# snap-research/graphless-neural-networks

Measured on AMD Instinct MI355X. Metric: aggregated edges/sec (teacher fwd) + student distill steps/sec, ogbn-products 1/2/4/8 GPU, higher is better.
Workload: dtype f32; 1 GPU; ogbn-products-shaped SAGE teacher forward (3 layers 100-256-256-47, BN, layer-wise full-neighbour inference, reference models.py:121-148) + MLP3w8 student KL distillation step; nodes=2449029, nnz=123718280, graph_fingerprint=2449029-123718280-12a892faaf-3b89008b386, parallelism=1 GPU

## Files before the change

graphless-neural-networks_amd/_lib.py:

```python
import ctypes
import os

_HERE = os.path.dirname(os.path.abspath(__file__))
LIB_PATH = os.environ.get("GLNN_LIB_PATH") or os.path.join(_HERE, "libglnn_hip.so")

c_i64, c_int, c_f32, c_vp, c_u32 = ctypes.c_int64, ctypes.c_int, ctypes.c_float, ctypes.c_void_p, ctypes.c_uint32
c_f64 = ctypes.c_double

SIGNATURES = {
    "glnn_abi_version": [],
    "glnn_device_info": [c_vp, c_vp, c_vp, c_int],
    "glnn_struct_bytes": [c_int],
    "glnn_spmm_csr_f32": [c_vp, c_vp, c_i64, c_i64, c_vp, c_i64, c_int, c_int, c_vp, c_vp, c_vp, c_i64, c_vp, c_vp, c_vp,
                          c_int, c_vp, c_i64, c_vp],
    "glnn_packed_weight_floats": [c_int, c_int],
    "glnn_pack_weight_f32": [c_vp, c_i64, c_int, c_int, c_vp, c_vp],
    "glnn_sage_fused_f32": [c_vp, c_vp, c_i64, c_i64, c_vp, c_i64, c_int, c_vp, c_i64, c_vp, c_int, c_vp, c_vp, c_int, c_vp,
                            c_i64, c_vp, c_int, c_vp, c_i64, c_vp, c_vp],
    "glnn_cast_f32_bf16": [c_vp, c_i64, c_i64, c_int, c_vp, c_i64, c_vp],
    "glnn_spmm_csr_bf16": [c_vp, c_vp, c_i64, c_i64, c_vp, c_i64, c_int, c_int, c_vp, c_vp, c_vp, c_i64, c_vp, c_vp, c_vp,
                           c_int, c_vp, c_i64, c_int, c_vp],
    "glnn_sage_fused_bf16": [c_vp, c_vp, c_i64, c_i64, c_vp, c_i64, c_int, c_vp, c_i64, c_vp, c_int, c_vp, c_vp, c_int, c_vp,
                             c_i64, c_int, c_vp, c_int, c_vp, c_i64, c_int, c_vp, c_vp],
    "glnn_hub_row_threshold": [],
    "glnn_hub_segment_edges": [],
    "glnn_spmm_csr_plan_f32": [c_vp, c_vp, c_i64, c_i64, c_vp, c_i64, c_int, c_int, c_vp, c_vp, c_vp, c_i64, c_vp, c_vp, c_vp,
                               c_int, c_vp, c_i64, c_vp, c_vp],
    "glnn_sage_fused_plan_f32": [c_vp, c_vp, c_i64, c_i64, c_vp, c_i64, c_int, c_vp, c_i64, c_vp, c_int, c_vp, c_vp, c_int, c_vp,
                                 c_i64, c_vp, c_int, c_vp, c_i64, c_vp, c_vp, c_vp],
    "glnn_sage_fused_agg_f32": [c_vp, c_vp, c_i64, c_i64, c_vp, c_i64, c_int, c_vp, c_i64, c_vp, c_int, c_vp, c_vp, c_int, c_vp,
                                c_i64, c_vp, c_int, c_vp, c_i64, c_vp, c_vp, c_vp, c_vp, c_i64, c_vp],
    "glnn_sage_fused_chunks_f32": [c_vp, c_vp, c_i64, c_i64, c_vp, c_i64, c_int, c_vp, c_i64, c_vp, c_int, c_vp, c_vp, c_int, c_vp,
                                   c_i64, c_vp, c_int, c_vp, c_i64, c_vp, c_vp, c_vp, c_vp],
    "glnn_spmm_csr_chunks_f32": [c_vp, c_vp, c_i64, c_i64, c_vp, c_i64, c_int, c_int, c_vp, c_vp, c_vp, c_i64, c_vp, c_vp, c_vp,
                                 c_int, c_vp, c_i64, c_vp, c_vp, c_vp],
    "glnn_signal_alloc": [c_vp],
    "glnn_signal_free": [c_vp],
    "glnn_signal_read": [c_vp, c_vp],
    "glnn_stream_wait_value32": [c_vp, c_vp, c_u32],
    "glnn_degrees_f32": [c_vp, c_vp, c_i64, c_i64, c_i64, c_int, c_vp, c_vp, c_vp],
    "glnn_gemm_f32": [c_vp, c_i64, c_vp, c_vp, c_vp, c_f32, c_u32, c_i64, c_int, c_vp, c_i64, c_int, c_int, c_vp, c_vp, c_vp, c_int,
                      c_vp, c_i64, c_vp, c_i64, c_vp],
    "glnn_gemm_tn_f32": [c_vp, c_i64, c_i64, c_int, c_vp, c_i64, c_vp, c_vp, c_vp, c_f32, c_u32, c_int, c_vp, c_i64, c_vp, c_vp,
                         c_i64, c_vp],
    "glnn_softmax_loss_f32": [c_vp, c_i64, c_i64, c_int, c_int, c_vp, c_vp, c_vp, c_i64, c_vp, c_f32, c_vp, c_i64,
                              c_vp, c_i64, c_vp, c_vp, c_vp, c_i64, c_vp],
    "glnn_log_softmax_f32": [c_vp, c_i64, c_i64, c_int, c_vp, c_i64, c_vp],
    "glnn_classifier_loss_f32": [c_vp, c_i64, c_vp, c_vp, c_f32, c_u32, c_i64, c_int, c_vp, c_i64, c_int, c_vp, c_vp, c_i64, c_int,
                                 c_vp, c_vp, c_vp, c_i64, c_vp, c_f32, c_vp, c_i64, c_vp, c_vp, c_vp, c_i64, c_vp],
    "glnn_linear_bn_stats_f32": [c_vp, c_i64, c_i64, c_int, c_vp, c_i64, c_int, c_vp, c_vp, c_i64, c_vp, c_vp, c_f32, c_f32, c_vp, c_vp, c_vp,
                                 c_vp, c_vp, c_vp, c_vp, c_vp, c_i64, c_vp, c_i64, c_vp],
    "glnn_bn_stats_f32": [c_vp, c_i64, c_i64, c_int, c_vp, c_vp, c_f32, c_f32, c_vp, c_vp, c_vp, c_vp, c_vp, c_vp,
                          c_vp, c_vp, c_i64, c_vp],
    "glnn_bn_relu_bwd_f32": [c_vp, c_i64, c_vp, c_i64, c_i64, c_int, c_vp, c_vp, c_vp, c_vp, c_vp, c_f32, c_u32, c_vp, c_i64,
                             c_vp, c_vp, c_vp, c_vp, c_i64, c_vp],
    "glnn_col_sum_f32": [c_vp, c_i64, c_i64, c_int, c_vp, c_vp, c_i64, c_vp],
    "glnn_adam_step_f32": [c_vp, c_vp, c_vp, c_vp, c_vp, c_int, c_i64, c_f32, c_f32, c_f32, c_f32, c_f32, c_i64, c_vp],
    "glnn_mlp_fwd_bwd_f32": [c_vp, c_vp, c_i64, c_vp, c_i64, c_int, c_vp, c_vp, c_i64, c_vp, c_f32, c_vp, c_vp],
    "glnn_mlp_train_step_f32": [c_vp, c_vp, c_i64, c_vp, c_i64, c_int, c_vp, c_vp, c_i64, c_vp, c_f32, c_vp, c_vp, c_vp],
    "glnn_sage_fwd_bwd_f32": [c_vp, c_vp],
    "glnn_sage_train_step_f32": [c_vp, c_vp, c_vp],
    "glnn_sage_step_ws_bn_floats": [c_i64, c_int],
    "glnn_sage_fwd_bwd_ln_f32": [c_vp, c_vp, c_vp],
    "glnn_sage_train_step_ln_f32": [c_vp, c_vp, c_vp, c_vp],
    "glnn_sage_step_ws_ln_floats": [c_i64, c_int],
    "glnn_sage_mean_fwd_bwd_f32": [c_vp, c_vp, c_vp, c_vp],
    "glnn_sage_mean_train_step_f32": [c_vp, c_vp, c_vp, c_vp, c_vp],
    "glnn_act_fwd_f32": [c_vp, c_i64, c_i64, c_int, c_vp, c_vp, c_f32, c_u32, c_vp, c_i64, c_vp],
    "glnn_norm_drop_fwd_f32": [c_vp, c_i64, c_i64, c_int, c_vp, c_vp, c_int, c_f32, c_u32, c_vp, c_i64, c_vp],
    "glnn_bn_bwd_f32": [c_vp, c_i64, c_vp, c_i64, c_i64, c_int, c_vp, c_vp, c_vp, c_vp, c_vp, c_int, c_f32, c_u32, c_vp, c_i64,
                        c_vp, c_vp, c_vp, c_vp, c_i64, c_vp],
    "glnn_layernorm_fwd_f32": [c_vp, c_i64, c_i64, c_int, c_vp, c_vp, c_f32, c_int, c_f32, c_u32, c_vp, c_i64, c_vp, c_vp, c_vp],
    "glnn_layernorm_bwd_workspace_floats": [c_i64, c_int],
    "glnn_layernorm_bwd_f32": [c_vp, c_i64, c_vp, c_i64, c_i64, c_int, c_vp, c_vp, c_vp, c_vp, c_int, c_f32, c_u32, c_vp, c_i64,
                               c_vp, c_vp, c_vp, c_vp, c_i64, c_vp],
    "glnn_dropout_mask_u8": [c_i64, c_int, c_f32, c_u32, c_vp, c_vp],
    "glnn_sample_neighbors": [c_vp, c_vp, c_vp, c_i64, c_int, c_u32, c_vp, c_vp, c_vp],
    "glnn_sample_csr_workspace_bytes": [c_i64],
    "glnn_sample_csr_indptr": [c_vp, c_i64, c_int, c_vp, c_vp, c_i64, c_vp],
    "glnn_sample_csr_fill": [c_vp, c_vp, c_i64, c_i64, c_vp, c_int, c_u32, c_vp, c_vp],
    "glnn_block_workspace_bytes": [c_i64, c_i64],
    "glnn_block_build": [c_vp, c_vp, c_vp, c_i64, c_vp, c_vp, c_int, c_i64, c_vp, c_vp, c_vp, c_vp, c_vp, c_vp, c_i64, c_vp],
    "glnn_block_build_ids": [c_vp, c_vp, c_vp, c_i64, c_vp, c_vp, c_int, c_i64, c_vp, c_vp, c_vp, c_vp, c_vp, c_i64, c_vp, c_i64, c_vp],
    "glnn_csr_transpose_workspace_bytes": [c_i64, c_i64],
    "glnn_csr_transpose": [c_vp, c_vp, c_i64, c_i64, c_i64, c_int, c_vp, c_vp, c_vp, c_i64, c_vp],
    "glnn_random_walk": [c_vp, c_vp, c_vp, c_i64, c_int, c_u32, c_vp, c_vp],
    "glnn_induced_subgraph_direct": [c_i64, c_i64],
    "glnn_induced_subgraph_workspace_bytes": [c_i64, c_i64],
    "glnn_induced_subgraph": [c_vp, c_vp, c_i64, c_vp, c_i64, c_int, c_i64, c_vp, c_vp, c_vp, c_vp, c_vp, c_i64, c_vp],
    "glnn_appnp_prop_f32": [c_vp, c_vp, c_i64, c_i64, c_vp, c_i64, c_int, c_vp, c_vp, c_vp, c_vp, c_i64, c_f32, c_f32, c_u32, c_int,
                            c_vp, c_i64, c_vp],
    "glnn_appnp_prop_bwd_f32": [c_vp, c_vp, c_vp, c_i64, c_i64, c_vp, c_i64, c_int, c_vp, c_vp, c_vp, c_f32, c_f32, c_u32, c_int, c_int,
                                c_vp, c_i64, c_vp, c_i64, c_vp],
    "glnn_csr_transpose_eids": [c_vp, c_vp, c_i64, c_i64, c_i64, c_vp, c_vp, c_vp, c_vp, c_i64, c_vp],
    "glnn_edge_drop_mask_u8": [c_i64, c_int, c_f32, c_u32, c_vp, c_vp],
    "glnn_deepwalk_pairs": [c_vp, c_vp, c_i64, c_vp, c_vp, c_i64, c_int, c_int, c_int, c_u32, c_u32, c_vp, c_vp, c_vp, c_vp, c_vp, c_vp],
    "glnn_deepwalk_score_f32": [c_vp, c_i64, c_int, c_vp, c_vp, c_i64, c_int, c_int, c_vp, c_vp, c_vp, c_vp, c_vp],
    "glnn_deepwalk_apply_f32": [c_vp, c_vp, c_vp, c_vp, c_i64, c_int, c_i64, c_int, c_int, c_vp, c_vp, c_vp, c_vp, c_vp, c_vp, c_f64,
                                c_f64, c_f64, c_f64, c_i64, c_vp, c_vp, c_vp],
    "glnn_node2vec_walk": [c_vp, c_vp, c_i64, c_vp, c_vp, c_i64, c_int, c_f64, c_f64, c_u32, c_vp, c_vp],
    "glnn_deepwalk_pairs_from_walks": [c_vp, c_i64, c_int, c_int, c_int, c_i64, c_u32, c_vp, c_vp, c_vp, c_vp, c_vp, c_vp],
    "glnn_deepwalk_score_ctx_f32": [c_vp, c_vp, c_i64, c_int, c_vp, c_vp, c_i64, c_int, c_int, c_vp, c_vp, c_vp, c_vp, c_vp],
    "glnn_gpr_prop_f32": [c_vp, c_vp, c_i64, c_i64, c_vp, c_i64, c_int, c_vp, c_vp, c_vp, c_vp, c_int, c_vp, c_i64, c_vp, c_i64, c_vp,
                          c_i64, c_vp, c_vp],
    "glnn_gpr_fold_f32": [c_vp, c_int, c_i64, c_vp, c_vp, c_i64, c_vp],
    "glnn_dagnn_gate_f32": [c_vp, c_i64, c_i64, c_int, c_vp, c_vp, c_int, c_vp, c_i64, c_vp, c_vp],
    "glnn_dagnn_gate_bwd_f32": [c_vp, c_i64, c_vp, c_i64, c_i64, c_int, c_vp, c_vp, c_int, c_vp, c_i64, c_vp, c_i64, c_vp, c_vp],
    "glnn_dagnn_fold_workspace_bytes": [c_i64, c_int],
    "glnn_dagnn_fold_f32": [c_vp, c_i64, c_vp, c_i64, c_int, c_vp, c_vp, c_vp, c_i64, c_vp],
    "glnn_gcnii_layer_f32": [c_vp, c_vp, c_i64, c_i64, c_vp, c_i64, c_int, c_vp, c_vp, c_vp, c_vp, c_i64, c_f32, c_f32, c_vp, c_f32, c_u32,
                             c_vp, c_i64, c_vp, c_i64, c_vp, c_vp],
    "glnn_gcnii_layer_bwd_f32": [c_vp, c_vp, c_i64, c_i64, c_vp, c_i64, c_int, c_vp, c_vp, c_vp, c_int, c_vp, c_i64, c_f32, c_u32, c_f32,
                                 c_f32, c_vp, c_f32, c_vp, c_i64, c_vp, c_i64, c_vp, c_i64, c_int, c_vp, c_vp],
    "glnn_gat_scores_f32": [c_vp, c_i64, c_vp, c_i64, c_i64, c_int, c_int, c_vp, c_vp, c_vp, c_vp, c_vp],
    "glnn_gat_attn_fwd_f32": [c_vp, c_vp, c_i64, c_i64, c_vp, c_i64, c_int, c_int, c_vp, c_vp, c_f32, c_f32, c_u32, c_int, c_vp, c_i64,
                              c_vp, c_vp],
    "glnn_gat_attn_bwd_workspace_floats": [c_i64, c_int, c_int],
    "glnn_gat_attn_bwd_f32": [c_vp, c_vp, c_vp, c_vp, c_vp, c_i64, c_i64, c_vp, c_i64, c_int, c_int, c_vp, c_vp, c_vp, c_vp, c_vp,
                              c_vp, c_i64, c_vp, c_i64, c_f32, c_f32, c_u32, c_vp, c_vp, c_vp, c_vp, c_i64, c_vp, c_vp, c_vp, c_i64, c_vp],
    "glnn_gat_attn_mask_u8": [c_i64, c_int, c_f32, c_u32, c_vp, c_vp],
    "glnn_gatv2_attn_fwd_f32": [c_vp, c_vp, c_i64, c_i64, c_vp, c_i64, c_vp, c_i64, c_int, c_int, c_vp, c_f32, c_f32, c_u32, c_int, c_vp,
                                c_i64, c_vp, c_vp],
    "glnn_gatv2_attn_bwd_workspace_floats": [c_i64, c_int, c_int],
    "glnn_gatv2_attn_bwd_f32": [c_vp, c_vp, c_vp, c_vp, c_vp, c_i64, c_i64, c_vp, c_i64, c_vp, c_i64, c_int, c_int, c_vp, c_vp, c_vp,
                                c_i64, c_f32, c_f32, c_u32, c_vp, c_vp, c_i64, c_vp, c_i64, c_vp, c_vp, c_i64, c_vp],
    "glnn_gt_attn_fwd_f32": [c_vp, c_vp, c_i64, c_i64, c_vp, c_i64, c_vp, c_i64, c_vp, c_i64, c_vp, c_i64, c_int, c_int, c_f32, c_u32, c_int,
                             c_vp, c_i64, c_vp, c_vp],
    "glnn_gt_attn_bwd_workspace_floats": [c_i64, c_int],
    "glnn_gt_attn_bwd_f32": [c_vp, c_vp, c_vp, c_vp, c_vp, c_i64, c_i64, c_vp, c_i64, c_vp, c_i64, c_vp, c_i64, c_int, c_int, c_vp, c_vp,
                             c_i64, c_f32, c_u32, c_vp, c_vp, c_i64, c_vp, c_i64, c_vp, c_i64, c_vp, c_i64, c_vp],
    "glnn_pna_agg_fwd_f32": [c_vp, c_vp, c_i64, c_i64, c_i64, c_vp, c_i64, c_int, c_vp, c_i64, c_vp, c_i64, c_vp, c_i64, c_vp, c_i64, c_vp],
    "glnn_pna_agg_bwd_f32": [c_vp, c_i64, c_vp, c_vp, c_vp, c_i64, c_i64, c_vp, c_i64, c_vp, c_i64, c_int, c_vp, c_i64, c_vp, c_i64, c_vp,
                             c_i64, c_vp, c_i64, c_vp],
    "glnn_pna_scale_fwd_f32": [c_vp, c_i64, c_int, c_f32, c_vp, c_i64, c_vp, c_i64, c_int, c_vp],
    "glnn_pna_scale_bwd_f32": [c_vp, c_i64, c_int, c_f32, c_vp, c_i64, c_vp, c_i64, c_vp],
    "glnn_pna_da_f32": [c_vp, c_i64, c_int, c_vp, c_i64, c_vp, c_i64, c_vp],
    "glnn_sage_mean_fused_f32": [c_vp, c_vp, c_i64, c_i64, c_vp, c_i64, c_int, c_vp, c_i64, c_vp, c_vp, c_int, c_vp, c_vp, c_int, c_vp,
                                 c_i64, c_vp, c_vp],
    "glnn_spmm_sage_mean_f32": [c_vp, c_vp, c_i64, c_i64, c_vp, c_i64, c_int, c_vp, c_i64, c_vp, c_vp, c_int, c_vp, c_i64, c_vp],
    "glnn_gather_rows_f32": [c_vp, c_i64, c_vp, c_i64, c_int, c_vp, c_i64, c_vp],
    "glnn_scatter_rows_f32": [c_vp, c_i64, c_vp, c_i64, c_int, c_vp, c_i64, c_vp],
    "glnn_gemm_bf16": [c_vp, c_i64, c_int, c_i64, c_int, c_vp, c_i64, c_int, c_vp, c_vp, c_int, c_vp, c_i64, c_int, c_int, c_vp],
    "glnn_mlp_forward_bf16": [c_vp, c_vp, c_i64, c_int, c_i64, c_vp, c_vp, c_i64, c_vp, c_i64, c_int, c_vp],
    "glnn_mlp_fused_bf16_tile_rows": [c_vp],
    "glnn_mlp_forward_fused_bf16": [c_vp, c_vp, c_i64, c_int, c_vp, c_i64, c_i64, c_vp, c_i64, c_int, c_vp],
    "glnn_position_rows": [c_vp, c_i64, c_vp, c_i64, c_int, c_int, c_vp, c_i64, c_int, c_i64, c_vp, c_i64, c_vp, c_vp, c_vp, c_i64, c_int,
                           c_vp],
}

MLP_MAX_LAYERS = 8
GPR_FOLD_CHUNK = 4096
DAGNN_FOLD_CHUNK = 2048
MLP_COUNTERS = 1024
_F = ctypes.c_void_p * MLP_MAX_LAYERS


ABI_VERSION = 12
GRAD_READY_FN = ctypes.CFUNCTYPE(ctypes.c_int, ctypes.c_void_p, ctypes.c_int, ctypes.c_void_p)
EXCHANGE_FN = ctypes.CFUNCTYPE(ctypes.c_int, ctypes.c_void_p, ctypes.c_void_p, ctypes.c_void_p, ctypes.c_int64, ctypes.c_void_p)


class AdamDesc(ctypes.Structure):
    _fields_ = [("params", ctypes.c_void_p), ("grads", ctypes.c_void_p), ("exp_avg", ctypes.c_void_p), ("exp_avg_sq", ctypes.c_void_p),
                ("sizes", ctypes.c_void_p), ("grads_host", ctypes.c_void_p), ("num_tensors", ctypes.c_int32), ("reserved", ctypes.c_int32),
                ("max_size", c_i64), ("lr", c_f32), ("beta1", c_f32), ("beta2", c_f32), ("eps", c_f32), ("weight_decay", c_f32),
                ("reserved2", ctypes.c_int32), ("step", c_i64)]


class HubPlanDesc(ctypes.Structure):
    _fields_ = [("rows", c_vp), ("seg_ptr", c_vp), ("n_hub", ctypes.c_int32), ("n_seg", ctypes.c_int32), ("slab", c_vp),
                ("ld_slab", c_i64), ("slab_rows", c_i64)]


MAX_CHUNKS = 8


class ChunkSignalsDesc(ctypes.Structure):
    _fields_ = [("n_chunks", ctypes.c_int32), ("row_start", c_i64 * (MAX_CHUNKS + 1)), ("self_row", c_i64 * MAX_CHUNKS),
# ... 116 lines not shown
```

graphless-neural-networks_amd/csrc/spmm.hip:

```cpp
#include "glnn_common.h"
#include "source_tail_dev.h"

namespace {

#ifndef GLNN_SPMM_U
#define GLNN_SPMM_U 8
#endif
#ifndef GLNN_FUSED_U
#define GLNN_FUSED_U 8
#endif
#ifndef GLNN_ROWS_PER_WAVE
#define GLNN_ROWS_PER_WAVE 16
#endif
#ifndef GLNN_LONG_ROW
#define GLNN_LONG_ROW 128
#endif
#ifndef GLNN_LONG_BLOCK_ROWS
#define GLNN_LONG_BLOCK_ROWS 512
#endif
#ifndef GLNN_LONG_BLOCK_CAP
#define GLNN_LONG_BLOCK_CAP 512
#endif
constexpr int kBlock = 512;
constexpr int kWavesPerBlock = kBlock / 64;
constexpr int kRowsPerWave = GLNN_ROWS_PER_WAVE;
constexpr int kLongRow = GLNN_LONG_ROW;
#ifndef GLNN_HUB_ROW
#define GLNN_HUB_ROW 1024
#endif
constexpr int kHubRow = GLNN_HUB_ROW;
constexpr int kHubSeg = 512;

struct HubPlan {
  const int64_t* rows;
  const int32_t* seg_ptr;
  int n_hub;
  float* slab;
  int64_t ld_slab;
};

struct ChunkMap {
  int n;
  int tile_start[GLNN_MAX_CHUNKS + 1];
  int64_t self_shift[GLNN_MAX_CHUNKS];
  int64_t out_shift[GLNN_MAX_CHUNKS];
  int* arrivals;
  uint32_t* signal[GLNN_MAX_CHUNKS];
  uint32_t epoch;
};

__device__ __forceinline__ int64_t cm_pick(const int64_t (&a)[GLNN_MAX_CHUNKS], int c) {
  int64_t r = a[0];
#pragma unroll
  for (int i = 1; i < GLNN_MAX_CHUNKS; ++i) r = (c == i) ? a[i] : r;
  return r;
}
__device__ __forceinline__ int cm_tile_start(const ChunkMap& cm, int c) {
  int r = cm.tile_start[0];
#pragma unroll
  for (int i = 1; i <= GLNN_MAX_CHUNKS; ++i) r = (c == i) ? cm.tile_start[i] : r;
  return r;
}
__device__ __forceinline__ uint32_t* cm_signal(const ChunkMap& cm, int c) {
  uint32_t* r = cm.signal[0];
#pragma unroll
  for (int i = 1; i < GLNN_MAX_CHUNKS; ++i) r = (c == i) ? cm.signal[i] : r;
  return r;
}
__device__ __forceinline__ void cm_arrive(const ChunkMap& cm, int c, int expected) {
  int* cnt = cm.arrivals + c;
  const int prev = __hip_atomic_fetch_add(cnt, 1, __ATOMIC_RELAXED, __HIP_MEMORY_SCOPE_AGENT);
  if (prev == expected - 1) {
    __hip_atomic_store(cnt, 0, __ATOMIC_RELAXED, __HIP_MEMORY_SCOPE_AGENT);
    __hip_atomic_store(cm_signal(cm, c), cm.epoch, __ATOMIC_RELEASE, __HIP_MEMORY_SCOPE_SYSTEM);
  }
}

struct SpmmArgs {
  const int64_t* indptr;
  const int32_t* indices;
  int64_t n_dst;
  const float* x;
  int64_t ldx;
  int d;
  const float* row_scale;
  const float* col_scale;
  const float* x_self;
  int64_t ld_self;
  const int64_t* self_rows;
  const float* ep_scale;
  const float* ep_shift;
  int relu;
  float* out;
  int64_t ldo;
  int n_long_blocks;
  int rows_per_block;
  int xf_on; const float* xf_scale; const float* xf_shift; uint32_t xf_thr; uint32_t xf_seed; float xf_dscale;
  const float* xf_mean; const float* xf_rstd;
  HubPlan hub;
  ChunkMap cm;
};

__device__ __forceinline__ float4 ld4(const float* p) { return *reinterpret_cast<const float4*>(p); }
__device__ __forceinline__ void st4(float* p, float4 v) { *reinterpret_cast<float4*>(p) = v; }
#ifndef GLNN_NT_STREAMS
#define GLNN_NT_STREAMS 1
#endif
typedef float f32x4_t __attribute__((ext_vector_type(4)));
__device__ __forceinline__ float4 ld4_stream(const float* p) {
#if GLNN_NT_STREAMS
  const f32x4_t t = __builtin_nontemporal_load(reinterpret_cast<const f32x4_t*>(p));
  return make_float4(t.x, t.y, t.z, t.w);
#else
  return ld4(p);
#endif
}
__device__ __forceinline__ void st4_stream(float* p, float4 v) {
#if GLNN_NT_STREAMS
  f32x4_t t = {v.x, v.y, v.z, v.w};
  __builtin_nontemporal_store(t, reinterpret_cast<f32x4_t*>(p));
#else
  st4(p, v);
#endif
}
__device__ __forceinline__ int ld_idx_stream(const int32_t* p) {
#if GLNN_NT_STREAMS
  return __builtin_nontemporal_load(p);
#else
  return *p;
#endif
}
__device__ __forceinline__ float div_corrected(float a, float d, float rd) {
  const float q = a * rd;
  const float e = fmaf(-q, d, a);
  return fmaf(e, rd, q);
}
__device__ __forceinline__ float4 mean4(float4 acc, float4 s, float d) {
  const float rd = __builtin_amdgcn_rcpf(d);
  return make_float4(div_corrected(acc.x + s.x, d, rd), div_corrected(acc.y + s.y, d, rd), div_corrected(acc.z + s.z, d, rd),
                     div_corrected(acc.w + s.w, d, rd));
}
__device__ __forceinline__ float4 add4(float4 a, float4 b) { return make_float4(a.x + b.x, a.y + b.y, a.z + b.z, a.w + b.w); }
__device__ __forceinline__ float4 fma4(float s, float4 v, float4 a) {
  return make_float4(fmaf(s, v.x, a.x), fmaf(s, v.y, a.y), fmaf(s, v.z, a.z), fmaf(s, v.w, a.w));
}
__device__ __forceinline__ float4 shfl_xor4(float4 v, int m) {
  return make_float4(__shfl_xor(v.x, m), __shfl_xor(v.y, m), __shfl_xor(v.z, m), __shfl_xor(v.w, m));
}

template <int LPR>
__device__ __forceinline__ float4 fold_groups(float4 acc) {
  constexpr int G = 64 / LPR;
  if (G >= 2) acc = add4(acc, shfl_xor4(acc, 32));
  if (G >= 4) acc = add4(acc, shfl_xor4(acc, 16));
  if (G >= 8) acc = add4(acc, shfl_xor4(acc, 8));
  if (G >= 16) acc = add4(acc, shfl_xor4(acc, 4));
  return acc;
}
template <int LPR, int U, bool CS, int XF = 0>
__device__ __forceinline__ float4 wave_gather_acc(const int32_t* __restrict__ indices, int64_t e0, int64_t e1,
                                                  int wave_id, int n_waves, const float* __restrict__ x,
                                                  int64_t ldx, int col4, bool col_ok,
                                                  const float* __restrict__ col_scale, int lane, const TailCols& xf, float4 acc) {
  constexpr int G = 64 / LPR;
  const int g = lane / LPR;
  for (int64_t base = e0 + (int64_t)wave_id * 64; base < e1; base += (int64_t)n_waves * 64) {
    const int64_t rem = e1 - base;
    const int cnt = rem < 64 ? (int)rem : 64;
    const int my_idx = lane < cnt ? ld_idx_stream(indices + base + lane) : 0;
    float my_cs = 1.f;
    if (CS) my_cs = lane < cnt ? col_scale[my_idx] : 0.f;
    for (int j = 0; j < cnt; j += G * U) {
      float4 v[U];
      float s[U];
      int srcs[U];
#pragma unroll
      for (int u = 0; u < U; ++u) {
        const int ei = j + u * G + g;
        int src;
        if (G == 1) {
          src = __builtin_amdgcn_readlane(my_idx, ei & 63);
        } else {
          src = __shfl(my_idx, ei & 63);
        }
        if (CS) s[u] = (G == 1) ? __builtin_bit_cast(float, __builtin_amdgcn_readlane(__builtin_bit_cast(int, my_cs), ei & 63))
                                : __shfl(my_cs, ei & 63);
        const bool ok = (ei < cnt) && col_ok;
        srcs[u] = ok ? src : -1;
        v[u] = ok ? ld4(x + (int64_t)src * ldx + col4) : make_float4(0.f, 0.f, 0.f, 0.f);
      }
      if (XF) {
#pragma unroll
        for (int u = 0; u < U; ++u)
          if (srcs[u] >= 0) v[u] = tail_apply<XF>(xf, v[u], (uint32_t)srcs[u]);
      }
#pragma unroll
      for (int u = 0; u < U; ++u) acc = CS ? fma4(s[u], v[u], acc) : add4(acc, v[u]);
    }
  }
  return acc;
}
template <int LPR, int U, bool CS, int XF = 0>
__device__ __forceinline__ float4 wave_gather_sum(const int32_t* __restrict__ indices, int64_t e0, int64_t e1,
                                                  int wave_id, int n_waves, const float* __restrict__ x,
                                                  int64_t ldx, int col4, bool col_ok,
                                                  const float* __restrict__ col_scale, int lane, const TailCols& xf) {
  return fold_groups<LPR>(wave_gather_acc<LPR, U, CS, XF>(indices, e0, e1, wave_id, n_waves, x, ldx, col4, col_ok, col_scale, lane, xf,
                                                           make_float4(0.f, 0.f, 0.f, 0.f)));
}

struct EpCols { float s[4], h[4]; };
__device__ __forceinline__ EpCols load_ep_cols(const SpmmArgs& a, int col4) {
  EpCols e;
#pragma unroll
  for (int t = 0; t < 4; ++t) {
    const bool ok = col4 + t < a.d;
    e.s[t] = (a.ep_scale && ok) ? a.ep_scale[col4 + t] : 1.f;
    e.h[t] = (a.ep_shift && ok) ? a.ep_shift[col4 + t] : 0.f;
  }
  return e;
}

template <int MODE>
__device__ __forceinline__ void finish_row_s(const SpmmArgs& a, int64_t v, int64_t deg, float4 acc, float4 s, int col4, const EpCols& ep,
                                             int64_t out_shift = 0) {
  float4 y;
  if (MODE == GLNN_AGG_SAGE_GCN) {
    const float dp1 = (float)deg + 1.0f;
    y = mean4(acc, s, dp1);
  } else {
    const float rs = a.row_scale ? a.row_scale[v] : 1.0f;
    y = make_float4(acc.x * rs, acc.y * rs, acc.z * rs, acc.w * rs);
  }
  float yy[4] = {y.x, y.y, y.z, y.w};
#pragma unroll
  for (int t = 0; t < 4; ++t) {
    const int c = col4 + t;
    if (c < a.d) {
      if (a.ep_scale) yy[t] *= ep.s[t];
      if (a.ep_shift) yy[t] += ep.h[t];
      if (a.relu) yy[t] = fmaxf(yy[t], 0.f);
    } else {
      yy[t] = 0.f;
    }
  }
  st4_stream(a.out + (v + out_shift) * a.ldo + col4, make_float4(yy[0], yy[1], yy[2], yy[3]));
}
template <int MODE, int XF = 0>
__device__ __forceinline__ void finish_row(const SpmmArgs& a, int64_t v, int64_t deg, float4 acc, int col4, const EpCols& ep,
                                           const TailCols& xf, int64_t out_shift = 0, int64_t self_shift = 0) {
  float4 s = make_float4(0.f, 0.f, 0.f, 0.f);
  if (MODE == GLNN_AGG_SAGE_GCN) {
    const int64_t sr = a.self_rows ? a.self_rows[v] : v + self_shift;
    s = ld4(a.x_self + sr * a.ld_self + col4);
    if (XF) s = tail_apply<XF>(xf, s, (uint32_t)sr);
  }
  finish_row_s<MODE>(a, v, deg, acc, s, col4, ep, out_shift);
}

__device__ __forceinline__ int hub_find(const HubPlan& h, int64_t v) {
  int lo = 0, hi = h.n_hub - 1;
  while (lo <= hi) {
    const int mid = (lo + hi) >> 1;
    const int64_t r = h.rows[mid];
    if (r == v) return mid;
    if (r < v) lo = mid + 1; else hi = mid - 1;
  }
  return -1;
}
template <int LPR, int U, bool CS, int XF>
__device__ __forceinline__ float4 hub_wave_share(const HubPlan& h, const int32_t* __restrict__ indices, int64_t v, int64_t e0, int64_t e1,
                                                 const float* __restrict__ x, int64_t ldx, int col4, bool col_ok, const float* __restrict__ col_scale,
                                                 int wave, int lane, const TailCols& xf) {
  float4 t = make_float4(0.f, 0.f, 0.f, 0.f);
  const int hi = h.n_hub > 0 ? hub_find(h, v) : -1;
  if (hi >= 0) {
    if (lane < LPR && col_ok) {
      const int s0 = h.seg_ptr[hi], s1 = h.seg_ptr[hi + 1];
      for (int sg = s0; sg < s1; ++sg) t = add4(t, ld4(h.slab + ((int64_t)sg * 8 + wave) * h.ld_slab + col4));
    }
    return t;
  }
  for (int64_t b = e0; b < e1; b += kHubSeg) {
    const int64_t be = b + kHubSeg < e1 ? b + kHubSeg : e1;
    t = add4(t, wave_gather_sum<LPR, U, CS, XF>(indices, b, be, wave, 8, x, ldx, col4, col_ok, col_scale, lane, xf));
  }
  return t;
}

template <int LPR, int U, bool CS, int XF>
__global__ __launch_bounds__(kBlock) void hub_gather_kernel(const SpmmArgs a) {
  const int lane = threadIdx.x & 63;
  const int wave = __builtin_amdgcn_readfirstlane(threadIdx.x >> 6);
  const int col4 = (lane % LPR) * 4;
  const bool col_ok = col4 < a.d;
  TailCols xf = {};
  if (XF) xf = load_tail_cols(a.xf_scale, a.xf_shift, a.xf_mean, a.xf_rstd, a.xf_thr, a.xf_seed, a.xf_dscale, a.d, col_ok ? col4 : 0, a.xf_on);
  const int sg = (int)blockIdx.x;
  int lo = 0, hi = a.hub.n_hub - 1;
  while (lo < hi) {
    const int mid = (lo + hi + 1) >> 1;
    if (a.hub.seg_ptr[mid] <= sg) lo = mid; else hi = mid - 1;
  }
  const int64_t v = a.hub.rows[lo];
  const int64_t e0 = a.indptr[v] + (int64_t)(sg - a.hub.seg_ptr[lo]) * kHubSeg;
  const int64_t e1r = a.indptr[v + 1];
  const int64_t e1 = e0 + kHubSeg < e1r ? e0 + kHubSeg : e1r;
  const float4 acc = wave_gather_sum<LPR, U, CS, XF>(a.indices, e0, e1, wave, 8, a.x, a.ldx, col4, col_ok, a.col_scale, lane, xf);
  if (lane < LPR && col_ok) st4(a.hub.slab + ((int64_t)sg * 8 + wave) * a.hub.ld_slab + col4, acc);
}

template <int LPR, int U, int MODE, bool CS, int XF = 0>
__device__ __forceinline__ void long_rows_role(const SpmmArgs& a, int lane, int wave, int col4, bool col_ok, const EpCols& ep,
                                               const TailCols& xf) {
  __shared__ int64_t s_rows[kBlock];
  __shared__ int s_count;
  __shared__ float4 s_part[kWavesPerBlock][64];
  const int64_t n_chunks = (a.n_dst + kBlock - 1) / kBlock;
  for (int64_t chunk = blockIdx.x; chunk < n_chunks; chunk += a.n_long_blocks) {
    if (threadIdx.x == 0) s_count = 0;
    __syncthreads();
    const int64_t r = (int64_t)threadIdx.x * n_chunks + chunk;
    if (r < a.n_dst && (a.indptr[r + 1] - a.indptr[r]) > kLongRow) {
      const int slot = atomicAdd(&s_count, 1);
      s_rows[slot] = r;
    }
    __syncthreads();
    const int n_found = s_count;
    for (int i = 0; i < n_found; ++i) {
      const int64_t v = s_rows[i];
      const int64_t e0 = a.indptr[v], e1 = a.indptr[v + 1];
      float4 acc;
      if (e1 - e0 > kHubRow)
        acc = hub_wave_share<LPR, U, CS, XF>(a.hub, a.indices, v, e0, e1, a.x, a.ldx, col4, col_ok, a.col_scale, wave, lane, xf);
      else
        acc = wave_gather_sum<LPR, U, CS, XF>(a.indices, e0, e1, wave, kWavesPerBlock, a.x, a.ldx, col4, col_ok, a.col_scale, lane, xf);
      if (lane < LPR) s_part[wave][lane] = acc;
      __syncthreads();
      if (wave == 0 && lane < LPR && col_ok) {
        float4 t = s_part[0][lane];
#pragma unroll
        for (int w = 1; w < kWavesPerBlock; ++w) t = add4(t, s_part[w][lane]);
        finish_row<MODE, XF>(a, v, e1 - e0, t, col4, ep, xf);
      }
      __syncthreads();
    }
  }
}

template <int LPR, int U, int MODE, bool CS, int XF>
__device__ __forceinline__ void long_rows_role_chunks(const SpmmArgs& a, const ChunkMap& cm, int lane, int wave, int col4, bool col_ok,
                                                      const EpCols& ep, const TailCols& xf) {
  __shared__ int64_t s_rows[kBlock];
  __shared__ int s_count;
  __shared__ float4 s_part[kWavesPerBlock][64];
  int64_t dealt = 0;
#pragma unroll 1
  for (int c = 0; c < cm.n; ++c) {
    const int64_t rs = (int64_t)cm_tile_start(cm, c) * 32;
    int64_t re = (int64_t)cm_tile_start(cm, c + 1) * 32;
    if (re > a.n_dst) re = a.n_dst;
    if (re <= rs) continue;
    const int64_t out_shift = cm_pick(cm.out_shift, c), self_shift = cm_pick(cm.self_shift, c);
    const int64_t n_sub = (re - rs + kBlock - 1) / kBlock;
    const int64_t first = ((int64_t)blockIdx.x - dealt % a.n_long_blocks + a.n_long_blocks) % a.n_long_blocks;
    dealt += n_sub;
#pragma unroll 1
    for (int64_t sub = first; sub < n_sub; sub += a.n_long_blocks) {
      if (threadIdx.x == 0) s_count = 0;
      __syncthreads();
      const int64_t r = rs + (int64_t)threadIdx.x * n_sub + sub;
      if (r < re && (a.indptr[r + 1] - a.indptr[r]) > kLongRow) {
        const int slot = atomicAdd(&s_count, 1);
        s_rows[slot] = r;
      }
      __syncthreads();
      const int n_found = s_count;
      for (int i = 0; i < n_found; ++i) {
        const int64_t v = s_rows[i];
        const int64_t e0 = a.indptr[v], e1 = a.indptr[v + 1];
        float4 acc;
        if (e1 - e0 > kHubRow)
          acc = hub_wave_share<LPR, U, CS, XF>(a.hub, a.indices, v, e0, e1, a.x, a.ldx, col4, col_ok, a.col_scale, wave, lane, xf);
        else
          acc = wave_gather_sum<LPR, U, CS, XF>(a.indices, e0, e1, wave, kWavesPerBlock, a.x, a.ldx, col4, col_ok, a.col_scale, lane, xf);
        if (lane < LPR) s_part[wave][lane] = acc;
        __syncthreads();
        if (wave == 0 && lane < LPR && col_ok) {
          float4 t = s_part[0][lane];
#pragma unroll
          for (int w = 1; w < kWavesPerBlock; ++w) t = add4(t, s_part[w][lane]);
          finish_row<MODE, XF>(a, v, e1 - e0, t, col4, ep, xf, out_shift, self_shift);
        }
        __syncthreads();
      }
    }
    if (wave == 0) {
      asm volatile("s_waitcnt vmcnt(0)" ::: "memory");
      if (lane == 0) {
        const int64_t rpb = a.rows_per_block;
        cm_arrive(cm, c, (int)((re - rs + rpb - 1) / rpb) + a.n_long_blocks);
      }
    }
  }
}

template <int LPR, int U, int MODE, bool CS, int XF = 0, bool CM = false>
__global__ __launch_bounds__(kBlock) void spmm_csr_kernel(const SpmmArgs a0) {
  SpmmArgs a = a0;
  if (gridDim.y > 1) {
    const int off = 256 * (int)blockIdx.y;
    a.x += off; a.out += off; a.d = a0.d - off < 256 ? a0.d - off : 256;
    if (a.x_self) a.x_self += off;
    if (a.ep_scale) a.ep_scale += off;
    if (a.ep_shift) a.ep_shift += off;
  }
  const int lane = threadIdx.x & 63;
  const int wave = __builtin_amdgcn_readfirstlane(threadIdx.x >> 6);
  const int c = lane % LPR;
  const int col4 = c * 4;
  const bool col_ok = col4 < a.d;
  const EpCols ep = load_ep_cols(a, col_ok ? col4 : 0);
  TailCols xf = {};
  if (XF) xf = load_tail_cols(a.xf_scale, a.xf_shift, a.xf_mean, a.xf_rstd, a.xf_thr, a.xf_seed, a.xf_dscale, a.d, col_ok ? col4 : 0, a.xf_on);

  if ((int)blockIdx.x < a.n_long_blocks) {
    if constexpr (CM) long_rows_role_chunks<LPR, U, MODE, CS, XF>(a, a0.cm, lane, wave, col4, col_ok, ep, xf);
    else long_rows_role<LPR, U, MODE, CS, XF>(a, lane, wave, col4, col_ok, ep, xf);
    return;
  }

  __shared__ int s_ticket;
  __shared__ int s_arrived;
  if (threadIdx.x == 0) { s_ticket = 0; if (CM) s_arrived = 0; }
  __syncthreads();
  const int64_t blk = (int64_t)blockIdx.x - a.n_long_blocks;
  const int64_t row_base = blk * a.rows_per_block;
  int chunk = 0;
  int64_t out_shift = 0, self_shift = 0;
  if constexpr (CM) {
#pragma unroll
    for (int c = 1; c < GLNN_MAX_CHUNKS; ++c)
      if (c < a0.cm.n && row_base >= (int64_t)a0.cm.tile_start[c] * 32) chunk = c;
    out_shift = cm_pick(a0.cm.out_shift, chunk);
    self_shift = cm_pick(a0.cm.self_shift, chunk);
  }
#pragma unroll 1
  while (true) {
    int lr = 0;
    if (lane == 0) lr = atomicAdd(&s_ticket, 1);
    lr = __builtin_amdgcn_readfirstlane(lr);
    if (lr >= a.rows_per_block) break;
    const int64_t v = row_base + lr;
    if (v >= a.n_dst) break;
    const int64_t e0 = a.indptr[v], e1 = a.indptr[v + 1];
    const int64_t deg = e1 - e0;
    if (deg > kLongRow) continue;
    float4 acc = wave_gather_sum<LPR, U, CS, XF>(a.indices, e0, e1, 0, 1, a.x, a.ldx, col4, col_ok, a.col_scale, lane, xf);
    if (lane < LPR && col_ok) finish_row<MODE, XF>(a, v, deg, acc, col4, ep, xf, out_shift, self_shift);
  }
  if constexpr (CM) {
    asm volatile("s_waitcnt vmcnt(0)" ::: "memory");
    if (lane == 0 && atomicAdd(&s_arrived, 1) == kWavesPerBlock - 1) {
      const int64_t rs = (int64_t)cm_tile_start(a0.cm, chunk) * 32;
      int64_t re = (int64_t)cm_tile_start(a0.cm, chunk + 1) * 32;
      if (re > a.n_dst) re = a.n_dst;
      const int64_t rpb = a.rows_per_block;
      cm_arrive(a0.cm, chunk, (int)((re - rs + rpb - 1) / rpb) + a.n_long_blocks);
    }
  }
}

constexpr int kShortRows = 4;
constexpr int kShortUnits = 3;
__device__ __forceinline__ int64_t readlane64(int64_t v, int l) {
  const uint32_t lo = (uint32_t)__builtin_amdgcn_readlane((int)(uint32_t)v, l);
  const uint32_t hi = (uint32_t)__builtin_amdgcn_readlane((int)(uint32_t)((uint64_t)v >> 32), l);
  return (int64_t)(((uint64_t)hi << 32) | lo);
}
template <int LPR, int U, int MODE, bool CS, int XF = 0>
__global__ __launch_bounds__(kBlock) void spmm_csr_short_kernel(const SpmmArgs a) {
  constexpr int G = 64 / LPR, RB = kShortRows, UB = kShortUnits;
  const int lane = threadIdx.x & 63;
  const int wave = __builtin_amdgcn_readfirstlane(threadIdx.x >> 6);
  const int c = lane % LPR, g = lane / LPR;
  const int col4 = c * 4;
  const bool col_ok = col4 < a.d;
  const EpCols ep = load_ep_cols(a, col_ok ? col4 : 0);
  TailCols xf = {};
  if (XF) xf = load_tail_cols(a.xf_scale, a.xf_shift, a.xf_mean, a.xf_rstd, a.xf_thr, a.xf_seed, a.xf_dscale, a.d, col_ok ? col4 : 0, a.xf_on);
  if ((int)blockIdx.x < a.n_long_blocks) {
    long_rows_role<LPR, U, MODE, CS, XF>(a, lane, wave, col4, col_ok, ep, xf);
    return;
  }
  __shared__ int s_ticket;
  if (threadIdx.x == 0) s_ticket = 0;
  __syncthreads();
  const int64_t blk = (int64_t)blockIdx.x - a.n_long_blocks;
  const int64_t row_base = blk * a.rows_per_block;
#pragma unroll 1
  while (true) {
    int lr = 0;
    if (lane == 0) lr = atomicAdd(&s_ticket, RB);
    lr = __builtin_amdgcn_readfirstlane(lr);
    if (lr >= a.rows_per_block) break;
    const int64_t v0 = row_base + lr;
    if (v0 >= a.n_dst) break;
    int nr = a.rows_per_block - lr;
    if (nr > RB) nr = RB;
    if (v0 + nr > a.n_dst) nr = (int)(a.n_dst - v0);
    const int64_t my_ptr = a.indptr[v0 + (lane <= nr ? lane : nr)];
    int64_t my_self = v0 + (lane < nr ? lane : 0);
    if (MODE == GLNN_AGG_SAGE_GCN && a.self_rows) my_self = a.self_rows[v0 + (lane < nr ? lane : 0)];
    int64_t e[RB + 1];
#pragma unroll
    for (int r = 0; r <= RB; ++r) e[r] = readlane64(my_ptr, r <= nr ? r : nr);
    const int64_t ebase = e[0];
    int64_t span = e[RB] - ebase;
    const int tot = span < 64 ? (int)span : 64;
    const int my_idx = lane < tot ? ld_idx_stream(a.indices + ebase + lane) : 0;
    float my_cs = 0.f;
    if (CS) my_cs = lane < tot ? a.col_scale[my_idx] : 0.f;
    int hd[RB];
    bool live[RB];
    float4 v[RB][UB], selfv[RB];
    float sc[RB][UB];
    int srcs[RB][UB];
#pragma unroll
    for (int r = 0; r < RB; ++r) {
      const int64_t deg = e[r + 1] - e[r];
      const int off = (int)(e[r] - ebase < 64 ? e[r] - ebase : 64);
      live[r] = r < nr && deg <= kLongRow;
      int h = deg < UB * G ? (int)deg : UB * G;
      if (!live[r] || off + h > tot) h = 0;
      hd[r] = h;
#pragma unroll
      for (int k = 0; k < UB; ++k) {
        const int first = k * G + g;
        const int ei = off + first;
        int src;
        if (G == 1) src = __builtin_amdgcn_readlane(my_idx, ei & 63);
        else src = __shfl(my_idx, ei & 63);
        float cs = 0.f;
        if (CS) cs = (G == 1) ? __builtin_bit_cast(float, __builtin_amdgcn_readlane(__builtin_bit_cast(int, my_cs), ei & 63)) : __shfl(my_cs, ei & 63);
        const bool ok = first < h && col_ok;
        srcs[r][k] = ok ? src : -1;
        sc[r][k] = ok ? cs : 0.f;
        v[r][k] = ok ? ld4(a.x + (int64_t)src * a.ldx + col4) : make_float4(0.f, 0.f, 0.f, 0.f);
      }
      selfv[r] = make_float4(0.f, 0.f, 0.f, 0.f);
      if (MODE == GLNN_AGG_SAGE_GCN) {
        const int64_t sr = readlane64(my_self, r < nr ? r : 0);
        if (live[r] && col_ok) {
          selfv[r] = ld4(a.x_self + sr * a.ld_self + col4);
          if (XF) selfv[r] = tail_apply<XF>(xf, selfv[r], (uint32_t)sr);
        }
      }
    }
#pragma unroll
    for (int r = 0; r < RB; ++r) {
      float4 acc = make_float4(0.f, 0.f, 0.f, 0.f);
#pragma unroll
      for (int k = 0; k < UB; ++k) {
        if (XF) {
          if (srcs[r][k] >= 0) v[r][k] = tail_apply<XF>(xf, v[r][k], (uint32_t)srcs[r][k]);
        }
        acc = CS ? fma4(sc[r][k], v[r][k], acc) : add4(acc, v[r][k]);
      }
      if (!live[r]) continue;
      const int64_t deg = e[r + 1] - e[r];
      if (deg > hd[r])
        acc = wave_gather_acc<LPR, U, CS, XF>(a.indices, e[r] + hd[r], e[r + 1], 0, 1, a.x, a.ldx, col4, col_ok, a.col_scale, lane, xf, acc);
      acc = fold_groups<LPR>(acc);
      if (lane < LPR && col_ok) finish_row_s<MODE>(a, v0 + r, deg, acc, selfv[r], col4, ep);
    }
  }
}

struct DyTail {
  const float* z; int64_t ldz; const float* mean; const float* rstd; const float* a_scale; const float* a_shift;
  uint32_t dthr; uint32_t dseed; float dscale; int relu; float* ws1; float* ws2; int h;
// ... 203 lines not shown
    dy[k] = d;
    dxh[k] = d * g[k];
    s1 += dxh[k];
    s2 = fmaf(dxh[k], x, s2);
  }
  const float m1 = wave_sum64(s1) * t.inv_h, m2 = wave_sum64(s2) * t.inv_h;
  if (!mine) return;
  float o[4];
#pragma unroll
  for (int k = 0; k < 4; ++k) {
    o[k] = col4 + k < t.h ? rs * (dxh[k] - m1 - xh[k] * m2) : 0.f;
    pg[k] = fmaf(dy[k], xh[k], pg[k]);
    pb[k] += dy[k];
    pz[k] += o[k];
  }
  st4_stream(a.out + v * a.ldo + col4, make_float4(o[0], o[1], o[2], o[3]));
}

template <int LPR, int U, bool DROP>
__global__ __launch_bounds__(kBlock) void spmm_ln_dz_kernel(const SpmmArgs a, const LnDzTail t) {
  const int lane = threadIdx.x & 63;
  const int wave = __builtin_amdgcn_readfirstlane(threadIdx.x >> 6);
  const int col4 = (lane % LPR) * 4;
  const bool col_ok = col4 < a.d;
  const bool mine = lane < LPR && col_ok;
  float g[4], b[4];
#pragma unroll
  for (int k = 0; k < 4; ++k) {
    const bool ok = col_ok && col4 + k < a.d;
    g[k] = ok ? t.gamma[col4 + k] : 0.f;
    b[k] = ok ? t.beta[col4 + k] : 0.f;
  }
  const TailCols xf = {};
  float pg[4] = {0.f, 0.f, 0.f, 0.f}, pb[4] = {0.f, 0.f, 0.f, 0.f}, pz[4] = {0.f, 0.f, 0.f, 0.f};
  __shared__ float4 s_part[kWavesPerBlock][64];
  if ((int)blockIdx.x < a.n_long_blocks) {
    __shared__ int64_t s_rows[kBlock], s_sorted[kBlock];
    __shared__ int s_count;
    const int64_t n_chunks = (a.n_dst + kBlock - 1) / kBlock;
    for (int64_t chunk = blockIdx.x; chunk < n_chunks; chunk += a.n_long_blocks) {
      if (threadIdx.x == 0) s_count = 0;
      __syncthreads();
      const int64_t r = (int64_t)threadIdx.x * n_chunks + chunk;
      if (r < a.n_dst && (a.indptr[r + 1] - a.indptr[r]) > kLongRow) s_rows[atomicAdd(&s_count, 1)] = r;
      __syncthreads();
      const int n_found = s_count;
      if ((int)threadIdx.x < n_found) {
        const int64_t me = s_rows[threadIdx.x];
        int rank = 0;
        for (int i = 0; i < n_found; ++i) rank += s_rows[i] < me ? 1 : 0;
        s_sorted[rank] = me;
      }
      __syncthreads();
      for (int i = 0; i < n_found; ++i) {
        const int64_t v = s_sorted[i];
        const int64_t e0 = a.indptr[v], e1 = a.indptr[v + 1];
        float4 z4 = make_float4(0.f, 0.f, 0.f, 0.f);
        if (wave == 0 && mine) z4 = ld4(t.z + v * t.ldz + col4);
        float4 acc;
        if (e1 - e0 > kHubRow) acc = hub_wave_share<LPR, U, true, 0>(a.hub, a.indices, v, e0, e1, a.x, a.ldx, col4, col_ok, a.col_scale, wave, lane, xf);
        else acc = wave_gather_sum<LPR, U, true, 0>(a.indices, e0, e1, wave, kWavesPerBlock, a.x, a.ldx, col4, col_ok, a.col_scale, lane, xf);
        if (lane < LPR) s_part[wave][lane] = acc;
        __syncthreads();
        if (wave == 0) {
          float4 sum = make_float4(0.f, 0.f, 0.f, 0.f);
          if (lane < LPR) {
            sum = s_part[0][lane];
#pragma unroll
            for (int w = 1; w < kWavesPerBlock; ++w) sum = add4(sum, s_part[w][lane]);
          }
          finish_ln_row<DROP>(a, t, g, b, v, sum, z4, col4, mine, pg, pb, pz);
        }
        __syncthreads();
      }
    }
  } else {
    const int64_t row_base = ((int64_t)blockIdx.x - a.n_long_blocks) * a.rows_per_block;
#pragma unroll 1
    for (int lr = wave; lr < a.rows_per_block; lr += kWavesPerBlock) {
      const int64_t v = row_base + lr;
      if (v >= a.n_dst) break;
      const int64_t e0 = a.indptr[v], e1 = a.indptr[v + 1];
      if (e1 - e0 > kLongRow) continue;
      float4 z4 = make_float4(0.f, 0.f, 0.f, 0.f);
      if (mine) z4 = ld4(t.z + v * t.ldz + col4);
      const float4 acc = wave_gather_sum<LPR, U, true, 0>(a.indices, e0, e1, 0, 1, a.x, a.ldx, col4, col_ok, a.col_scale, lane, xf);
      finish_ln_row<DROP>(a, t, g, b, v, acc, z4, col4, mine, pg, pb, pz);
    }
  }
  float* slot = t.ws + (int64_t)blockIdx.x * 3 * t.h;
#pragma unroll
  for (int q = 0; q < 3; ++q) {
    const float* p = q == 0 ? pg : (q == 1 ? pb : pz);
    __syncthreads();
    if (lane < LPR) s_part[wave][lane] = make_float4(p[0], p[1], p[2], p[3]);
    __syncthreads();
    if (wave == 0 && mine) {
      float4 u = s_part[0][lane];
#pragma unroll
      for (int w = 1; w < kWavesPerBlock; ++w) u = add4(u, s_part[w][lane]);
      const float uu[4] = {u.x, u.y, u.z, u.w};
#pragma unroll
      for (int k = 0; k < 4; ++k)
        if (col4 + k < t.h) slot[q * t.h + col4 + k] = uu[k];
    }
  }
}

typedef float f32x16 __attribute__((ext_vector_type(16)));
constexpr int kFusedWaves = 8;
constexpr int kFusedBlock = 64 * kFusedWaves;

template <bool CM>
__device__ __forceinline__ void store_out(float* p, float v) {
  *p = v;
}

template <bool CM>
__device__ __forceinline__ void chunk_arrive(const ChunkMap& cm, int chunk, bool stored, int lane, int* s_arrived) {
  if constexpr (CM) {
    if (stored) asm volatile("s_waitcnt vmcnt(0)" ::: "memory");
    if (lane != 0) return;
    if (atomicAdd(s_arrived, 1) != kFusedWaves - 1) return;
    int* cnt = cm.arrivals + chunk;
    const int prev = __hip_atomic_fetch_add(cnt, 1, __ATOMIC_RELAXED, __HIP_MEMORY_SCOPE_AGENT);
    int expected = 0;
    uint32_t* sig = nullptr;
#pragma unroll
    for (int c = 0; c < GLNN_MAX_CHUNKS; ++c)
      if (c == chunk) { expected = cm.tile_start[c + 1] - cm.tile_start[c]; sig = cm.signal[c]; }
    if (prev == expected - 1) {
      __hip_atomic_store(cnt, 0, __ATOMIC_RELAXED, __HIP_MEMORY_SCOPE_AGENT);
      __hip_atomic_store(sig, cm.epoch, __ATOMIC_RELEASE, __HIP_MEMORY_SCOPE_SYSTEM);
    }
  }
}

struct FusedArgs {
  const int64_t* indptr; const int32_t* indices; int64_t n_dst;
  const float* x; int64_t ldx; int d_in;
  const float* x_self; int64_t ld_self;
  const float* w_packed; int d_out; int kgroups;
  const float* ep_scale; const float* ep_shift; int relu;
  float* out; int64_t ldo;
  const float* w2_packed; int d_out2; int kgroups2; float* out2; int64_t ldo2;
  const int32_t* tile_order;
  HubPlan hub;
  ChunkMap cm;
  float* agg_out; const float* agg_in; int64_t ld_agg;
};

constexpr int kAggNone = 0, kAggOut = 1, kAggIn = 2;

template <int LPR, int U, int RT, bool CM = false, int AGG = kAggNone>
__global__ __launch_bounds__(kFusedBlock) void sage_fused_kernel(const FusedArgs a) {
  constexpr int kFusedRows = 32 * RT;
  extern __shared__ __attribute__((aligned(16))) float lds_a[];
  __shared__ float4 s_part[kFusedWaves / 2][64];
  const int lane = threadIdx.x & 63;
  const int wave = __builtin_amdgcn_readfirstlane(threadIdx.x >> 6);
  const int col4 = (lane % LPR) * 4;
  const bool col_ok = col4 < a.d_in;
  const int kpad = a.kgroups * 8;
  const int lda = kpad + 4;
  const int tile_id = (AGG != kAggIn && a.tile_order) ? a.tile_order[blockIdx.x] : (int)blockIdx.x;
  const int64_t row0 = (int64_t)tile_id * kFusedRows;
  int chunk = 0;
  int64_t self_shift = 0, out_shift = 0;
  if constexpr (CM) {
    self_shift = a.cm.self_shift[0];
    out_shift = a.cm.out_shift[0];
#pragma unroll
    for (int c = 1; c < GLNN_MAX_CHUNKS; ++c)
      if (c < a.cm.n && tile_id >= a.cm.tile_start[c]) { chunk = c; self_shift = a.cm.self_shift[c]; out_shift = a.cm.out_shift[c]; }
  }

  __shared__ int s_next;
  __shared__ int s_arrived;
  if constexpr (AGG == kAggIn) {
    const int kv = kpad / 4, dpad = (a.d_in + 3) & ~3;
    for (int i = threadIdx.x; i < kFusedRows * kv; i += kFusedBlock) {
      const int lr = i / kv, c4 = (i - lr * kv) * 4;
      const int64_t v = row0 + lr;
      float4 y = make_float4(0.f, 0.f, 0.f, 0.f);
      if (v < a.n_dst && c4 < dpad) y = ld4_stream(a.agg_in + v * a.ld_agg + c4);
      st4(lds_a + lr * lda + c4, y);
    }
  }
  if (threadIdx.x == 0) { s_next = 0; if (CM) s_arrived = 0; }
  __syncthreads();
#pragma unroll 1
  while (AGG != kAggIn) {
    int lr = 0;
    if (lane == 0) lr = atomicAdd(&s_next, 1);
    lr = __builtin_amdgcn_readfirstlane(lr);
    if (lr >= kFusedRows) break;
    const int64_t v = row0 + lr;
    float4 y = make_float4(0.f, 0.f, 0.f, 0.f);
    bool deferred = false;
    if (v < a.n_dst) {
      const int64_t e0 = a.indptr[v], e1 = a.indptr[v + 1];
      const int64_t deg = e1 - e0;
      deferred = deg > kLongRow;
      if (!deferred) {
        const float4 acc = wave_gather_sum<LPR, U, false>(a.indices, e0, e1, 0, 1, a.x, a.ldx, col4, col_ok, nullptr, lane, TailCols{});
        if (lane < LPR && col_ok) {
          const float4 sf = ld4(a.x_self + (v + self_shift) * a.ld_self + col4);
          const float dp1 = (float)deg + 1.0f;
          y = mean4(acc, sf, dp1);
          if (col4 + 1 >= a.d_in) y.y = 0.f;
          if (col4 + 2 >= a.d_in) y.z = 0.f;
          if (col4 + 3 >= a.d_in) y.w = 0.f;
        }
      }
    }
    if (!deferred && lane < LPR && col4 < kpad) {
      st4(lds_a + lr * lda + col4, y);
      if constexpr (AGG == kAggOut)
        if (v < a.n_dst && col4 < a.ld_agg) st4_stream(a.agg_out + v * a.ld_agg + col4, y);
    }
  }
  __syncthreads();
#pragma unroll 1
  for (int lr = 0; AGG != kAggIn && lr < kFusedRows; ++lr) {
    const int64_t v = row0 + lr;
    if (v >= a.n_dst) break;
    const int64_t e0 = a.indptr[v], e1 = a.indptr[v + 1];
    if (e1 - e0 <= kLongRow) continue;
    const float4 acc = e1 - e0 > kHubRow
        ? hub_wave_share<LPR, U, false, false>(a.hub, a.indices, v, e0, e1, a.x, a.ldx, col4, col_ok, nullptr, wave, lane, TailCols{})
        : wave_gather_sum<LPR, U, false>(a.indices, e0, e1, wave, kFusedWaves, a.x, a.ldx, col4, col_ok, nullptr, lane, TailCols{});
    if (wave >= 4 && lane < LPR) s_part[wave - 4][lane] = acc;
    __syncthreads();
    if (wave < 4 && lane < LPR) s_part[wave][lane] = add4(acc, s_part[wave][lane]);
    __syncthreads();
    if (wave == 0 && lane < LPR && col4 < kpad) {
      const float4 t = add4(add4(s_part[0][lane], s_part[1][lane]), add4(s_part[2][lane], s_part[3][lane]));
      float4 y = make_float4(0.f, 0.f, 0.f, 0.f);
      if (col_ok) {
        const float4 sf = ld4(a.x_self + (v + self_shift) * a.ld_self + col4);
        const float dp1 = (float)(e1 - e0) + 1.0f;
        y = mean4(t, sf, dp1);
        if (col4 + 1 >= a.d_in) y.y = 0.f;
        if (col4 + 2 >= a.d_in) y.z = 0.f;
        if (col4 + 3 >= a.d_in) y.w = 0.f;
      }
      st4(lds_a + lr * lda + col4, y);
      if constexpr (AGG == kAggOut)
        if (col4 < a.ld_agg) st4_stream(a.agg_out + v * a.ld_agg + col4, y);
    }
    __syncthreads();
  }

  const int n_tiles = (a.d_out + 31) / 32;
  const int nt = wave;
  const bool chain = a.w2_packed != nullptr;
  if (nt >= n_tiles && !chain) { chunk_arrive<CM>(a.cm, chunk, false, lane, &s_arrived); return; }
  const int li = lane & 31, kk = lane >> 5;
  f32x16 acc[RT];
#pragma unroll
  for (int t = 0; t < RT; ++t)
#pragma unroll
    for (int r = 0; r < 16; ++r) acc[t][r] = 0.f;
  if (nt < n_tiles) {
    const float4* wp = reinterpret_cast<const float4*>(a.w_packed) + ((int64_t)nt * a.kgroups) * 64 + lane;
    const float* ap = lds_a + li * lda + kk * 4;
    constexpr int PF = 4;
    float4 bq[PF];
#pragma unroll
    for (int q = 0; q < PF; ++q) bq[q] = (q < a.kgroups) ? wp[(int64_t)q * 64] : make_float4(0.f, 0.f, 0.f, 0.f);
    for (int kg0 = 0; kg0 < a.kgroups; kg0 += PF) {
#pragma unroll
      for (int q = 0; q < PF; ++q) {
        const int kg = kg0 + q;
        if (kg < a.kgroups) {
          const float4 bv = bq[q];
          const int nxt = kg + PF;
          if (nxt < a.kgroups) bq[q] = wp[(int64_t)nxt * 64];
          float4 av[RT];
#pragma unroll
          for (int t = 0; t < RT; ++t) av[t] = *reinterpret_cast<const float4*>(ap + t * 32 * lda + kg * 8);
#pragma unroll
          for (int t = 0; t < RT; ++t) acc[t] = __builtin_amdgcn_mfma_f32_32x32x2f32(av[t].x, bv.x, acc[t], 0, 0, 0);
#pragma unroll
          for (int t = 0; t < RT; ++t) acc[t] = __builtin_amdgcn_mfma_f32_32x32x2f32(av[t].y, bv.y, acc[t], 0, 0, 0);
#pragma unroll
          for (int t = 0; t < RT; ++t) acc[t] = __builtin_amdgcn_mfma_f32_32x32x2f32(av[t].z, bv.z, acc[t], 0, 0, 0);
#pragma unroll
          for (int t = 0; t < RT; ++t) acc[t] = __builtin_amdgcn_mfma_f32_32x32x2f32(av[t].w, bv.w, acc[t], 0, 0, 0);
        }
      }
    }
  }
  const int col = nt * 32 + li;
  const int ldh = a.kgroups2 * 8 + 4;
  if (chain) __syncthreads();
  if (nt < n_tiles) {
    const bool col_ok2 = col < a.d_out;
    const float es = (a.ep_scale && col_ok2) ? a.ep_scale[col] : 1.f;
    const float eh = (a.ep_shift && col_ok2) ? a.ep_shift[col] : 0.f;
#pragma unroll
    for (int t = 0; t < RT; ++t)
#pragma unroll
      for (int r = 0; r < 16; ++r) {
        const int lr = t * 32 + (r & 3) + 8 * (r >> 2) + 4 * kk;
        const int64_t row = row0 + lr;
        float v = fmaf(acc[t][r], es, eh);
        if (a.relu) v = fmaxf(v, 0.f);
        if (!col_ok2) v = 0.f;
        if (a.out && col_ok2 && row < a.n_dst) store_out<CM>(a.out + (row + out_shift) * a.ldo + col, v);
        if (chain && col < a.kgroups2 * 8) lds_a[lr * ldh + col] = v;
      }
  }
  if (!chain) { chunk_arrive<CM>(a.cm, chunk, true, lane, &s_arrived); return; }
  __syncthreads();
  const int n_tiles2 = (a.d_out2 + 31) / 32;
  if (nt >= n_tiles2) { chunk_arrive<CM>(a.cm, chunk, a.out != nullptr && nt < n_tiles, lane, &s_arrived); return; }
  {
    const float4* wp = reinterpret_cast<const float4*>(a.w2_packed) + ((int64_t)nt * a.kgroups2) * 64 + lane;
    const float* ap = lds_a + li * ldh + kk * 4;
#pragma unroll
    for (int t = 0; t < RT; ++t)
#pragma unroll
      for (int r = 0; r < 16; ++r) acc[t][r] = 0.f;
    for (int kg = 0; kg < a.kgroups2; ++kg) {
      const float4 bv = wp[(int64_t)kg * 64];
#pragma unroll
      for (int t = 0; t < RT; ++t) {
        const float4 av = *reinterpret_cast<const float4*>(ap + t * 32 * ldh + kg * 8);
        acc[t] = __builtin_amdgcn_mfma_f32_32x32x2f32(av.x, bv.x, acc[t], 0, 0, 0);
        acc[t] = __builtin_amdgcn_mfma_f32_32x32x2f32(av.y, bv.y, acc[t], 0, 0, 0);
        acc[t] = __builtin_amdgcn_mfma_f32_32x32x2f32(av.z, bv.z, acc[t], 0, 0, 0);
        acc[t] = __builtin_amdgcn_mfma_f32_32x32x2f32(av.w, bv.w, acc[t], 0, 0, 0);
      }
    }
    const int col2 = nt * 32 + li;
    if (col2 < a.d_out2) {
#pragma unroll
      for (int t = 0; t < RT; ++t)
#pragma unroll
        for (int r = 0; r < 16; ++r) {
          const int64_t row = row0 + t * 32 + (r & 3) + 8 * (r >> 2) + 4 * kk;
          if (row < a.n_dst) store_out<CM>(a.out2 + (row + out_shift) * a.ldo2 + col2, acc[t][r]);
        }
    }
  }
  chunk_arrive<CM>(a.cm, chunk, true, lane, &s_arrived);
}

__global__ void pack_weight_kernel(const float* __restrict__ w, int64_t ldw, int d_out, int d_in, int kgroups,
                                   float* __restrict__ wp) {
  const int64_t total = (int64_t)((d_out + 31) / 32) * kgroups * 256;
  for (int64_t i = (int64_t)blockIdx.x * blockDim.x + threadIdx.x; i < total; i += (int64_t)gridDim.x * blockDim.x) {
    const int t = (int)(i & 3), lane = (int)((i >> 2) & 63);
    const int64_t g = i >> 8;
    const int kg = (int)(g % kgroups), nt = (int)(g / kgroups);
    const int n = nt * 32 + (lane & 31), k = kg * 8 + (lane >> 5) * 4 + t;
    wp[i] = (n < d_out && k < d_in) ? w[(int64_t)n * ldw + k] : 0.f;
  }
}

template <int LPR, int U>
int launch_hub_gather(const SpmmArgs& a, int mode, int n_seg, hipStream_t st) {
  const bool cs = a.col_scale != nullptr;
  const dim3 g((unsigned)n_seg);
  if (mode == GLNN_AGG_SAGE_GCN && a.xf_on == 2) hipLaunchKernelGGL((hub_gather_kernel<LPR, U, false, 2>), g, dim3(kBlock), 0, st, a);
  else if (mode == GLNN_AGG_SAGE_GCN && a.xf_on) hipLaunchKernelGGL((hub_gather_kernel<LPR, U, false, true>), g, dim3(kBlock), 0, st, a);
  else if (cs) hipLaunchKernelGGL((hub_gather_kernel<LPR, U, true, false>), g, dim3(kBlock), 0, st, a);
  else hipLaunchKernelGGL((hub_gather_kernel<LPR, U, false, false>), g, dim3(kBlock), 0, st, a);
  return glnn::check_launch("glnn_spmm_csr_f32(hub segments)");
}

template <int LPR, int U>
int launch_lpr(const SpmmArgs& a, int mode, hipStream_t st, int grid, int col_tiles = 1, int hub_segs = 0, bool short_rows = false) {
  const bool cs = a.col_scale != nullptr;
  const dim3 g(grid, col_tiles);
  if (hub_segs > 0) {
    const int rc = launch_hub_gather<LPR, U>(a, mode, hub_segs, st);
    if (rc != GLNN_OK) return rc;
  }
  if constexpr (LPR >= 32) {
    if (short_rows && col_tiles == 1 && mode == GLNN_AGG_SAGE_GCN && !a.xf_on && a.cm.n == 0) {
      hipLaunchKernelGGL((spmm_csr_short_kernel<LPR, U, GLNN_AGG_SAGE_GCN, false>), g, dim3(kBlock), 0, st, a);
      return glnn::check_launch("glnn_spmm_csr_f32(short rows)");
    }
  }
  if (a.cm.n > 0) {
    if (mode != GLNN_AGG_SAGE_GCN || a.xf_on || col_tiles != 1)
      return glnn::fail(GLNN_ERR_UNSUPPORTED, "glnn_spmm_csr_chunks_f32: SAGE_GCN rows of <= 256 floats without a source transform only");
    hipLaunchKernelGGL((spmm_csr_kernel<LPR, U, GLNN_AGG_SAGE_GCN, false, false, true>), g, dim3(kBlock), 0, st, a);
    return glnn::check_launch("glnn_spmm_csr_chunks_f32");
  }
  if (mode == GLNN_AGG_SAGE_GCN && a.xf_on == 2) {
    hipLaunchKernelGGL((spmm_csr_kernel<LPR, U, GLNN_AGG_SAGE_GCN, false, 2>), g, dim3(kBlock), 0, st, a);
  } else if (mode == GLNN_AGG_SAGE_GCN && a.xf_on) {
    hipLaunchKernelGGL((spmm_csr_kernel<LPR, U, GLNN_AGG_SAGE_GCN, false, true>), g, dim3(kBlock), 0, st, a);
  } else if (mode == GLNN_AGG_SAGE_GCN) {
    hipLaunchKernelGGL((spmm_csr_kernel<LPR, U, GLNN_AGG_SAGE_GCN, false>), g, dim3(kBlock), 0, st, a);
  } else if (cs) {
    hipLaunchKernelGGL((spmm_csr_kernel<LPR, U, GLNN_AGG_SUM, true>), g, dim3(kBlock), 0, st, a);
  } else {
    hipLaunchKernelGGL((spmm_csr_kernel<LPR, U, GLNN_AGG_SUM, false>), g, dim3(kBlock), 0, st, a);
  }
  return glnn::check_launch("glnn_spmm_csr_f32");
}

__device__ __forceinline__ float degree_transform(float deg, int transform) {
  if (transform == GLNN_DEG_RSQRT_CLAMP1) return rsqrtf(fmaxf(deg, 1.0f));
  if (transform == GLNN_DEG_INV_PLUS1) return 1.0f / (deg + 1.0f);
  return deg;
}

__global__ void degrees_kernel(const int64_t* __restrict__ indptr, const int32_t* __restrict__ indices, int64_t n_dst,
                               int64_t nnz, float* in_deg, float* out_deg_as_int, int transform) {
  const int64_t i = (int64_t)blockIdx.x * blockDim.x + threadIdx.x;
  const int64_t stride = (int64_t)gridDim.x * blockDim.x;
  if (in_deg)
    for (int64_t v = i; v < n_dst; v += stride) in_deg[v] = degree_transform((float)(indptr[v + 1] - indptr[v]), transform);
  if (out_deg_as_int) {
    int* cnt = reinterpret_cast<int*>(out_deg_as_int);
    for (int64_t e = i; e < nnz; e += stride) atomicAdd(&cnt[indices[e]], 1);
  }
}

__global__ void int_to_float_kernel(float* p, int64_t n, int transform) {
  const int64_t i = (int64_t)blockIdx.x * blockDim.x + threadIdx.x;
  if (i < n) p[i] = degree_transform((float)reinterpret_cast<int*>(p)[i], transform);
}

}

static int hub_plan_of(const glnn_hub_plan* plan, int d, HubPlan* h, int* n_seg, const char* who) {
  h->rows = nullptr; h->seg_ptr = nullptr; h->n_hub = 0; h->slab = nullptr; h->ld_slab = 0;
  *n_seg = 0;
  if (!plan || plan->n_hub == 0) return GLNN_OK;
  const int dpad = (d + 3) & ~3;
  GLNN_REQUIRE(plan->n_hub > 0 && plan->n_seg >= plan->n_hub && plan->rows && plan->seg_ptr && plan->slab, "%s: incomplete hub plan", who);
  GLNN_REQUIRE(plan->ld_slab % 4 == 0 && plan->ld_slab >= dpad && plan->slab_rows >= 8 * (int64_t)plan->n_seg && glnn::aligned16(plan->slab),
               "%s: the hub plan's slab needs >= %d rows (8 per segment) of >= %d floats (ld multiple of 4), 16-byte aligned", who, 8 * plan->n_seg, dpad);
  h->rows = plan->rows; h->seg_ptr = plan->seg_ptr; h->n_hub = plan->n_hub; h->slab = plan->slab; h->ld_slab = plan->ld_slab;
  *n_seg = plan->n_seg;
  return GLNN_OK;
}

static int fill_chunk_map(const glnn_chunk_signals* chunks, int64_t n_dst, ChunkMap* cm, const char* who) {
  *cm = ChunkMap{};
  if (!chunks) return GLNN_OK;
  const int nc = chunks->n_chunks;
  GLNN_REQUIRE(nc >= 1 && nc <= GLNN_MAX_CHUNKS && chunks->arrivals && chunks->row_start[0] == 0 && chunks->row_start[nc] >= n_dst,
               "%s: 1..%d chunks covering rows [0, n_dst), arrival counters", who, GLNN_MAX_CHUNKS);
  const int64_t tiles = (n_dst + 31) / 32;
  GLNN_REQUIRE(tiles < ((int64_t)1 << 31), "%s: n_dst too large for one launch", who);
  cm->n = nc; cm->arrivals = chunks->arrivals; cm->epoch = chunks->epoch;
  for (int c = 0; c < nc; ++c) {
    const int64_t r0 = chunks->row_start[c], r1 = chunks->row_start[c + 1];
    GLNN_REQUIRE(r0 % 32 == 0 && r1 >= r0 && chunks->signal[c] && chunks->self_row[c] >= 0 && chunks->out_row[c] >= 0,
                 "%s: chunk %d: row_start must be an ascending multiple of 32, signal / rows set", who, c);
    cm->tile_start[c] = (int)(r0 / 32 < tiles ? r0 / 32 : tiles);
    cm->self_shift[c] = chunks->self_row[c] - r0;
    cm->out_shift[c] = chunks->out_row[c] - r0;
    cm->signal[c] = chunks->signal[c];
  }
  for (int c = nc; c <= GLNN_MAX_CHUNKS; ++c) cm->tile_start[c] = (int)tiles;
  return GLNN_OK;
}

static int spmm_impl(const int64_t* indptr, const int32_t* indices, int64_t n_dst, int64_t n_src,
                     const float* x, int64_t ldx, int d, int mode, const float* row_scale,
                     const float* col_scale, const float* x_self, int64_t ld_self, const int64_t* self_rows,
                     const float* ep_scale, const float* ep_shift, int relu, float* out, int64_t ldo,
                     void* stream, const glnn::SourceTail* tail, const glnn_hub_plan* plan = nullptr, int64_t nnz_hint = -1,
                     const glnn_chunk_signals* chunks = nullptr) {
  if (n_dst == 0) return GLNN_OK;
  GLNN_REQUIRE(indptr && x && out, "glnn_spmm_csr_f32: null pointer");
  GLNN_REQUIRE(n_dst >= 0 && n_src >= 0 && n_src < (int64_t)1 << 31, "glnn_spmm_csr_f32: bad n_dst/n_src");
  GLNN_REQUIRE(d >= 1, "glnn_spmm_csr_f32: d=%d must be >= 1", d);
  GLNN_REQUIRE(mode == GLNN_AGG_SUM || mode == GLNN_AGG_SAGE_GCN, "glnn_spmm_csr_f32: unknown mode %d", mode);
  const int dpad = (d + 3) & ~3;
  GLNN_REQUIRE(ldx % 4 == 0 && ldx >= dpad, "glnn_spmm_csr_f32: ldx=%lld must be a multiple of 4 and >= %d", (long long)ldx, dpad);
  GLNN_REQUIRE(ldo % 4 == 0 && ldo >= dpad, "glnn_spmm_csr_f32: ldo=%lld must be a multiple of 4 and >= %d", (long long)ldo, dpad);
  GLNN_REQUIRE(glnn::aligned16(x) && glnn::aligned16(out), "glnn_spmm_csr_f32: x/out must be 16-byte aligned");
  if (mode == GLNN_AGG_SAGE_GCN) {
    GLNN_REQUIRE(x_self && ld_self % 4 == 0 && ld_self >= dpad && glnn::aligned16(x_self),
                 "glnn_spmm_csr_f32: SAGE_GCN needs x_self with ld multiple of 4");
    GLNN_REQUIRE(!row_scale && !col_scale, "glnn_spmm_csr_f32: scales are not used in SAGE_GCN mode");
  } else {
    GLNN_REQUIRE(!self_rows, "glnn_spmm_csr_f32: self_rows belongs to SAGE_GCN mode");
  }
  if (n_dst == 0) return GLNN_OK;
  hipStream_t st = reinterpret_cast<hipStream_t>(stream);

  const bool wide = d > 256 && (d + 255) / 256 <= 65535;
  if (tail) {
    GLNN_REQUIRE(mode == GLNN_AGG_SAGE_GCN && d <= 256, "glnn::spmm_csr_tail: SAGE_GCN rows of <= 256 floats only");
    GLNN_REQUIRE((tail->scale == nullptr) == (tail->shift == nullptr) && tail->drop_p >= 0.f && tail->drop_p < 1.f, "glnn::spmm_csr_tail: bad tail");
    GLNN_REQUIRE((tail->mean == nullptr) == (tail->rstd == nullptr) && (!tail->mean || tail->scale), "glnn::spmm_csr_tail: bad LayerNorm tail");
  }
  for (int c0 = 0; c0 < d; c0 += (wide ? d : 256)) {
    const int dt = wide ? 256 : ((d - c0) < 256 ? (d - c0) : 256);
    SpmmArgs a;
    a.indptr = indptr; a.indices = indices; a.n_dst = n_dst;
    a.x = x + c0; a.ldx = ldx; a.d = wide ? d : dt;
    a.row_scale = row_scale; a.col_scale = col_scale;
    a.x_self = x_self ? x_self + c0 : nullptr; a.ld_self = ld_self; a.self_rows = self_rows;
    a.ep_scale = ep_scale ? ep_scale + c0 : nullptr; a.ep_shift = ep_shift ? ep_shift + c0 : nullptr;
    a.relu = relu; a.out = out + c0; a.ldo = ldo;
    a.xf_on = tail ? (tail->mean ? 2 : 1) : 0;
    a.xf_mean = tail ? tail->mean : nullptr; a.xf_rstd = tail ? tail->rstd : nullptr;
    a.xf_scale = tail ? tail->scale : nullptr; a.xf_shift = tail ? tail->shift : nullptr;
    a.xf_thr = tail ? glnn::drop_threshold(tail->drop_p) : 0u; a.xf_seed = tail ? tail->drop_seed : 0u;
    a.xf_dscale = tail ? 1.0f / (1.0f - tail->drop_p) : 1.f;
    {
      GLNN_REQUIRE(!chunks || (d <= 256 && mode == GLNN_AGG_SAGE_GCN && !tail), "glnn_spmm_csr_chunks_f32: SAGE_GCN rows of <= 256 floats only");
      const int rcm = fill_chunk_map(chunks, n_dst, &a.cm, "glnn_spmm_csr_chunks_f32");
      if (rcm != GLNN_OK) return rcm;
    }
    int hub_segs = 0;
    {
      const int rch = hub_plan_of(d <= 256 ? plan : nullptr, d, &a.hub, &hub_segs, "glnn_spmm_csr_f32");
      if (rch != GLNN_OK) return rch;
    }
    int64_t n_long = (n_dst + GLNN_LONG_BLOCK_ROWS - 1) / GLNN_LONG_BLOCK_ROWS;
    if (n_long < 1) n_long = 1;
    if (n_long > GLNN_LONG_BLOCK_CAP) n_long = GLNN_LONG_BLOCK_CAP;
    a.n_long_blocks = (int)n_long;
    int64_t rpw = n_dst / (2048 * kWavesPerBlock);
    if (rpw < 1) rpw = 1;
    if (rpw > kRowsPerWave) rpw = kRowsPerWave;
    if (a.cm.n > 0) {
      int64_t p = 1;
      while (p * 2 <= rpw) p *= 2;
      for (int c = 1; c < a.cm.n; ++c)
        while (p > 1 && ((int64_t)a.cm.tile_start[c] * 32) % (kWavesPerBlock * p) != 0) p /= 2;
      rpw = p;
    }
    const int64_t rows_per_block = kWavesPerBlock * rpw;
    a.rows_per_block = (int)rows_per_block;
    const int64_t row_blocks = (n_dst + rows_per_block - 1) / rows_per_block;
    GLNN_REQUIRE(row_blocks + n_long < ((int64_t)1 << 31), "glnn_spmm_csr_f32: n_dst too large for one launch");
    const int grid = (int)(row_blocks + n_long);
    const int dv = (dt + 3) / 4;
    const bool short_rows = nnz_hint >= 0 && nnz_hint <= 6 * n_dst && glnn::opts().spmm_short != 0 && a.rows_per_block % kShortRows == 0;
    int rc;
    if (dv <= 4) rc = launch_lpr<4, GLNN_SPMM_U>(a, mode, st, grid, 1, hub_segs);
    else if (dv <= 8) rc = launch_lpr<8, GLNN_SPMM_U>(a, mode, st, grid, 1, hub_segs);
    else if (dv <= 16) rc = launch_lpr<16, GLNN_SPMM_U>(a, mode, st, grid, 1, hub_segs);
    else if (dv <= 32) rc = launch_lpr<32, GLNN_SPMM_U>(a, mode, st, grid, 1, hub_segs, short_rows);
    else rc = launch_lpr<64, GLNN_SPMM_U>(a, mode, st, grid, wide ? (d + 255) / 256 : 1, hub_segs, short_rows);
    if (rc != GLNN_OK) return rc;
  }
  return GLNN_OK;
}

extern "C" int glnn_spmm_csr_f32(const int64_t* indptr, const int32_t* indices, int64_t n_dst, int64_t n_src,
                                 const float* x, int64_t ldx, int d, int mode, const float* row_scale,
                                 const float* col_scale, const float* x_self, int64_t ld_self, const int64_t* self_rows,
                                 const float* ep_scale, const float* ep_shift, int relu, float* out, int64_t ldo,
                                 void* stream) {
  return spmm_impl(indptr, indices, n_dst, n_src, x, ldx, d, mode, row_scale, col_scale, x_self, ld_self, self_rows, ep_scale, ep_shift, relu,
                   out, ldo, stream, nullptr);
}

extern "C" int glnn_spmm_csr_plan_f32(const int64_t* indptr, const int32_t* indices, int64_t n_dst, int64_t n_src,
                                      const float* x, int64_t ldx, int d, int mode, const float* row_scale,
                                      const float* col_scale, const float* x_self, int64_t ld_self, const int64_t* self_rows,
                                      const float* ep_scale, const float* ep_shift, int relu, float* out, int64_t ldo,
                                      const glnn_hub_plan* plan, void* stream) {
  return spmm_impl(indptr, indices, n_dst, n_src, x, ldx, d, mode, row_scale, col_scale, x_self, ld_self, self_rows, ep_scale, ep_shift, relu,
                   out, ldo, stream, nullptr, plan);
}

extern "C" int glnn_spmm_csr_chunks_f32(const int64_t* indptr, const int32_t* indices, int64_t n_dst, int64_t n_src,
                                        const float* x, int64_t ldx, int d, int mode, const float* row_scale,
                                        const float* col_scale, const float* x_self, int64_t ld_self, const int64_t* self_rows,
                                        const float* ep_scale, const float* ep_shift, int relu, float* out, int64_t ldo,
                                        const glnn_hub_plan* plan, const glnn_chunk_signals* chunks, void* stream) {
  GLNN_REQUIRE(chunks, "glnn_spmm_csr_chunks_f32: chunks is NULL (use glnn_spmm_csr_plan_f32)");
  return spmm_impl(indptr, indices, n_dst, n_src, x, ldx, d, mode, row_scale, col_scale, x_self, ld_self, self_rows, ep_scale, ep_shift, relu,
                   out, ldo, stream, nullptr, plan, -1, chunks);
}

extern "C" int glnn_hub_row_threshold(void) { return kHubRow; }
extern "C" int glnn_hub_segment_edges(void) { return kHubSeg; }

int glnn::spmm_csr_tail(const int64_t* indptr, const int32_t* indices, int64_t n_dst, int64_t n_src, const float* z, int64_t ldz, int d,
                        const glnn::SourceTail& tail, float* out, int64_t ldo, void* stream, int64_t nnz) {
  return spmm_impl(indptr, indices, n_dst, n_src, z, ldz, d, GLNN_AGG_SAGE_GCN, nullptr, nullptr, z, ldz, nullptr, nullptr, nullptr, 0, out, ldo,
                   stream, &tail, nullptr, nnz);
}

int glnn::spmm_csr_nnz(const int64_t* indptr, const int32_t* indices, int64_t n_dst, int64_t n_src, int64_t nnz, const float* x, int64_t ldx, int d,
                       int mode, const float* col_scale, const float* x_self, int64_t ld_self, const int64_t* self_rows, float* out, int64_t ldo,
                       void* stream) {
  return spmm_impl(indptr, indices, n_dst, n_src, x, ldx, d, mode, nullptr, col_scale, x_self, ld_self, self_rows, nullptr, nullptr, 0, out, ldo,
                   stream, nullptr, nullptr, nnz);
}

static int64_t bn_dy_grid(int64_t n_dst, int* n_long_blocks, int* rows_per_block) {
  int64_t n_long = (n_dst + GLNN_LONG_BLOCK_ROWS - 1) / GLNN_LONG_BLOCK_ROWS;
  if (n_long < 1) n_long = 1;
  if (n_long > GLNN_LONG_BLOCK_CAP) n_long = GLNN_LONG_BLOCK_CAP;
  int64_t rpw = n_dst / (2048 * kWavesPerBlock);
  if (rpw < 4) rpw = 4;
  if (rpw > kRowsPerWave) rpw = kRowsPerWave;
  const int64_t rpb = kWavesPerBlock * rpw;
  if (n_long_blocks) *n_long_blocks = (int)n_long;
  if (rows_per_block) *rows_per_block = (int)rpb;
  return (n_dst + rpb - 1) / rpb + n_long;
}
extern "C" int64_t glnn_sage_step_ws_bn_floats(int64_t n_dst_0, int hidden) {
  if (n_dst_0 < 1 || hidden < 1) return 0;
  const int64_t h = (hidden + 3) & ~3;
  return 2 * bn_dy_grid(n_dst_0, nullptr, nullptr) * h + 5 * h + 8;
}

int glnn::spmm_csr_bn_dy(const int64_t* indptr, const int32_t* indices, int64_t n_dst, int64_t n_src, const float* x, int64_t ldx, int d,
                         const float* col_scale, const glnn::BnTail& tail, float* out, int64_t ldo, float* ws, int64_t ws_floats, int* nslots,
                         void* stream) {
  if (!indptr || !x || !out || !col_scale || !ws || !nslots || n_dst < 1 || n_src < 0 || n_src >= ((int64_t)1 << 31)) return GLNN_ERR_UNSUPPORTED;
  if (d <= 64 || d > 256 || (d & 3) || (ldx & 3) || (ldo & 3) || (tail.ldz & 3) || ldx < d || ldo < d || tail.ldz < d) return GLNN_ERR_UNSUPPORTED;
  if (!tail.z || !tail.mean || !tail.rstd || !tail.a_scale || !tail.a_shift || tail.drop_p < 0.f || tail.drop_p >= 1.f) return GLNN_ERR_UNSUPPORTED;
  if (!glnn::aligned16(x) || !glnn::aligned16(out) || !glnn::aligned16(tail.z) || !glnn::aligned16(tail.mean) || !glnn::aligned16(tail.rstd) ||
      !glnn::aligned16(tail.a_scale) || !glnn::aligned16(tail.a_shift) || !glnn::aligned16(ws))
    return GLNN_ERR_UNSUPPORTED;
  SpmmArgs a = {};
  a.indptr = indptr; a.indices = indices; a.n_dst = n_dst; a.x = x; a.ldx = ldx; a.d = d; a.col_scale = col_scale; a.out = out; a.ldo = ldo;
  const int64_t slots = bn_dy_grid(n_dst, &a.n_long_blocks, &a.rows_per_block);
  if (slots >= ((int64_t)1 << 24) || 2 * slots * d > ws_floats) return GLNN_ERR_UNSUPPORTED;
  DyTail t;
  t.z = tail.z; t.ldz = tail.ldz; t.mean = tail.mean; t.rstd = tail.rstd; t.a_scale = tail.a_scale; t.a_shift = tail.a_shift;
  t.dthr = glnn::drop_threshold(tail.drop_p); t.dseed = tail.drop_seed; t.dscale = 1.0f / (1.0f - tail.drop_p); t.relu = tail.relu;
  t.ws1 = ws; t.ws2 = ws + slots * d; t.h = d;
  hipStream_t st = reinterpret_cast<hipStream_t>(stream);
  const dim3 g((unsigned)slots);
  if (d > 128) {
    if (t.dthr) hipLaunchKernelGGL((spmm_bn_dy_kernel<64, GLNN_SPMM_U, true>), g, dim3(kBlock), 0, st, a, t);
    else hipLaunchKernelGGL((spmm_bn_dy_kernel<64, GLNN_SPMM_U, false>), g, dim3(kBlock), 0, st, a, t);
  } else {
    if (t.dthr) hipLaunchKernelGGL((spmm_bn_dy_kernel<32, GLNN_SPMM_U, true>), g, dim3(kBlock), 0, st, a, t);
    else hipLaunchKernelGGL((spmm_bn_dy_kernel<32, GLNN_SPMM_U, false>), g, dim3(kBlock), 0, st, a, t);
  }
  *nslots = (int)slots;
  return glnn::check_launch("glnn::spmm_csr_bn_dy");
}

int64_t glnn::spmm_csr_ln_dz_ws_floats(int64_t n_dst, int d) { return n_dst < 1 || d < 1 ? 0 : 3 * bn_dy_grid(n_dst, nullptr, nullptr) * (int64_t)d; }

int glnn::spmm_csr_ln_dz(const int64_t* indptr, const int32_t* indices, int64_t n_dst, int64_t n_src, const float* x, int64_t ldx, int d,
                         const float* col_scale, const glnn::LnTail& tail, float* out, int64_t ldo, float* ws, int64_t ws_floats, int* nslots,
                         void* stream) {
  if (!indptr || !x || !out || !col_scale || !ws || !nslots || n_dst < 1 || n_src < 0 || n_src >= ((int64_t)1 << 31)) return GLNN_ERR_UNSUPPORTED;
  const int dpad = (d + 3) & ~3;
  if (d < 1 || d > 256 || (ldx & 3) || (ldo & 3) || (tail.ldz & 3) || ldx < dpad || ldo < dpad || tail.ldz < dpad) return GLNN_ERR_UNSUPPORTED;
  if (!tail.z || !tail.mean || !tail.rstd || !tail.gamma || !tail.beta || tail.drop_p < 0.f || tail.drop_p >= 1.f) return GLNN_ERR_UNSUPPORTED;
  if (!glnn::aligned16(x) || !glnn::aligned16(out) || !glnn::aligned16(tail.z)) return GLNN_ERR_UNSUPPORTED;
  SpmmArgs a = {};
  a.indptr = indptr; a.indices = indices; a.n_dst = n_dst; a.x = x; a.ldx = ldx; a.d = d; a.col_scale = col_scale; a.out = out; a.ldo = ldo;
  const int64_t slots = bn_dy_grid(n_dst, &a.n_long_blocks, &a.rows_per_block);
  if (slots >= ((int64_t)1 << 24) || 3 * slots * d > ws_floats) return GLNN_ERR_UNSUPPORTED;
  LnDzTail t;
  t.z = tail.z; t.ldz = tail.ldz; t.mean = tail.mean; t.rstd = tail.rstd; t.gamma = tail.gamma; t.beta = tail.beta;
  t.dthr = glnn::drop_threshold(tail.drop_p); t.dseed = tail.drop_seed; t.dscale = 1.0f / (1.0f - tail.drop_p); t.inv_h = 1.0f / (float)d;
  t.ws = ws; t.h = d;
  hipStream_t st = reinterpret_cast<hipStream_t>(stream);
  const dim3 g((unsigned)slots);
  const int dv = dpad / 4;
  const bool drop = t.dthr != 0;
#define GLNN_LN_DZ(LPR)                                                                                             \
  do {                                                                                                              \
    if (drop) hipLaunchKernelGGL((spmm_ln_dz_kernel<LPR, GLNN_SPMM_U, true>), g, dim3(kBlock), 0, st, a, t);        \
    else hipLaunchKernelGGL((spmm_ln_dz_kernel<LPR, GLNN_SPMM_U, false>), g, dim3(kBlock), 0, st, a, t);            \
  } while (0)
  if (dv <= 8) GLNN_LN_DZ(8);
  else if (dv <= 16) GLNN_LN_DZ(16);
  else if (dv <= 32) GLNN_LN_DZ(32);
  else GLNN_LN_DZ(64);
#undef GLNN_LN_DZ
  *nslots = (int)slots;
  return glnn::check_launch("glnn::spmm_csr_ln_dz");
}

extern "C" int64_t glnn_sage_step_ws_ln_floats(int64_t n_dst, int hidden) {
  if (n_dst < 1 || hidden < 1) return 0;
  const int64_t fused = glnn::spmm_csr_ln_dz_ws_floats(n_dst, hidden), plain = glnn_layernorm_bwd_workspace_floats(n_dst, hidden);
  return (fused > plain ? fused : plain) + 1024;
}

extern "C" int glnn_degrees_f32(const int64_t* indptr, const int32_t* indices, int64_t n_dst, int64_t n_src,
                                int64_t nnz, int transform, float* in_deg, float* out_deg, void* stream) {
  GLNN_REQUIRE(indptr, "glnn_degrees_f32: null indptr");
  GLNN_REQUIRE(transform >= GLNN_DEG_RAW && transform <= GLNN_DEG_INV_PLUS1, "glnn_degrees_f32: unknown transform %d", transform);
  GLNN_REQUIRE(!out_deg || indices, "glnn_degrees_f32: out_deg needs indices");
  hipStream_t st = reinterpret_cast<hipStream_t>(stream);
  GLNN_REQUIRE(nnz >= 0 && n_dst >= 0 && n_src >= 0, "glnn_degrees_f32: negative size");
  if (out_deg) {
    if (hipMemsetAsync(out_deg, 0, sizeof(float) * (size_t)n_src, st) != hipSuccess)
      return glnn::fail(GLNN_ERR_HIP, "glnn_degrees_f32: memset failed");
  }
  const int64_t work = nnz > n_dst ? nnz : n_dst;
  int grid = (int)((work + 255) / 256);
  if (grid > 4096) grid = 4096;
  if (grid < 1) grid = 1;
  hipLaunchKernelGGL(degrees_kernel, dim3(grid), dim3(256), 0, st, indptr, indices, n_dst, nnz, in_deg, out_deg, transform);
  if (out_deg && n_src > 0)
    hipLaunchKernelGGL(int_to_float_kernel, dim3((unsigned)((n_src + 255) / 256)), dim3(256), 0, st, out_deg, n_src, transform);
  return glnn::check_launch("glnn_degrees_f32");
}

extern "C" int64_t glnn_packed_weight_floats(int d_out, int d_in) {
  return (int64_t)((d_out + 31) / 32) * ((d_in + 7) / 8) * 256;
}

extern "C" int glnn_pack_weight_f32(const float* w, int64_t ldw, int d_out, int d_in, float* w_packed, void* stream) {
  GLNN_REQUIRE(w && w_packed && d_out >= 1 && d_in >= 1 && ldw >= d_in, "glnn_pack_weight_f32: bad arguments");
  GLNN_REQUIRE(glnn::aligned16(w_packed), "glnn_pack_weight_f32: w_packed must be 16-byte aligned");
  const int kgroups = (d_in + 7) / 8;
  const int64_t total = glnn_packed_weight_floats(d_out, d_in);
  int64_t blocks = (total + 255) / 256;
  if (blocks > 1024) blocks = 1024;
  hipLaunchKernelGGL(pack_weight_kernel, dim3((unsigned)blocks), dim3(256), 0, reinterpret_cast<hipStream_t>(stream), w, ldw, d_out,
                     d_in, kgroups, w_packed);
  return glnn::check_launch("glnn_pack_weight_f32");
}

static int sage_fused_agg_in(int64_t n_dst, int d_in, const float* w_packed, int d_out, const float* ep_scale, const float* ep_shift,
                             int relu, float* out, int64_t ldo, const float* w2_packed, int d_out2, float* out2, int64_t ldo2,
                             const float* agg_in, int64_t ld_agg, void* stream) {
  GLNN_REQUIRE(w_packed && (out || w2_packed), "glnn_sage_fused_agg_f32: null pointer");
  GLNN_REQUIRE(!w2_packed || (out2 && d_out2 >= 1 && d_out2 <= 256 && ldo2 >= d_out2 && glnn::aligned16(w2_packed)),
               "glnn_sage_fused_agg_f32: the chained projection needs out2 with ldo2 >= d_out2 in [1,256]");
  GLNN_REQUIRE(n_dst >= 0, "glnn_sage_fused_agg_f32: bad n_dst");
  GLNN_REQUIRE(d_in >= 1 && d_in <= 256 && d_out >= 1 && d_out <= 256, "glnn_sage_fused_agg_f32: d_in and d_out must be in [1,256]");
  const int dpad = (d_in + 3) & ~3;
  GLNN_REQUIRE(ld_agg % 4 == 0 && ld_agg >= dpad && (!out || ldo >= d_out),
               "glnn_sage_fused_agg_f32: leading dimensions (ld_agg a multiple of 4 and >= %d; ldo >= d_out)", dpad);
  GLNN_REQUIRE(glnn::aligned16(agg_in) && glnn::aligned16(w_packed), "glnn_sage_fused_agg_f32: 16-byte alignment required");
  FusedArgs a = {};
  a.n_dst = n_dst; a.d_in = d_in; a.w_packed = w_packed; a.d_out = d_out; a.kgroups = (d_in + 7) / 8; a.ep_scale = ep_scale;
  a.ep_shift = ep_shift; a.relu = relu; a.out = out; a.ldo = ldo;
  a.w2_packed = w2_packed; a.d_out2 = w2_packed ? d_out2 : 0; a.kgroups2 = w2_packed ? (d_out + 7) / 8 : 0; a.out2 = out2; a.ldo2 = ldo2;
  a.agg_in = agg_in; a.ld_agg = ld_agg;
  if (!w2_packed && out && d_out >= 96 && n_dst >= 2048 && glnn::opts().agg_in_rowwalk) {
    const int rc = glnn::gemm_rowwalk_packed(agg_in, ld_agg, n_dst, d_in, w_packed, d_out, ep_scale, ep_shift, relu, out, ldo, stream);
    if (rc != GLNN_ERR_UNSUPPORTED) return rc;
    (void)hipGetLastError();
  }
  constexpr int rt = 1;
  const int64_t blocks = (n_dst + 32 * rt - 1) / (32 * rt);
  GLNN_REQUIRE(blocks < ((int64_t)1 << 31), "glnn_sage_fused_agg_f32: n_dst too large for one launch");
  const int kg_lds = a.kgroups2 > a.kgroups ? a.kgroups2 : a.kgroups;
  const size_t smem = sizeof(float) * 32 * rt * (kg_lds * 8 + 4);
  hipLaunchKernelGGL((sage_fused_kernel<64, GLNN_FUSED_U, rt, false, kAggIn>), dim3((unsigned)blocks), dim3(kFusedBlock), smem,
                     reinterpret_cast<hipStream_t>(stream), a);
  return glnn::check_launch("glnn_sage_fused_agg_f32");
}

static int sage_fused_impl(const int64_t* indptr, const int32_t* indices, int64_t n_dst, int64_t n_src, const float* x,
                           int64_t ldx, int d_in, const float* x_self, int64_t ld_self, const float* w_packed,
                           int d_out, const float* ep_scale, const float* ep_shift, int relu, float* out,
                           int64_t ldo, const float* w2_packed, int d_out2, float* out2, int64_t ldo2, const int32_t* tile_order,
                           const glnn_hub_plan* plan, void* stream, const glnn_chunk_signals* chunks = nullptr,
                           float* agg_out = nullptr, const float* agg_in = nullptr, int64_t ld_agg = 0) {
  if (n_dst == 0) return GLNN_OK;
  if (agg_in) return sage_fused_agg_in(n_dst, d_in, w_packed, d_out, ep_scale, ep_shift, relu, out, ldo, w2_packed, d_out2, out2, ldo2,
                                       agg_in, ld_agg, stream);
  GLNN_REQUIRE(indptr && x && x_self && w_packed && (out || w2_packed), "glnn_sage_fused_f32: null pointer");
  GLNN_REQUIRE(!w2_packed || (out2 && d_out2 >= 1 && d_out2 <= 256 && ldo2 >= d_out2 && glnn::aligned16(w2_packed)),
               "glnn_sage_fused_f32: the chained projection needs out2 with ldo2 >= d_out2 in [1,256]");
  GLNN_REQUIRE(n_dst >= 0 && n_src >= 0 && n_src < (int64_t)1 << 31, "glnn_sage_fused_f32: bad n_dst/n_src");
  GLNN_REQUIRE(d_in >= 1 && d_in <= 256 && d_out >= 1 && d_out <= 256, "glnn_sage_fused_f32: d_in and d_out must be in [1,256]");
  const int dpad = (d_in + 3) & ~3;
  GLNN_REQUIRE(ldx % 4 == 0 && ldx >= dpad && ld_self % 4 == 0 && ld_self >= dpad && (!out || ldo >= d_out),
               "glnn_sage_fused_f32: leading dimensions (ldx, ld_self multiples of 4 and >= %d; ldo >= d_out)", dpad);
  GLNN_REQUIRE(glnn::aligned16(x) && glnn::aligned16(x_self) && glnn::aligned16(w_packed), "glnn_sage_fused_f32: 16-byte alignment required");
  GLNN_REQUIRE(!agg_out || (ld_agg % 4 == 0 && ld_agg >= dpad && glnn::aligned16(agg_out) && !chunks),
               "glnn_sage_fused_agg_f32: agg_out needs ld_agg a multiple of 4 and >= %d, 16-byte alignment, no chunks", dpad);
  if (n_dst == 0) return GLNN_OK;
  FusedArgs a;
  a.agg_out = agg_out; a.agg_in = nullptr; a.ld_agg = ld_agg;
  a.indptr = indptr; a.indices = indices; a.n_dst = n_dst; a.x = x; a.ldx = ldx; a.d_in = d_in; a.x_self = x_self;
  a.ld_self = ld_self; a.w_packed = w_packed; a.d_out = d_out; a.kgroups = (d_in + 7) / 8; a.ep_scale = ep_scale;
  a.ep_shift = ep_shift; a.relu = relu; a.out = out; a.ldo = ldo;
  a.w2_packed = w2_packed; a.d_out2 = w2_packed ? d_out2 : 0; a.kgroups2 = w2_packed ? (d_out + 7) / 8 : 0; a.out2 = out2; a.ldo2 = ldo2;
  a.tile_order = tile_order;
  {
    const int rcm = fill_chunk_map(chunks, n_dst, &a.cm, "glnn_sage_fused_chunks_f32");
    if (rcm != GLNN_OK) return rcm;
  }
  constexpr int rt = 1;
  const int rows_per_wg = 32 * rt;
  const int64_t blocks = (n_dst + rows_per_wg - 1) / rows_per_wg;
  GLNN_REQUIRE(blocks < ((int64_t)1 << 31), "glnn_sage_fused_f32: n_dst too large for one launch");
  const int kg_lds = a.kgroups2 > a.kgroups ? a.kgroups2 : a.kgroups;
  const size_t smem = sizeof(float) * rows_per_wg * (kg_lds * 8 + 4);
  hipStream_t st = reinterpret_cast<hipStream_t>(stream);
  const int dv = dpad / 4;
  const int kv = a.kgroups * 2;
  int hub_segs = 0;
  {
    const int rch = hub_plan_of(plan, d_in, &a.hub, &hub_segs, "glnn_sage_fused_f32");
    if (rch != GLNN_OK) return rch;
  }
  if (hub_segs > 0) {
    SpmmArgs h = {};
    h.indptr = indptr; h.indices = indices; h.n_dst = n_dst; h.x = x; h.ldx = ldx; h.d = d_in; h.hub = a.hub;
    int rc;
    if (kv <= 16 && dv <= 16) rc = launch_hub_gather<16, GLNN_FUSED_U>(h, GLNN_AGG_SUM, hub_segs, st);
    else if (kv <= 32) rc = launch_hub_gather<32, GLNN_FUSED_U>(h, GLNN_AGG_SUM, hub_segs, st);
    else rc = launch_hub_gather<64, GLNN_FUSED_U>(h, GLNN_AGG_SUM, hub_segs, st);
    if (rc != GLNN_OK) return rc;
  }
#define GLNN_FUSED_LAUNCH(LPR_, RT_)                                                                                                          \
  do {                                                                                                                                        \
    if (a.cm.n) hipLaunchKernelGGL((sage_fused_kernel<LPR_, GLNN_FUSED_U, RT_, true>), dim3((unsigned)blocks), dim3(kFusedBlock), smem, st, a); \
    else if (a.agg_out)                                                                                                                       \
      hipLaunchKernelGGL((sage_fused_kernel<LPR_, GLNN_FUSED_U, RT_, false, kAggOut>), dim3((unsigned)blocks), dim3(kFusedBlock), smem, st, a); \
    else hipLaunchKernelGGL((sage_fused_kernel<LPR_, GLNN_FUSED_U, RT_>), dim3((unsigned)blocks), dim3(kFusedBlock), smem, st, a);             \
  } while (0)
  if (kv <= 16 && dv <= 16) GLNN_FUSED_LAUNCH(16, 1); else if (kv <= 32) GLNN_FUSED_LAUNCH(32, 1); else GLNN_FUSED_LAUNCH(64, 1);
#undef GLNN_FUSED_LAUNCH
  return glnn::check_launch("glnn_sage_fused_f32");
}

extern "C" int glnn_sage_fused_f32(const int64_t* indptr, const int32_t* indices, int64_t n_dst, int64_t n_src, const float* x,
                                   int64_t ldx, int d_in, const float* x_self, int64_t ld_self, const float* w_packed,
                                   int d_out, const float* ep_scale, const float* ep_shift, int relu, float* out,
                                   int64_t ldo, const float* w2_packed, int d_out2, float* out2, int64_t ldo2, const int32_t* tile_order,
                                   void* stream) {
  return sage_fused_impl(indptr, indices, n_dst, n_src, x, ldx, d_in, x_self, ld_self, w_packed, d_out, ep_scale, ep_shift, relu, out, ldo,
                         w2_packed, d_out2, out2, ldo2, tile_order, nullptr, stream);
}

extern "C" int glnn_sage_fused_plan_f32(const int64_t* indptr, const int32_t* indices, int64_t n_dst, int64_t n_src, const float* x,
                                        int64_t ldx, int d_in, const float* x_self, int64_t ld_self, const float* w_packed,
                                        int d_out, const float* ep_scale, const float* ep_shift, int relu, float* out,
                                        int64_t ldo, const float* w2_packed, int d_out2, float* out2, int64_t ldo2, const int32_t* tile_order,
                                        const glnn_hub_plan* plan, void* stream) {
  return sage_fused_impl(indptr, indices, n_dst, n_src, x, ldx, d_in, x_self, ld_self, w_packed, d_out, ep_scale, ep_shift, relu, out, ldo,
                         w2_packed, d_out2, out2, ldo2, tile_order, plan, stream);
}

extern "C" int glnn_sage_fused_chunks_f32(const int64_t* indptr, const int32_t* indices, int64_t n_dst, int64_t n_src, const float* x,
                                          int64_t ldx, int d_in, const float* x_self, int64_t ld_self, const float* w_packed,
                                          int d_out, const float* ep_scale, const float* ep_shift, int relu, float* out,
                                          int64_t ldo, const float* w2_packed, int d_out2, float* out2, int64_t ldo2, const int32_t* tile_order,
                                          const glnn_hub_plan* plan, const glnn_chunk_signals* chunks, void* stream) {
  GLNN_REQUIRE(chunks, "glnn_sage_fused_chunks_f32: chunks is NULL (use glnn_sage_fused_plan_f32)");
  return sage_fused_impl(indptr, indices, n_dst, n_src, x, ldx, d_in, x_self, ld_self, w_packed, d_out, ep_scale, ep_shift, relu, out, ldo,
                         w2_packed, d_out2, out2, ldo2, tile_order, plan, stream, chunks);
}

extern "C" int glnn_sage_fused_agg_f32(const int64_t* indptr, const int32_t* indices, int64_t n_dst, int64_t n_src, const float* x,
                                       int64_t ldx, int d_in, const float* x_self, int64_t ld_self, const float* w_packed,
                                       int d_out, const float* ep_scale, const float* ep_shift, int relu, float* out,
                                       int64_t ldo, const float* w2_packed, int d_out2, float* out2, int64_t ldo2, const int32_t* tile_order,
                                       const glnn_hub_plan* plan, float* agg_out, const float* agg_in, int64_t ld_agg, void* stream) {
  GLNN_REQUIRE((agg_out != nullptr) != (agg_in != nullptr), "glnn_sage_fused_agg_f32: exactly one of agg_out and agg_in must be given");
  return sage_fused_impl(indptr, indices, n_dst, n_src, x, ldx, d_in, x_self, ld_self, w_packed, d_out, ep_scale, ep_shift, relu, out, ldo,
                         w2_packed, d_out2, out2, ldo2, tile_order, plan, stream, nullptr, agg_out, agg_in, ld_agg);
}

extern "C" int glnn_signal_alloc(uint32_t** signal) {
  GLNN_REQUIRE(signal, "glnn_signal_alloc: null pointer");
  void* p = nullptr;
  if (hipExtMallocWithFlags(&p, 8, hipMallocSignalMemory) != hipSuccess || !p) {
    (void)hipGetLastError();
    return glnn::fail(GLNN_ERR_HIP, "glnn_signal_alloc: hipExtMallocWithFlags(hipMallocSignalMemory) failed");
  }
  if (hipMemset(p, 0, 8) != hipSuccess) return glnn::fail(GLNN_ERR_HIP, "glnn_signal_alloc: memset failed");
  *signal = reinterpret_cast<uint32_t*>(p);
  return GLNN_OK;
}

extern "C" int glnn_signal_free(uint32_t* signal) {
  if (signal && hipFree(signal) != hipSuccess) return glnn::fail(GLNN_ERR_HIP, "glnn_signal_free: hipFree failed");
  return GLNN_OK;
}

extern "C" int glnn_signal_read(const uint32_t* signal, uint32_t* value) {
  GLNN_REQUIRE(signal && value, "glnn_signal_read: null pointer");
  if (hipMemcpy(value, signal, 4, hipMemcpyDeviceToHost) != hipSuccess) return glnn::fail(GLNN_ERR_HIP, "glnn_signal_read: copy failed");
  return GLNN_OK;
}

__global__ void signal_fence_kernel() {}

extern "C" int glnn_stream_wait_value32(void* stream, uint32_t* signal, uint32_t value) {
  GLNN_REQUIRE(signal, "glnn_stream_wait_value32: null pointer");
  hipStream_t st = reinterpret_cast<hipStream_t>(stream);
  if (hipStreamWaitValue32(st, signal, value, hipStreamWaitValueGte, 0xffffffffu) != hipSuccess) {
    (void)hipGetLastError();
    return glnn::fail(GLNN_ERR_HIP, "glnn_stream_wait_value32: hipStreamWaitValue32 failed (not supported on this device?)");
  }
  if (glnn::opts().signal_fence) {
    hipLaunchKernelGGL(signal_fence_kernel, dim3(1), dim3(64), 0, st);
    return glnn::check_launch("glnn_stream_wait_value32(fence)");
  }
  return GLNN_OK;
}
```

graphless-neural-networks_amd/graph.py:

```python
import torch


class CSRGraph:
    def __init__(self, indptr, indices, n_dst, n_src=None):
        assert indptr.dtype == torch.int64 and indices.dtype == torch.int32
        assert indptr.numel() == n_dst + 1
        self.indptr = indptr.contiguous()
        self.indices = indices.contiguous()
        self.n_dst = int(n_dst)
        self.n_src = int(n_dst if n_src is None else n_src)
        self.ndata = {}
        self._nnz = None
        self._cache = {}
        self.gindices = None
        self.dst_nodes = None
        self.t_indptr = self.t_indices = self.inv_deg = None
        self.t_add_self = None

    @classmethod
    def from_edges(cls, src, dst, num_nodes):
        src = torch.as_tensor(src, dtype=torch.int64)
        dst = torch.as_tensor(dst, dtype=torch.int64)
        order = torch.argsort(dst, stable=True)
        counts = torch.bincount(dst, minlength=num_nodes)
        indptr = torch.zeros(num_nodes + 1, dtype=torch.int64, device=dst.device)
        torch.cumsum(counts, 0, out=indptr[1:])
        return cls(indptr, src[order].to(torch.int32), num_nodes)

    @property
    def device(self):
        return self.indptr.device

    def num_nodes(self):
        return self.n_src

    number_of_nodes = num_nodes

    def num_src_nodes(self):
        return self.n_src

    def num_dst_nodes(self):
        return self.n_dst

    def num_edges(self):
        if self._nnz is None:
            self._nnz = int(self.indptr[-1].item())
        return self._nnz

    number_of_edges = num_edges

    def int(self):
        return self

    def create_formats_(self):
        return None

    def to(self, device):
        device = torch.device(device) if not isinstance(device, torch.device) else device
        if device == self.indptr.device:
            return self
        g = CSRGraph(self.indptr.to(device), self.indices.to(device), self.n_dst, self.n_src)
        g._nnz = self._nnz
        g.ndata = {k: v.to(device) for k, v in self.ndata.items()}
        return g

    def in_degrees(self):
        return self.indptr[1:] - self.indptr[:-1]

    def out_degrees(self):
        return torch.bincount(self.indices.long(), minlength=self.n_src)

    def degree_norms(self):
        if "norms" not in self._cache:
            from . import ops
            self._cache["norms"] = ops.degrees(self.indptr, self.indices, self.n_dst, self.n_src, self.num_edges(),
                                               transform=ops.DEG_RSQRT_CLAMP1)
        return self._cache["norms"]

    def inv_deg_plus1(self):
        if "inv1" not in self._cache:
            from . import ops
            self._cache["inv1"] = ops.degrees(self.indptr, None, self.n_dst, self.n_src, 0, want_out=False, transform=ops.DEG_INV_PLUS1)[0]
        return self._cache["inv1"]

    def fused_tile_order(self):
        if self.n_dst < 4096 or not self.indptr.is_cuda:
            return None
        if "tile_order" not in self._cache:
            from . import ops
            self._cache["tile_order"] = ops.fused_tile_order(self.indptr, self.n_dst)
        return self._cache["tile_order"]

    def hub_plan(self):
        if not self.indptr.is_cuda or self.n_dst == 0:
            return None
        if "hub_plan" not in self._cache:
            from . import ops
            self._cache["hub_plan"] = ops.hub_plan(self.indptr, self.n_dst)
        return self._cache["hub_plan"]

    def has_zero_in_degree(self):
        if "zero_in" not in self._cache:
            self._cache["zero_in"] = bool((self.in_degrees() == 0).any()) if self.n_dst else False
        return self._cache["zero_in"]

    def transposed(self, add_self=False):
        key = ("tr", bool(add_self))
        if key not in self._cache:
            from . import ops
            t_indptr, t_indices = ops.csr_transpose(self.indptr, self.indices, self.n_dst, self.n_src, self.num_edges(), add_self)
            t = CSRGraph(t_indptr, t_indices, self.n_src, self.n_dst)
            t._nnz = self.num_edges() + (self.n_dst if add_self else 0)
            self._cache[key] = t
        return self._cache[key]

    def transposed_eids(self):
        if "tr_eids" not in self._cache:
            from . import ops
            t_indptr, t_indices, t_eids = ops.csr_transpose_eids(self.indptr, self.indices, self.n_dst, self.n_src, self.num_edges())
            t = CSRGraph(t_indptr, t_indices, self.n_src, self.n_dst)
            t._nnz = self.num_edges()
            self._cache["tr_eids"] = (t, t_eids)
        return self._cache["tr_eids"]

    def reverse(self):
        if self.indptr.is_cuda:
            return self.transposed(False)
        if "rev" not in self._cache:
            dst_all = torch.repeat_interleave(torch.arange(self.n_dst), self.in_degrees())
            src = self.indices.long()
            order = torch.argsort(src, stable=True)
            indptr = torch.zeros(self.n_src + 1, dtype=torch.int64)
            torch.cumsum(torch.bincount(src, minlength=self.n_src), 0, out=indptr[1:])
            self._cache["rev"] = CSRGraph(indptr, dst_all[order].to(torch.int32), self.n_src, self.n_dst)
        return self._cache["rev"]

    def sampled(self, fanout, seed):
        from . import ops
        ops._check_fanout("CSRGraph.sampled", fanout)
        if not self.indptr.is_cuda:
            raise RuntimeError("CSRGraph.sampled: the sampled graph is built on the GPU (move the graph with g.to(device))")
        key = ("sampled_indptr", fanout)
        if key not in self._cache:
            s_indptr = ops.sample_csr_indptr(self.indptr, self.n_dst, fanout)
            self._cache[key] = (s_indptr, int(s_indptr[-1].item()))
        s_indptr, nnz = self._cache[key]
        s_indices = ops.sample_csr_fill(self.indptr, self.indices, self.n_dst, self.n_src, s_indptr, nnz, fanout, int(seed) & 0xFFFFFFFF)
        g = CSRGraph(s_indptr, s_indices, self.n_dst, self.n_src)
        g._nnz = nnz
        g._cache["tile_order"] = None
        return g

    def row_range(self, start, stop):
        lo, hi = int(self.indptr[start].item()), int(self.indptr[stop].item())
        g = CSRGraph((self.indptr[start:stop + 1] - lo).contiguous(), self.indices[lo:hi], stop - start, self.n_src)
        g._nnz = hi - lo
        return g

    def subgraph(self, idx):
        idx = torch.as_tensor(idx, dtype=torch.int64, device=self.device)
        remap = torch.full((self.n_src,), -1, dtype=torch.int64, device=self.device)
        remap[idx] = torch.arange(idx.numel(), device=self.device)
        deg = self.in_degrees()
        dst_all = torch.repeat_interleave(torch.arange(self.n_dst, device=self.device), deg)
        src_new, dst_new = remap[self.indices.long()], remap[dst_all]
        keep = (src_new >= 0) & (dst_new >= 0)
        g = CSRGraph.from_edges(src_new[keep], dst_new[keep], idx.numel())
        g.ndata = {k: v[idx] for k, v in self.ndata.items()}
        return g


class FullNeighborLoader:

    def __init__(self, graph, batch_size):
        self.graph = graph
        self.batch_size = int(batch_size)
        self.global_blocks = False

    def __len__(self):
        return (self.graph.n_dst + self.batch_size - 1) // self.batch_size

    def __iter__(self):
        from . import ops
        g = self.graph
        if not g.indptr.is_cuda:
            raise RuntimeError("FullNeighborLoader: blocks are built on the GPU (move the graph with g.to(device))")
        n = g.n_dst
        bounds = list(range(0, n, self.batch_size)) + [n]
        key = ("loader_offs", self.batch_size)
        if key not in g._cache:
            g._cache[key] = g.indptr[torch.tensor(bounds, device=g.device)].tolist()
        offs = g._cache[key]
        for b in range(len(bounds) - 1):
            s, e = bounds[b], bounds[b + 1]
            if getattr(self, "global_blocks", False):
                output_nodes = None
                block = CSRGraph(g.indptr[s:e + 1], g.indices, e - s, g.n_src)
                block._nnz = offs[b + 1] - offs[b]
                block.dst_range = (s, e)
                block._cache["tile_order"] = None
                yield None, output_nodes, [block]
                continue
            output_nodes = torch.arange(s, e, device=g.device)
            indptr, indices, _, input_nodes, nnz, n_src = ops.block_build(output_nodes, g.indptr, g.indices, nnz_cap=offs[b + 1] - offs[b],
                                                                          n_nodes=g.n_src)
            block = CSRGraph(indptr, indices, e - s, n_src)
            block._nnz = nnz
            yield input_nodes, output_nodes, [block]


class MultiLayerNeighborSampler:

    def __init__(self, fanouts):
        self.fanouts = [int(f) for f in fanouts]


class MultiLayerFullNeighborSampler:

    def __init__(self, n_layers):
        self.n_layers = int(n_layers)


_SIDE_STREAMS = {}


class NodeDataLoader:

    def __init__(self, g, nids, sampler, batch_size=1, shuffle=False, drop_last=False, num_workers=0, seed=None):
        self.g, self.nids, self.sampler = g, torch.as_tensor(nids, dtype=torch.int64), sampler
        self.batch_size, self.shuffle, self.drop_last = int(batch_size), shuffle, drop_last
        self._epoch = 0
        self._seed = int(torch.initial_seed() if seed is None else seed) & 0x7FFFFFFF
        self.prefetch, self._side = True, None
        self.threaded = __import__("os").environ.get("GLNN_LOADER_THREAD", "1") != "0"
        self.depth = 2
        self.global_first_block = False
        self.plain_transpose = False
        if isinstance(sampler, MultiLayerFullNeighborSampler) and sampler.n_layers == 1 and not shuffle \
                and self.nids.numel() == g.num_dst_nodes() and bool((self.nids.cpu() == torch.arange(g.num_dst_nodes())).all()):
            self.graph = g

    def __len__(self):
        n = self.nids.numel()
        return n // self.batch_size if self.drop_last else (n + self.batch_size - 1) // self.batch_size

    def _block(self, seeds, fanout, rng_seed, want_global=False, global_only=False):
        from . import ops
        g = self.g
        if fanout is None:
            deg_sum = int((g.indptr[seeds + 1] - g.indptr[seeds]).sum().item())
            indptr, indices, gidx, input_nodes, nnz, n_src = ops.block_build(seeds, g.indptr, g.indices, nnz_cap=deg_sum,
                                                                              want_global=want_global, n_nodes=g.n_src, global_only=global_only)
# ... 173 lines not shown
```

graphless-neural-networks_amd/models.py:

```python
import contextlib
import os
import weakref

import torch
import torch.nn as nn
import torch.nn.functional as F

from . import _lib, ops
from .autograd import appnp_propagate, gcnii_stack, linear_fn, norm_act_drop
from .kinds import BY_KIND, FULL_GRAPH_KINDS, teacher_kind
from .nn import DAGNNConv, GATConv, GATv2Conv, GCNIIConv, GPRConv, GraphConv, PNAConv, SAGEConv, TransformerConv, _whole_graph_only


def _bn_eval_fold(bn, bias):
    s = bn.weight.detach() * torch.rsqrt(bn.running_var + bn.eps)
    b = bias.detach() if bias is not None else 0.0
    return s.contiguous(), ((b - bn.running_mean) * s + bn.bias.detach()).contiguous()


def _need_hip(x, what):
    if not x.is_cuda:
        raise _lib.GlnnError(f"{what}: tensors must live on the GPU -- this package computes on libglnn_hip.so only, there is no "
                             "CPU path (the reference's default --device -1 selects the CPU: pass --device 0)")

# ... 311 lines not shown
                                      "resident graph); the chunked and literal sweeps are fp32")
        if self.norm_type == "layer":
            raise NotImplementedError("SAGE.inference(dtype=torch.bfloat16): LayerNorm teachers are fp32 only (the per-row statistics pass "
                                      "is not part of the bf16 storage path)")
        with torch.no_grad():
            first = self.layers[0]
            if first._in_feats <= first._out_feats:
                x = ops.as_bf16_feat(feats) if feats.dtype == torch.bfloat16 else ops.to_bf16(feats)
            else:
                x = feats.float() if feats.dtype == torch.bfloat16 else feats
            projected = None
            for l in range(self.num_layers):
                x, projected = self._whole_graph_layer_bf16(l, g, x, projected)
            return x

    def _inference_mean(self, dataloader, feats, whole_graph, dtype):
        if dtype != torch.float32:
            raise NotImplementedError("SAGE.inference(dtype=torch.bfloat16): bf16 activation storage is implemented for the 'gcn' aggregator "
                                      "only, not for aggregator_type 'mean'")
        g = getattr(dataloader, "graph", None)
        if g is None or not (whole_graph or hasattr(dataloader, "global_blocks")):
            raise NotImplementedError("SAGE.inference(aggregator_type 'mean'): a glnn_amd.graph.FullNeighborLoader over the resident graph")
        with torch.no_grad():
            x = ops.as_feat(feats)
            n = g.num_dst_nodes()
            for l, layer in enumerate(self.layers):
                tail = self._layer_tail(l)
                if whole_graph:
                    y = layer(g, (x, x[:n]), ep_scale=tail[0], ep_shift=tail[1], relu=tail[2])
                else:
                    y = ops.feat_empty(n, layer._out_feats, x.device, zero=True)
                    self._mean_engine_layer(l, dataloader, x, y, tail)
                x = _eval_tail(self, l, y) if tail[3] else y
            return x

    def _mean_engine_layer(self, l, dataloader, x, y, tail):
        layer, form = self.layers[l], self.layers[l].mean_form()
        ep_scale, ep_shift, relu, _ = tail
        wn, ws, d, r4 = layer.fc_neigh.weight, layer.fc_self.weight, layer._out_feats, ops.round4(layer._out_feats)
        if form == "project":
            p = ops.gemm(x, ops.stack_weight_pair(wn, ws))
            chunk = lambda s, e, block: ops.spmm_sage_mean(block.indptr, block.indices, p[:, :d], p[s:e, r4:], e - s, ep_scale=ep_scale,
                                                           ep_shift=ep_shift, relu=relu, out=y[s:e])
        else:
            wp = ops.pack_weight_pair(wn, ws) if form == "fused" else None
            chunk = lambda s, e, block: layer(block, (x, x[s:e]), ep_scale=ep_scale, ep_shift=ep_shift, relu=relu, w_packed=wp, out=y[s:e])
        with _chunk_sweep(dataloader, x.device, []) as chunks:
            for _, s, e, block in chunks:
                chunk(s, e, block)

    def _check_fan_out(self, fan_out, dataloader, whole_graph):
        if isinstance(fan_out, (str, bytes)) or not hasattr(fan_out, "__len__"):
            raise ValueError(f"SAGE.inference: fan_out must be a list of {self.num_layers} integers, one per layer (got {fan_out!r})")
        fan_out = list(fan_out)
        if len(fan_out) != self.num_layers:
            raise ValueError(f"SAGE.inference: fan_out names {len(fan_out)} layers, the encoder has {self.num_layers} (got {fan_out!r})")
        for f in fan_out:
            if isinstance(f, bool) or not isinstance(f, int):
                raise ValueError(f"SAGE.inference: fan_out must hold integers (got {f!r} in {fan_out!r})")
            if not 1 <= f <= 64:
                raise ValueError(f"SAGE.inference: every fan_out value must be in [1, 64] (got {f} in {fan_out!r})")
        if not whole_graph:
            raise NotImplementedError("SAGE.inference(fan_out=...): the whole-graph sweep only (whole_graph=True); the chunked and literal "
                                      "sweeps are full-neighbour")
        if getattr(dataloader, "graph", None) is None:
            raise NotImplementedError("SAGE.inference(fan_out=...): a loader over a resident graph (one that sweeps every node in id order "
                                      "and carries `.graph`); this one has none")
        return fan_out

    def inference_over(self, graphs, feats, dtype=torch.float32):
        _need_hip(feats, "SAGE.inference_over")
        if len(graphs) != self.num_layers:
            raise ValueError(f"SAGE.inference_over: {len(graphs)} graphs for {self.num_layers} layers")
        if dtype not in (torch.float32, torch.bfloat16):
            raise ValueError(f"SAGE.inference_over: dtype must be torch.float32 or torch.bfloat16, not {dtype}")
        mean = self.aggregator_type != "gcn"
        if mean:
            _check_tail(self)
            if dtype != torch.float32:
                raise NotImplementedError("SAGE.inference(dtype=torch.bfloat16): bf16 activation storage is implemented for the 'gcn' aggregator "
                                          "only, not for aggregator_type 'mean'")
        elif dtype == torch.bfloat16 and self.norm_type == "layer":
            raise NotImplementedError("SAGE.inference(dtype=torch.bfloat16): LayerNorm teachers are fp32 only (the per-row statistics pass "
                                      "is not part of the bf16 storage path)")
        with torch.no_grad():
            if mean:
                x = ops.as_feat(feats)
                for l, (layer, g) in enumerate(zip(self.layers, graphs)):
                    tail = self._layer_tail(l)
                    y = layer(g, (x, x[:g.num_dst_nodes()]), ep_scale=tail[0], ep_shift=tail[1], relu=tail[2])
                    x = _eval_tail(self, l, y) if tail[3] else y
                return x
            projected = None
            if dtype == torch.bfloat16:
                first = self.layers[0]
                if first._in_feats <= first._out_feats:
                    x = ops.as_bf16_feat(feats) if feats.dtype == torch.bfloat16 else ops.to_bf16(feats)
                else:
                    x = feats.float() if feats.dtype == torch.bfloat16 else feats
                for l, g in enumerate(graphs):
                    x, projected = self._whole_graph_layer_bf16(l, g, x, projected)
                return x
            x = ops.as_feat(feats)
            for l, g in enumerate(graphs):
                x, projected = self._whole_graph_layer(l, g, x, projected, place=False)
            return x

    def sampled_graphs(self, g, fan_out, sample_seed=0):
        return [g.sampled(f, sample_layer_seed(sample_seed, l)) for l, f in enumerate(fan_out)]

    def inference(self, dataloader, feats, whole_graph=True, dtype=torch.float32, fan_out=None, sample_seed=0):
        if fan_out is not None:
            fan_out = self._check_fan_out(fan_out, dataloader, whole_graph)
            _need_hip(feats, "SAGE.inference")
            return self.inference_over(self.sampled_graphs(dataloader.graph, fan_out, sample_seed), feats, dtype)
        _need_hip(feats, "SAGE.inference")
        if dtype not in (torch.float32, torch.bfloat16):
            raise ValueError(f"SAGE.inference: dtype must be torch.float32 or torch.bfloat16, not {dtype}")
        if self.aggregator_type != "gcn":
            _check_tail(self)
            return self._inference_mean(dataloader, feats, whole_graph, dtype)
        if dtype == torch.bfloat16:
            return self._inference_bf16(dataloader, feats, whole_graph)
        g = getattr(dataloader, "graph", None)
        with torch.no_grad():
            x = ops.as_feat(feats)
            if not whole_graph or g is None:
                return self._inference_chunked(dataloader, x)
            x = self._placed_input(g, feats, x)
            agg, agg_ent = self._input_aggregate(g, feats, x)
            projected = None
            for l in range(self.num_layers):
                x, projected = self._whole_graph_layer(l, g, x, projected, agg=agg if l == 0 else None)
                if l == 0 and agg_ent is not None:
                    self.__dict__["_agg_x"] = agg_ent
            return x

    def _inference_chunked(self, dataloader, x):
        for l, layer in enumerate(self.layers):
            tail = self._layer_tail(l)
            y = ops.feat_empty(x.shape[0], self.hidden_dim if l != self.num_layers - 1 else self.output_dim, x.device, zero=True)
            wp = ops.pack_weight(layer.fc_neigh.weight) if layer.fused_eligible() else None
            engine = hasattr(dataloader, "global_blocks") and not tail[3]
            (self._engine_layer if engine else self._literal_layer)(l, dataloader, x, y, tail, wp)
            x = y
        return x

    def _engine_layer(self, l, dataloader, x, y, tail, wp):
        layer, g = self.layers[l], getattr(dataloader, "graph", None)
        ep_scale, ep_shift, relu, _ = tail
        xp = ops.gemm(x, layer.fc_neigh.weight) if layer._in_feats > layer._out_feats else None
        if g is not None and (xp is not None or layer.fused_eligible()):
            tailed = ep_scale is not None or ep_shift is not None or relu
            launch = (ops.RowRangeLaunch(g.indptr, g.indices, xp, y, ep_scale=ep_scale, ep_shift=ep_shift, relu=relu) if xp is not None else
                      ops.RowRangeLaunch(g.indptr, g.indices, x, y, w=layer.fc_neigh.weight, ep_scale=ep_scale,
                                         ep_shift=ep_shift if tailed else layer.fc_neigh.bias, relu=relu, w_packed=wp))
            chunk = lambda s, e, block: launch(s, e)
        elif xp is not None:
            chunk = lambda s, e, block: ops.spmm(block.indptr, block.indices, xp, e - s, ops.AGG_SAGE_GCN, ep_scale=ep_scale, ep_shift=ep_shift,
                                                 relu=relu, out=y[s:e], x_self=xp[s:e])
        else:
            chunk = lambda s, e, block: layer(block, (x, x[s:e]), ep_scale=ep_scale, ep_shift=ep_shift, relu=relu, w_packed=wp, out=y[s:e])
        with _chunk_sweep(dataloader, x.device, _sweep_streams(x.device)) as chunks:
            for _, s, e, block in chunks:
                chunk(s, e, block)

    def _literal_layer(self, l, dataloader, x, y, tail, wp):
        layer, (ep_scale, ep_shift, relu, post_ln) = self.layers[l], tail
        for input_nodes, output_nodes, blocks in dataloader:
            block = blocks[0].int().to(x.device)
            h = ops.gather_rows(x, input_nodes)
            h = layer(block, (h, h[: block.num_dst_nodes()]), ep_scale=ep_scale, ep_shift=ep_shift, relu=relu, w_packed=wp)
            if post_ln:
                h = _eval_tail(self, l, h)
            ops.scatter_rows(h, output_nodes, y)


@contextlib.contextmanager
def _chunk_sweep(dataloader, device, pool):
    def chunks():
        for k, (input_nodes, _, blocks) in enumerate(dataloader):
            if input_nodes is not None:
                raise RuntimeError(f"SAGE.inference: {type(dataloader).__name__} has a global_blocks attribute and ignores it: its chunks carry input_nodes")
            s, e = blocks[0].dst_range
            if pool:
                with torch.cuda.stream(pool[k % len(pool)]):
                    yield k, s, e, blocks[0]
            else:
                yield k, s, e, blocks[0]
    cur = torch.cuda.current_stream(device)
    for st in pool:
        st.wait_stream(cur)
    dataloader.global_blocks = True
    it = chunks()
    try:
        yield it
    finally:
        it.close()
        dataloader.global_blocks = False
    for st in pool:
        cur.wait_stream(st)


SWEEP_STREAMS = int(os.environ.get("GLNN_SWEEP_STREAMS", "8"))
_SWEEP_POOLS = {}


def _sweep_streams(device):
    if SWEEP_STREAMS <= 1 or device.type != "cuda":
        return []
    key = (device.index, SWEEP_STREAMS)
    if key not in _SWEEP_POOLS:
        _SWEEP_POOLS[key] = [torch.cuda.Stream(device=device) for _ in range(SWEEP_STREAMS)]
    return _SWEEP_POOLS[key]


class GCN(nn.Module):

    def __init__(self, num_layers, input_dim, hidden_dim, output_dim, dropout_ratio, activation, norm_type="none"):
        super().__init__()
        self.num_layers = num_layers
        self.norm_type = norm_type
        self.dropout = nn.Dropout(dropout_ratio)
        self.layers = nn.ModuleList()
        self.norms = nn.ModuleList()
        if num_layers == 1:
            self.layers.append(GraphConv(input_dim, output_dim, activation=activation))
        else:
            self.layers.append(GraphConv(input_dim, hidden_dim, activation=activation))
            self._add_norm(hidden_dim)
            for _ in range(num_layers - 2):
                self.layers.append(GraphConv(hidden_dim, hidden_dim, activation=activation))
                self._add_norm(hidden_dim)
            self.layers.append(GraphConv(hidden_dim, output_dim))

    def _add_norm(self, hidden_dim):
        if self.norm_type == "batch":
            self.norms.append(nn.BatchNorm1d(hidden_dim))
        elif self.norm_type == "layer":
            self.norms.append(nn.LayerNorm(hidden_dim))

    def forward(self, g, feats):
        _need_hip(feats, "GCN.forward")
        _check_tail(self)
        h = feats
        h_list = []
        for l, layer in enumerate(self.layers):
            h = layer(g, h)
            if l != self.num_layers - 1:
                h_list.append(h)
                if self.training:
                    if self.norm_type != "none" or self.dropout.p > 0:
                        h = norm_act_drop(h, _norm_of(self, l), self.dropout.p, relu=False)
                elif self.norm_type != "none":
                    with torch.no_grad():
                        h = _eval_tail(self, l, h, relu=False)
        return h_list, h


class _TrunkProp(MLP):

    def __init__(self, num_layers, input_dim, hidden_dim, output_dim, dropout_ratio, activation, norm_type="none"):
        super().__init__(num_layers, input_dim, hidden_dim, output_dim, dropout_ratio, norm_type)
        self.activation = activation
        self.reset_parameters()

    def reset_parameters(self):
        for layer in self.layers:
            layer.reset_parameters()

    def forward(self, g, feats):
        h_list, h = super().forward(feats)
        return h_list, self.propagate(g, h)


class APPNP(_TrunkProp):

    def __init__(self, num_layers, input_dim, hidden_dim, output_dim, dropout_ratio, activation, norm_type="none", edge_drop=0.5,
                 alpha=0.1, k=10):
        super().__init__(num_layers, input_dim, hidden_dim, output_dim, dropout_ratio, activation, norm_type)
        self.k, self.alpha, self.edge_drop = int(k), float(alpha), float(edge_drop)

    def propagate(self, g, h):
        return appnp_propagate(g, h, self.k, self.alpha, self.edge_drop, self.training)


class GPRGNN(_TrunkProp):

    def __init__(self, num_layers, input_dim, hidden_dim, output_dim, dropout_ratio, activation, norm_type="none", k=10, alpha=0.1,
                 init="PPR"):
        super().__init__(num_layers, input_dim, hidden_dim, output_dim, dropout_ratio, activation, norm_type)
        self.propagate = GPRConv(k, alpha, init)
        self.k, self.alpha = self.propagate.k, self.propagate.alpha


class DAGNN(_TrunkProp):

    def __init__(self, num_layers, input_dim, hidden_dim, output_dim, dropout_ratio, activation, norm_type="none", k=10):
        super().__init__(num_layers, input_dim, hidden_dim, output_dim, dropout_ratio, activation, norm_type)
        self.propagate = DAGNNConv(k, output_dim)
        self.k = self.propagate.k


STACK_MAX_LAYERS = 64


class _ConvStack(nn.Module):
    MAX_HIDDEN = WHY = None

    def __init__(self, conv, num_layers, input_dim, hidden_dim, output_dim, dropout_ratio, activation, norm_type):
        super().__init__()
        who, (why_width, why_norm, why_relu) = type(self).__name__, self.WHY
        if hidden_dim > self.MAX_HIDDEN:
            raise NotImplementedError(f"{who}: hidden_dim of at most {self.MAX_HIDDEN} ({why_width}; got {hidden_dim})")
        if norm_type != "none":
            raise NotImplementedError(f"{who}: norm_type 'none' only ({why_norm}; got {norm_type!r})")
        if not 1 <= num_layers <= STACK_MAX_LAYERS:
            raise NotImplementedError(f"{who}: 1 to {STACK_MAX_LAYERS} conv layers (got num_layers {num_layers})")
        if activation is not F.relu and getattr(activation, "__name__", "") != "relu":
            raise NotImplementedError(f"{who}: only the ReLU activation ({why_relu})")
        self.num_layers, self.norm_type, self.activation, self.hidden_dim = num_layers, norm_type, activation, hidden_dim
        self.dropout = nn.Dropout(dropout_ratio)
        self.fc_in = nn.Linear(input_dim, hidden_dim)
        self.layers = nn.ModuleList(conv(l) for l in range(1, num_layers + 1))
        self.fc_out = nn.Linear(hidden_dim, output_dim)

    def forward(self, g, feats):
        who = type(self).__name__
        _need_hip(feats, f"{who}.forward")
        _whole_graph_only(g, feats, who, f"{who} runs on the whole graph")
        if not self.training:
            with torch.no_grad():
                h0 = ops.gemm(ops.as_feat(feats), self.fc_in.weight, ep_shift=self.fc_in.bias, relu=True)
                hs = self.stack(g, h0)
                return hs, ops.gemm(hs[-1], self.fc_out.weight, ep_shift=self.fc_out.bias)
        p = self.dropout.p
        x = norm_act_drop(feats, None, p, relu=False) if p > 0 else feats
        h0 = norm_act_drop(linear_fn(x, self.fc_in.weight, self.fc_in.bias), None, 0.0)
        hs = self.stack(g, h0)
        h = norm_act_drop(hs[-1], None, p, relu=False) if p > 0 else hs[-1]
        return hs, linear_fn(h, self.fc_out.weight, self.fc_out.bias)


class GCNII(_ConvStack):
    MAX_HIDDEN = ops.GCNII_MAX_HIDDEN
    WHY = ("the fused kernel's tile width", "the paper's model has no norm layers", "the fused layer kernel's epilogue")

    def __init__(self, num_layers, input_dim, hidden_dim, output_dim, dropout_ratio, activation, norm_type="none", alpha=0.1, lamda=0.5):
        super().__init__(lambda l: GCNIIConv(hidden_dim, l, alpha, lamda), num_layers, input_dim, hidden_dim, output_dim, dropout_ratio,
                         activation, norm_type)
        self.alpha, self.lamda = float(alpha), float(lamda)

    def betas(self):
        return [layer.beta for layer in self.layers]

    def stack(self, g, h0):
        return gcnii_stack(g, h0, [layer.weight for layer in self.layers], self.alpha, self.betas(),
# ... 173 lines not shown
```

graphless-neural-networks_amd/ops.py:

```python
import ctypes

import torch

from . import _lib

AGG_SUM, AGG_SAGE_GCN = 0, 1
LOSS_NLL, LOSS_KL = 0, 1

_TIMING = None


def set_timing(collector):
    global _TIMING
    _TIMING = collector


class _Timed:
    __slots__ = ("name", "info", "s")

    def __init__(self, name, **info):
        self.name, self.info, self.s = name, info, None

    def __enter__(self):
        if _TIMING is not None:
# ... 21 lines not shown
    return None if t is None else ctypes.c_void_p(t.data_ptr())


def _need_cuda(*ts):
    for t in ts:
        if t is not None and not t.is_cuda:
            raise _lib.GlnnError("glnn_amd.ops: tensors must live on the GPU (HIP path only, no CPU fallback)")


def _vec(t, n, name, dtype=torch.float32):
    if t is None:
        return None
    if t.dtype != dtype or t.dim() != 1 or t.numel() < n or not t.is_contiguous():
        raise ValueError(f"{name}: expected contiguous {dtype} vector with >= {n} elements")
    return t


def _mat(t, name):
    if t.dtype != torch.float32 or t.dim() != 2 or (t.shape[1] > 1 and t.stride(1) != 1):
        raise ValueError(f"{name}: expected 2-D float32 row-major tensor")
    return t


def _ld(t):
    return t.stride(0) if t.shape[0] > 1 else max(t.stride(0), t.shape[1])


def round4(d):
    return (d + 3) // 4 * 4


def feat_empty(n, d, device, zero=False):
    ld = round4(d)
    buf = (torch.zeros if zero else torch.empty)((n, ld), dtype=torch.float32, device=device)
    return buf[:, :d]


DTYPE_F32, DTYPE_BF16 = 0, 1


def round8(d):
    return (d + 7) // 8 * 8


def bf16_empty(n, d, device, zero=False):
    buf = (torch.zeros if zero else torch.empty)((n, round8(d)), dtype=torch.bfloat16, device=device)
    return buf[:, :d]


def _bf16_mat(t, name):
    if t.dtype != torch.bfloat16 or t.dim() != 2 or (t.shape[1] > 1 and t.stride(1) != 1):
        raise ValueError(f"{name}: expected 2-D bfloat16 row-major tensor")
    return t


def as_bf16_feat(t):
    _bf16_mat(t, "as_bf16_feat")
    if _ld(t) % 8 == 0 and _ld(t) >= t.shape[1] and t.data_ptr() % 16 == 0:
        return t
    out = bf16_empty(t.shape[0], t.shape[1], t.device, zero=True)
    out.copy_(t)
    return out


def to_bf16(x, out=None):
    _need_cuda(x, out)
    _mat(x, "to_bf16 x")
    n, d = x.shape
    if out is None:
        out = bf16_empty(n, d, x.device)
    elif tuple(out.shape) != (n, d) or _ld(_bf16_mat(out, "to_bf16 out")) % 8:
        raise ValueError("to_bf16: out must be a bf16 [n, d] tensor with a leading dimension that is a multiple of 8")
    if n == 0 or d == 0:
        return out
    rc = _lib.lib().glnn_cast_f32_bf16(_p(x), _ld(x), n, d, _p(out), _ld(out), _stream())
    _lib.check(rc, "glnn_cast_f32_bf16")
    return out


def _out_like(out, out_dtype, default, n, d, device, name):
    if out_dtype is not None and out_dtype not in (torch.float32, torch.bfloat16):
        raise ValueError(f"{name}: out_dtype must be torch.float32 or torch.bfloat16")
    if out is None:
        dt = default if out_dtype is None else out_dtype
        return bf16_empty(n, d, device) if dt == torch.bfloat16 else feat_empty(n, d, device)
    if out_dtype is not None and out.dtype != out_dtype:
        raise ValueError(f"{name}: out is {out.dtype}, out_dtype {out_dtype}")
    if out.dtype == torch.bfloat16:
        _bf16_mat(out, name)
    else:
        _mat(out, name)
    if out.shape[0] < n or out.shape[1] != d:
        raise ValueError(f"{name}: out must hold {n} rows of {d} columns")
    return out


def _dtype_code(t):
    return DTYPE_BF16 if t.dtype == torch.bfloat16 else DTYPE_F32


_RANDPERM_LOCK = __import__("threading").Lock()


def randperm_cpu(n):
    with _RANDPERM_LOCK:
        k = torch.get_num_threads()
        if k <= 1:
            return torch.randperm(n)
        torch.set_num_threads(1)
        try:
            return torch.randperm(n)
        finally:
            torch.set_num_threads(k)


_PADDED = []


def _pad_key(t):
    try:
        ver = t._version
    except RuntimeError:
        return None
    return (ver, t.data_ptr(), tuple(t.stride()), tuple(t.shape))


def clear_pad_cache():
    _PADDED.clear()


def as_feat(t):
    _mat(t, "as_feat")
    if t.stride(0) % 4 == 0 and t.stride(0) >= t.shape[1] and t.data_ptr() % 16 == 0:
        return t
    _PADDED[:] = [e for e in _PADDED if e[0]() is not None]
    key = _pad_key(t) if (t.numel() >= (1 << 20) and not t.requires_grad) else None
    if key is not None:
        for i, (ref, k, pad) in enumerate(_PADDED):
            if ref() is t and k == key and pad.device == t.device:
                if i:
                    _PADDED.insert(0, _PADDED.pop(i))
                return pad
    out = feat_empty(t.shape[0], t.shape[1], t.device, zero=True)
    out.copy_(t)
    if key is not None:
        import weakref
        _PADDED[:] = [e for e in _PADDED if e[0]() is not t][:1]
        _PADDED.insert(0, (weakref.ref(t), key, out))
    return out


class HubPlan:

    def __init__(self, indptr, n_dst):
        thr, seg = _lib.lib().glnn_hub_row_threshold(), _lib.lib().glnn_hub_segment_edges()
        deg = indptr[1:n_dst + 1] - indptr[:n_dst]
        rows = torch.nonzero(deg > thr).flatten()
        self.n_hub = int(rows.numel())
        self.rows = rows.contiguous()
        segs = (deg[rows] + (seg - 1)) // seg
        self.seg_ptr = torch.zeros(self.n_hub + 1, dtype=torch.int32, device=indptr.device)
        if self.n_hub:
            self.seg_ptr[1:] = segs.cumsum(0).to(torch.int32)
        self.n_seg = int(self.seg_ptr[-1].item()) if self.n_hub else 0
        self.hub_edges = int(deg[rows].sum().item()) if self.n_hub else 0
        self.slab = None
        self.desc = _lib.HubPlanDesc()

    def desc_for(self, d, device):
        if self.n_hub == 0:
            return None
        ld = (d + 3) // 4 * 4
        if self.slab is None or self.slab.shape[1] < ld:
            self.slab = torch.empty(8 * self.n_seg, ld, dtype=torch.float32, device=device)
        p = self.desc
        p.rows, p.seg_ptr, p.n_hub, p.n_seg = _p(self.rows), _p(self.seg_ptr), self.n_hub, self.n_seg
        p.slab, p.ld_slab, p.slab_rows = _p(self.slab), self.slab.shape[1], self.slab.shape[0]
        return ctypes.byref(p)


def hub_plan(indptr, n_dst):
    _need_cuda(indptr)
    plan = HubPlan(indptr, int(n_dst))
    return plan if plan.n_hub else None


def spmm(indptr, indices, x, n_dst, mode, row_scale=None, col_scale=None, ep_scale=None, ep_shift=None,
         relu=False, out=None, x_self=None, self_rows=None, hub=None, chunks=None, out_dtype=None):
    _need_cuda(indptr, indices, x, row_scale, col_scale, ep_scale, ep_shift, out, x_self, self_rows)
    if x.dtype == torch.bfloat16:
        return _spmm_bf16(indptr, indices, x, n_dst, mode, row_scale, col_scale, ep_scale, ep_shift, relu, out, x_self, self_rows, hub,
                          chunks, out_dtype)
    if out_dtype not in (None, torch.float32):
        raise ValueError("spmm: fp32 rows give an fp32 output (a bf16 output needs bf16 rows: ops.to_bf16)")
    x = as_feat(x)
    if self_rows is not None and (self_rows.dtype != torch.int64 or not self_rows.is_contiguous() or self_rows.numel() < n_dst):
        raise ValueError("spmm: self_rows must be a contiguous int64 vector of n_dst row ids")
    if x_self is None:
        x_self = x
    elif (self_rows is None and chunks is None and x_self.shape[0] < n_dst) or x_self.shape[1] != x.shape[1]:
        raise ValueError("spmm: x_self must hold n_dst rows of the same width as x")
    if chunks is not None and (out is None or mode != AGG_SAGE_GCN):
        raise ValueError("spmm(chunks=...): SAGE_GCN with the whole output buffer given (it is addressed by the chunks' rows)")
    n_src, d = x.shape
    if indptr.dtype != torch.int64 or indices.dtype != torch.int32:
        raise ValueError("spmm: indptr must be int64 and indices int32")
    if out is None:
        out = feat_empty(n_dst, d, x.device)
    _mat(out, "spmm out")
    with _Timed("spmm", d=d, n_dst=n_dst, mode=mode):
        rc = _spmm_call(indptr, indices, n_dst, n_src, x, d, mode, row_scale, col_scale, ep_scale, ep_shift, relu, out,
                        as_feat(x_self), self_rows, hub, chunks)
    _lib.check(rc, "glnn_spmm_csr_f32")
    return out


def _spmm_call(indptr, indices, n_dst, n_src, x, d, mode, row_scale, col_scale, ep_scale, ep_shift, relu, out, x_self,
               self_rows=None, hub=None, chunks=None):
    args = (_p(indptr), _p(indices), n_dst, n_src, _p(x), _ld(x), d, mode,
            _p(_vec(row_scale, n_dst, "row_scale")), _p(_vec(col_scale, n_src, "col_scale")),
            _p(x_self) if mode == AGG_SAGE_GCN else None, _ld(x_self), _p(self_rows),
            _p(_vec(ep_scale, d, "ep_scale")), _p(_vec(ep_shift, d, "ep_shift")), 1 if relu else 0,
            _p(out), _ld(out))
    plan = hub.desc_for(d, x.device) if hub is not None else None
    if chunks is not None:
        return _lib.lib().glnn_spmm_csr_chunks_f32(*args, plan, ctypes.byref(chunks), _stream())
    if plan is not None:
        return _lib.lib().glnn_spmm_csr_plan_f32(*args, plan, _stream())
    return _lib.lib().glnn_spmm_csr_f32(*args, _stream())


def _spmm_bf16(indptr, indices, x, n_dst, mode, row_scale, col_scale, ep_scale, ep_shift, relu, out, x_self, self_rows, hub, chunks,
               out_dtype):
    if hub is not None or chunks is not None:
        raise ValueError("spmm: bf16 rows take neither a hub plan nor chunks")
    x = as_bf16_feat(x)
    if self_rows is not None and (self_rows.dtype != torch.int64 or not self_rows.is_contiguous() or self_rows.numel() < n_dst):
        raise ValueError("spmm: self_rows must be a contiguous int64 vector of n_dst row ids")
    if x_self is None:
        x_self = x
    elif x_self.dtype != torch.bfloat16 or (self_rows is None and x_self.shape[0] < n_dst) or x_self.shape[1] != x.shape[1]:
        raise ValueError("spmm: x_self must be bf16 like x and hold n_dst rows of the same width")
    n_src, d = x.shape
    if indptr.dtype != torch.int64 or indices.dtype != torch.int32:
        raise ValueError("spmm: indptr must be int64 and indices int32")
    out = _out_like(out, out_dtype, torch.bfloat16, n_dst, d, x.device, "spmm out")
    x_self = as_bf16_feat(x_self)
    with _Timed("spmm_bf16", d=d, n_dst=n_dst, mode=mode):
        rc = _lib.lib().glnn_spmm_csr_bf16(
            _p(indptr), _p(indices), n_dst, n_src, _p(x), _ld(x), d, mode,
            _p(_vec(row_scale, n_dst, "row_scale")), _p(_vec(col_scale, n_src, "col_scale")),
            _p(x_self) if mode == AGG_SAGE_GCN else None, _ld(x_self), _p(self_rows),
            _p(_vec(ep_scale, d, "ep_scale")), _p(_vec(ep_shift, d, "ep_shift")), 1 if relu else 0,
            _p(out), _ld(out), _dtype_code(out), _stream())
    _lib.check(rc, "glnn_spmm_csr_bf16")
    return out


PARAM_EPOCH = 0


def note_param_write():
    global PARAM_EPOCH
    PARAM_EPOCH += 1


_PACKED = []


def pack_weight(w):
    _need_cuda(w)
    key = (w.data_ptr(), tuple(w.shape), w.stride(0), w._version, PARAM_EPOCH)
    for i, (ref, k, wp) in enumerate(_PACKED):
        if ref() is w and k == key:
            if i:
                _PACKED.insert(0, _PACKED.pop(i))
            return wp
    wp = _pack_weight(w)
    import weakref
    _PACKED[:] = [e for e in _PACKED if e[0]() is not None and e[0]() is not w][:15]
    _PACKED.insert(0, (weakref.ref(w), key, wp))
    return wp


def _pack_weight(w):
    _mat(w, "pack_weight w")
    d_out, d_in = w.shape
    wp = torch.empty(_lib.lib().glnn_packed_weight_floats(d_out, d_in), dtype=torch.float32, device=w.device)
    rc = _lib.lib().glnn_pack_weight_f32(_p(w), _ld(w), d_out, d_in, _p(wp), _stream())
    _lib.check(rc, "glnn_pack_weight_f32")
    return wp


def fused_tile_order(indptr, n_dst):
    deg = (indptr[1:n_dst + 1] - indptr[:n_dst])
    tiles = (n_dst + 31) // 32
    pad = tiles * 32 - n_dst
    if pad:
        deg = torch.cat([deg, deg.new_zeros(pad)])
    return torch.argsort(deg.view(tiles, 32).amax(1), descending=True, stable=True).to(torch.int32)


class ChunkSignals:
    MAX = _lib.MAX_CHUNKS

    def __init__(self, row_start, device):
        n = len(row_start) - 1
        if not 1 <= n <= self.MAX or row_start[0] != 0 or any(r % 32 for r in row_start[:-1]) or any(a > b for a, b in zip(row_start[:-1], row_start[1:])):
            raise ValueError(f"ChunkSignals: 1..{self.MAX} chunks whose first rows are ascending multiples of 32, starting at 0")
        self.row_start, self.n, self.device, self.epoch = [int(r) for r in row_start], n, device, 0
        self.arrivals = torch.zeros(n, dtype=torch.int32, device=device)
        self._signals = []
        for _ in range(n):
            p = ctypes.c_void_p()
            _lib.check(_lib.lib().glnn_signal_alloc(ctypes.byref(p)), "glnn_signal_alloc")
            self._signals.append(p.value)
        self._n_dst = None

    def empty(self, c, n_dst=None):
        n_dst = self._n_dst if n_dst is None else n_dst
        return min(self.row_start[c + 1], n_dst) <= self.row_start[c]

    def launch(self, self_rows, out_rows, n_dst):
        if len(self_rows) != self.n or len(out_rows) != self.n or self.row_start[-1] < n_dst:
            raise ValueError("ChunkSignals.launch: one self row and one output row per chunk, chunks covering the launch's rows")
        self.epoch += 1
        self._n_dst = int(n_dst)
        d = _lib.ChunkSignalsDesc()
        d.n_chunks = self.n
        for c in range(self.n + 1):
            d.row_start[c] = self.row_start[c]
# ... 98 lines not shown
            _p(_vec(ep_shift, d_out, "ep_shift")), 1 if relu else 0, _p(out), _ld(out) if out is not None else 0,
            _p(w2p), d_out2, _p(out_next), _ld(out_next) if out_next is not None else 0, None, None, None, _p(agg), _ld(agg), _stream())
    _lib.check(rc, "glnn_sage_fused_agg_f32")
    return out if w_next is None else (out, out_next)


def _sage_fused_bf16(indptr, indices, x, n_dst, w, ep_scale, ep_shift, relu, out, x_self, w_packed, w_next, out_next, want_out, tile_order,
                     hub, chunks, out_dtype, out_next_dtype):
    if hub is not None or chunks is not None:
        raise ValueError("sage_fused: bf16 rows take neither a hub plan nor chunks")
    x = as_bf16_feat(x)
    if x_self is not None and (x_self.dtype != torch.bfloat16 or x_self.shape[0] < n_dst or x_self.shape[1] != x.shape[1]):
        raise ValueError("sage_fused: x_self must be bf16 like x and hold n_dst rows of the same width")
    x_self = x if x_self is None else as_bf16_feat(x_self)
    n_src, d_in = x.shape
    d_out = w.shape[0]
    if w.shape[1] != d_in:
        raise ValueError("sage_fused: weight must be [d_out, d_in]")
    if indptr.dtype != torch.int64 or indices.dtype != torch.int32:
        raise ValueError("sage_fused: indptr must be int64 and indices int32")
    if tile_order is not None and (tile_order.dtype != torch.int32 or not tile_order.is_contiguous() or tile_order.numel() != (n_dst + 31) // 32):
        raise ValueError("sage_fused: tile_order must be a contiguous int32 permutation of the ceil(n_dst / 32) tile ids")
    if w_packed is None:
        w_packed = pack_weight(w)
    if out is not None or want_out or w_next is None:
        out = _out_like(out, out_dtype, torch.bfloat16, n_dst, d_out, x.device, "sage_fused out")
    w2p, d_out2 = None, 0
    if w_next is not None:
        if w_next.shape[1] != d_out:
            raise ValueError("sage_fused: w_next must be [d_out2, d_out]")
        w2p, d_out2 = pack_weight(w_next), w_next.shape[0]
        out_next = _out_like(out_next, out_next_dtype, torch.bfloat16, n_dst, d_out2, x.device, "sage_fused out_next")
    with _Timed("sage_fused_bf16", d=d_in, n_dst=n_dst, d_out=d_out, d_chain=d_out2, d_written=(d_out if out is not None else 0) + d_out2):
        rc = _lib.lib().glnn_sage_fused_bf16(
            _p(indptr), _p(indices), n_dst, n_src, _p(x), _ld(x), d_in, _p(x_self), _ld(x_self),
            _p(w_packed), d_out, _p(_vec(ep_scale, d_out, "ep_scale")), _p(_vec(ep_shift, d_out, "ep_shift")), 1 if relu else 0,
            _p(out), _ld(out) if out is not None else 0, _dtype_code(out) if out is not None else DTYPE_F32,
            _p(w2p), d_out2, _p(out_next), _ld(out_next) if out_next is not None else 0,
            _dtype_code(out_next) if out_next is not None else DTYPE_F32, _p(tile_order), _stream())
    _lib.check(rc, "glnn_sage_fused_bf16")
    return out if w_next is None else (out, out_next)


_PAIRS = []


def _pair_cached(kind, w_neigh, w_self, build):
    key = tuple((w.data_ptr(), tuple(w.shape), w.stride(0), w._version) for w in (w_neigh, w_self)) + (PARAM_EPOCH,)
    for i, (kd, rn, rs, k, val) in enumerate(_PAIRS):
        if kd == kind and rn() is w_neigh and rs() is w_self and k == key:
            if i:
                _PAIRS.insert(0, _PAIRS.pop(i))
            return val
    val = build()
    import weakref
    _PAIRS[:] = [e for e in _PAIRS if e[1]() is not None and e[2]() is not None
                 and not (e[0] == kind and e[1]() is w_neigh and e[2]() is w_self)][:15]
    _PAIRS.insert(0, (kind, weakref.ref(w_neigh), weakref.ref(w_self), key, val))
    return val


def _check_pair(w_neigh, w_self, who):
    _need_cuda(w_neigh, w_self)
    _mat(w_neigh, who + " w_neigh")
    _mat(w_self, who + " w_self")
    if w_neigh.shape != w_self.shape:
        raise ValueError(f"{who}: fc_neigh.weight and fc_self.weight must have the same [d_out, d_in] shape")


def pack_weight_pair(w_neigh, w_self):
    _check_pair(w_neigh, w_self, "pack_weight_pair")

    def build():
        d_out, d_in = w_neigh.shape
        kpad = round8(d_in)
        cat = torch.zeros(d_out, 2 * kpad, dtype=torch.float32, device=w_neigh.device)
        cat[:, :d_in] = w_neigh.detach()
        cat[:, kpad:kpad + d_in] = w_self.detach()
        return _pack_weight(cat)
    return _pair_cached("cat", w_neigh, w_self, build)


def stack_weight_pair(w_neigh, w_self):
    _check_pair(w_neigh, w_self, "stack_weight_pair")

    def build():
        d_out, d_in = w_neigh.shape
        r4 = round4(d_out)
        st = torch.zeros(r4 + d_out, d_in, dtype=torch.float32, device=w_neigh.device)
        st[:d_out] = w_neigh.detach()
        st[r4:] = w_self.detach()
        return st
    return _pair_cached("stack", w_neigh, w_self, build)


def sage_mean_fused(indptr, indices, x, n_dst, w_neigh, w_self, ep_scale=None, ep_shift=None, relu=False, out=None, x_self=None,
                    self_rows=None, w_packed=None, tile_order=None):
    _need_cuda(indptr, indices, x, ep_scale, ep_shift, out, x_self, self_rows, w_packed, tile_order)
    _check_pair(w_neigh, w_self, "sage_mean_fused")
    x = as_feat(x)
    x_self = x if x_self is None else as_feat(x_self)
    n_src, d_in = x.shape
    d_out = w_neigh.shape[0]
    if w_neigh.shape[1] != d_in or x_self.shape[1] != d_in:
        raise ValueError("sage_mean_fused: weights must be [d_out, d_in] and x_self as wide as x")
    if indptr.dtype != torch.int64 or indices.dtype != torch.int32 or indptr.numel() < n_dst + 1:
        raise ValueError("sage_mean_fused: indptr must be int64 with n_dst + 1 entries and indices int32")
    if self_rows is not None:
        if self_rows.dtype != torch.int64 or not self_rows.is_contiguous() or self_rows.numel() < n_dst:
            raise ValueError("sage_mean_fused: self_rows must be a contiguous int64 vector of n_dst row ids")
    elif x_self.shape[0] < n_dst:
        raise ValueError("sage_mean_fused: x_self must hold n_dst rows")
    if tile_order is not None and (tile_order.dtype != torch.int32 or not tile_order.is_contiguous() or tile_order.numel() != (n_dst + 31) // 32):
        raise ValueError("sage_mean_fused: tile_order must be a contiguous int32 permutation of the ceil(n_dst / 32) tile ids")
    if w_packed is None:
        w_packed = pack_weight_pair(w_neigh, w_self)
    if out is None:
        out = feat_empty(n_dst, d_out, x.device)
    _mat(out, "sage_mean_fused out")
    if out.shape[0] < n_dst or out.shape[1] != d_out:
        raise ValueError("sage_mean_fused: out must hold n_dst rows of d_out columns")
    with _Timed("sage_mean_fused", d=d_in, n_dst=n_dst, d_out=d_out):
        rc = _lib.lib().glnn_sage_mean_fused_f32(
            _p(indptr), _p(indices), n_dst, n_src, _p(x), _ld(x), d_in, _p(x_self), _ld(x_self), _p(self_rows), _p(w_packed), d_out,
            _p(_vec(ep_scale, d_out, "ep_scale")), _p(_vec(ep_shift, d_out, "ep_shift")), 1 if relu else 0, _p(out), _ld(out),
            _p(tile_order), _stream())
    _lib.check(rc, "glnn_sage_mean_fused_f32")
    return out


def spmm_sage_mean(indptr, indices, x, s, n_dst, ep_scale=None, ep_shift=None, relu=False, out=None):
    _need_cuda(indptr, indices, x, s, ep_scale, ep_shift, out)
    x, s = as_feat(x), as_feat(s)
    n_src, d = x.shape
    if s.shape[1] != d or s.shape[0] < n_dst:
        raise ValueError("spmm_sage_mean: s must hold n_dst rows as wide as x")
    if indptr.dtype != torch.int64 or indices.dtype != torch.int32 or indptr.numel() < n_dst + 1:
        raise ValueError("spmm_sage_mean: indptr must be int64 with n_dst + 1 entries and indices int32")
    if out is None:
        out = feat_empty(n_dst, d, x.device)
    _mat(out, "spmm_sage_mean out")
    if out.shape[0] < n_dst or out.shape[1] != d:
        raise ValueError("spmm_sage_mean: out must hold n_dst rows of d columns")
    with _Timed("spmm_sage_mean", d=d, n_dst=n_dst):
        rc = _lib.lib().glnn_spmm_sage_mean_f32(
            _p(indptr), _p(indices), n_dst, n_src, _p(x), _ld(x), d, _p(s), _ld(s), _p(_vec(ep_scale, d, "ep_scale")),
            _p(_vec(ep_shift, d, "ep_shift")), 1 if relu else 0, _p(out), _ld(out), _stream())
    _lib.check(rc, "glnn_spmm_sage_mean_f32")
    return out


class RowRangeLaunch:

    def __init__(self, indptr, indices, x, out, w=None, ep_scale=None, ep_shift=None, relu=False, w_packed=None):
        _need_cuda(indptr, indices, x, out, w, ep_scale, ep_shift)
        x = as_feat(x)
        _mat(out, "RowRangeLaunch out")
        if indptr.dtype != torch.int64 or indices.dtype != torch.int32 or out.shape[0] < indptr.numel() - 1:
            raise ValueError("RowRangeLaunch: indptr int64, indices int32, one output row per CSR row")
        n_src, d_in = x.shape
        self.keep = (indptr, indices, x, out, w, ep_scale, ep_shift)
        self.n = indptr.numel() - 1
        self.ip0, self.x0, self.ldx, self.o0, self.ldo = indptr.data_ptr(), x.data_ptr(), _ld(x), out.data_ptr(), _ld(out)
        if w is None:
            d = d_in
            if out.shape[1] != d:
                raise ValueError("RowRangeLaunch: out must be as wide as x")
            self.fused, self.info = False, dict(d=d, mode=AGG_SAGE_GCN)
            self.tail = (_p(_vec(ep_scale, d, "ep_scale")), _p(_vec(ep_shift, d, "ep_shift")), 1 if relu else 0)
            self.head = (_p(indices),)
            self.mid = (n_src, self.x0, self.ldx, d, AGG_SAGE_GCN, None, None)
        else:
            d_out = w.shape[0]
            if w.shape[1] != d_in or d_in > 256 or d_out > 256 or out.shape[1] != d_out:
                raise ValueError("RowRangeLaunch: weight [d_out, d_in] with d_in, d_out <= 256, out [n, d_out]")
            wp = pack_weight(w) if w_packed is None else w_packed
            self.keep += (wp,)
            self.fused, self.info = True, dict(d=d_in, d_out=d_out, d_chain=0, d_written=d_out)
            self.head = (_p(indices),)
            self.mid = (n_src, self.x0, self.ldx, d_in)
            self.tail = (_p(wp), d_out, _p(_vec(ep_scale, d_out, "ep_scale")), _p(_vec(ep_shift, d_out, "ep_shift")), 1 if relu else 0)
        self.fn = _lib.lib().glnn_sage_fused_f32 if self.fused else _lib.lib().glnn_spmm_csr_f32

    def __call__(self, s, e):
        if not 0 <= s <= e <= self.n:
            raise ValueError("RowRangeLaunch: row range outside the CSR")
        n_dst = e - s
        ip, xs, o = self.ip0 + 8 * s, self.x0 + 4 * self.ldx * s, self.o0 + 4 * self.ldo * s
        if self.fused:
            args = (ip,) + self.head + (n_dst,) + self.mid + (xs, self.ldx) + self.tail + (o, self.ldo, None, 0, None, 0, None, _stream())
        else:
            args = (ip,) + self.head + (n_dst,) + self.mid + (xs, self.ldx, None) + self.tail + (o, self.ldo, _stream())
        if _TIMING is not None:
            with _Timed("sage_fused" if self.fused else "spmm", n_dst=n_dst, **self.info):
                rc = self.fn(*args)
        else:
            rc = self.fn(*args)
        if rc != 0:
            _lib.check(rc, "glnn_sage_fused_f32" if self.fused else "glnn_spmm_csr_f32")


import os as _os
PLACEMENT_CANDIDATES = int(_os.environ.get("GLNN_PLACEMENT_CANDIDATES", "12"))
PLACEMENT_BALLAST_FRAC = float(_os.environ.get("GLNN_PLACEMENT_BALLAST_FRAC", "0.15"))
PLACEMENT_BALLAST_MAX = 48 << 30
PLACEMENT_MIN_BYTES = 1 << 30
PLACEMENT_MAX_BYTES = 8 << 30
PLACEMENT_LOG = []


def placement_applies(rows, d):
    nbytes = 4 * rows * round4(d)
    return PLACEMENT_CANDIDATES > 1 and PLACEMENT_MIN_BYTES <= nbytes <= PLACEMENT_MAX_BYTES


def placed_for_gather(rows, d, device, indptr, indices, n_dst, what="", first=None, zero=False, probe=None):
    if not placement_applies(rows, d):
        return first if first is not None else feat_empty(rows, d, device, zero=zero)
    nbytes_m = 4 * rows * round4(d)
    cands, ballast = ([first] if first is not None else []), []
    scratch = None

    def fallback():
        del cands[:], ballast[:]
        torch.cuda.empty_cache()
        return first if first is not None else feat_empty(rows, d, device, zero=zero)

    try:
        budget = torch.cuda.mem_get_info(device)[0] - 2 * nbytes_m
        want = PLACEMENT_CANDIDATES
        while len(cands) < want:
            if budget < nbytes_m:
                break
            if len(cands) and len(cands) % 4 == 0 and PLACEMENT_BALLAST_FRAC > 0:
                free = torch.cuda.mem_get_info(device)[0]
                nb = int(min(PLACEMENT_BALLAST_FRAC * free, PLACEMENT_BALLAST_MAX))
                if nb >= (1 << 30) and free - nb > 8 * nbytes_m and budget - nb >= (want - len(cands)) * nbytes_m:
                    ballast.append(torch.empty(nb, dtype=torch.uint8, device=device))
                    budget -= nb
            cands.append(feat_empty(rows, d, device, zero=zero))
            budget -= nbytes_m
    except torch.cuda.OutOfMemoryError:
        del ballast[:]
        torch.cuda.empty_cache()
    try:
        if len(cands) <= 1:
            return fallback() if not cands else cands[0]
        if probe is None:
            scratch = feat_empty(n_dst, d, device)

            def probe(c):
                _lib.check(_spmm_call(indptr, indices, n_dst, rows, c, d, AGG_SAGE_GCN, None, None, None, None, False, scratch,
                                      c[:n_dst] if rows >= n_dst else c, None), "glnn_spmm_csr_f32 (placement probe)")
        ms = []
        for c in cands:
            probe(c)
            best = None
            for _ in range(3):
                e0, e1 = torch.cuda.Event(enable_timing=True), torch.cuda.Event(enable_timing=True)
                e0.record()
                probe(c)
                e1.record()
                e1.synchronize()
                t = e0.elapsed_time(e1)
                best = t if best is None else min(best, t)
            ms.append(best)
    except torch.cuda.OutOfMemoryError:
        scratch = None
        return fallback()
    k = min(range(len(cands)), key=lambda i: ms[i])
    PLACEMENT_LOG.append({"what": what, "rows": int(rows), "d": int(d), "ms": [round(v, 3) for v in ms], "chosen": k})
    keep = cands[k]
    del cands, scratch, ballast
    torch.cuda.empty_cache()
    return keep


def place_for_gather(x, indptr, indices, n_dst, what="features"):
    x = as_feat(x)
    if not placement_applies(x.shape[0], x.shape[1]) or x.shape[0] < n_dst:
        return x
    best = placed_for_gather(x.shape[0], x.shape[1], x.device, indptr, indices, n_dst, what=what, first=x)
    if best is not x:
        _storage_copy(best, x)
    return best


def _storage_copy(dst, src):
    d = src.shape[1]
    dst.copy_(src)
    if dst.stride(0) > d:
        torch.as_strided(dst, (dst.shape[0], dst.stride(0) - d), (dst.stride(0), 1), dst.storage_offset() + d).zero_()


DEG_RAW, DEG_RSQRT_CLAMP1, DEG_INV_PLUS1 = 0, 1, 2
SELF_ROWS = True


def degrees(indptr, indices, n_dst, n_src, nnz, want_out=True, transform=DEG_RAW, want_in=True):
    _need_cuda(indptr, indices)
    in_deg = torch.empty(n_dst, dtype=torch.float32, device=indptr.device) if want_in else None
    out_deg = torch.empty(n_src, dtype=torch.float32, device=indptr.device) if want_out else None
    rc = _lib.lib().glnn_degrees_f32(_p(indptr), _p(indices), n_dst, n_src, nnz, transform, _p(in_deg), _p(out_deg), _stream())
    _lib.check(rc, "glnn_degrees_f32")
    return in_deg, out_deg


_DEFAULT_WS = {}


def _default_ws(device):
    key = (str(device), int(_stream().value or 0))
    if key not in _DEFAULT_WS:
        if len(_DEFAULT_WS) >= 8:
            _DEFAULT_WS.clear()
        _DEFAULT_WS[key] = torch.empty(1 << 24, dtype=torch.float32, device=device)
    return _DEFAULT_WS[key]


def gemm(a, w, w_is_kn=False, a_rows=None, a_scale=None, a_shift=None, row_scale=None, ep_scale=None,
         ep_shift=None, relu=False, out=None, m=None, drop_p=0.0, drop_seed=0, workspace=None):
    _need_cuda(a, w, a_rows, a_scale, a_shift, row_scale, ep_scale, ep_shift, out)
    _mat(a, "gemm a")
    _mat(w, "gemm w")
    k = a.shape[1]
    n = w.shape[1] if w_is_kn else w.shape[0]
    if (w.shape[0] if w_is_kn else w.shape[1]) != k:
        raise ValueError(f"gemm: inner dimensions differ: a {tuple(a.shape)} w {tuple(w.shape)} kn={w_is_kn}")
    if m is None:
        m = a_rows.numel() if a_rows is not None else a.shape[0]
    if a_rows is not None and (a_rows.dtype != torch.int64 or not a_rows.is_contiguous()):
        raise ValueError("gemm: a_rows must be contiguous int64")
    if out is None:
        out = feat_empty(m, n, a.device)
    _mat(out, "gemm out")
    if w.stride(0) % 4 and w.numel() <= (1 << 22) and (w_is_kn or k < 4 or n > 512 or m >= 1024):
        w = as_feat(w)
    if workspace is None and m * n <= (1 << 22) and k >= 2048:
        workspace = _default_ws(a.device)
    with _Timed("gemm", m=m, k=k, n=n):
        rc = _gemm_call(a, a_rows, a_scale, a_shift, drop_p, drop_seed, m, k, w, w_is_kn, n, row_scale, ep_scale, ep_shift, relu, out,
                        workspace)
    _lib.check(rc, "glnn_gemm_f32")
    return out


def _gemm_call(a, a_rows, a_scale, a_shift, drop_p, drop_seed, m, k, w, w_is_kn, n, row_scale, ep_scale, ep_shift, relu, out,
               workspace):
    return _lib.lib().glnn_gemm_f32(
        _p(a), _ld(a), _p(a_rows), _p(_vec(a_scale, k, "a_scale")), _p(_vec(a_shift, k, "a_shift")),
# ... 1290 lines not shown
```

include/glnn_hip.h:

```cpp
#ifndef GLNN_HIP_H
#define GLNN_HIP_H

#include <stdint.h>

#ifdef __cplusplus
extern "C" {
#endif

#define GLNN_API __attribute__((visibility("default")))

typedef enum {
  GLNN_OK = 0,
  GLNN_ERR_INVALID_ARG = -1,
  GLNN_ERR_UNSUPPORTED = -2,
  GLNN_ERR_HIP = -3,
  GLNN_ERR_NO_DEVICE = -4
} glnn_status;

GLNN_API int glnn_abi_version(void);
GLNN_API const char* glnn_last_error(void);
GLNN_API int glnn_device_info(int* cu_count, int* xcd_count, char* arch_buf, int arch_buf_len);
GLNN_API int64_t glnn_struct_bytes(int which);
GLNN_API void glnn_reload_options(void);

#define GLNN_AGG_SUM 0
#define GLNN_AGG_SAGE_GCN 1

GLNN_API int glnn_spmm_csr_f32(const int64_t* indptr, const int32_t* indices, int64_t n_dst,
                               int64_t n_src, const float* x, int64_t ldx, int d, int mode,
                               const float* row_scale, const float* col_scale,
                               const float* x_self, int64_t ld_self, const int64_t* self_rows,
                               const float* ep_scale, const float* ep_shift, int relu, float* out,
                               int64_t ldo, void* stream);

GLNN_API int64_t glnn_packed_weight_floats(int d_out, int d_in);
GLNN_API int glnn_pack_weight_f32(const float* w, int64_t ldw, int d_out, int d_in, float* w_packed,
                                  void* stream);
GLNN_API int glnn_sage_fused_f32(const int64_t* indptr, const int32_t* indices, int64_t n_dst,
                                 int64_t n_src, const float* x, int64_t ldx, int d_in,
                                 const float* x_self, int64_t ld_self, const float* w_packed,
                                 int d_out, const float* ep_scale, const float* ep_shift, int relu,
                                 float* out, int64_t ldo, const float* w2_packed, int d_out2,
                                 float* out2, int64_t ldo2, const int32_t* tile_order, void* stream);

typedef struct glnn_hub_plan {
  const int64_t* rows;
  const int32_t* seg_ptr;
  int32_t n_hub, n_seg;
  float* slab;
  int64_t ld_slab, slab_rows;
} glnn_hub_plan;
GLNN_API int glnn_hub_row_threshold(void);
GLNN_API int glnn_hub_segment_edges(void);
GLNN_API int glnn_spmm_csr_plan_f32(const int64_t* indptr, const int32_t* indices, int64_t n_dst,
                                    int64_t n_src, const float* x, int64_t ldx, int d, int mode,
                                    const float* row_scale, const float* col_scale,
                                    const float* x_self, int64_t ld_self, const int64_t* self_rows,
                                    const float* ep_scale, const float* ep_shift, int relu, float* out,
                                    int64_t ldo, const glnn_hub_plan* plan, void* stream);
GLNN_API int glnn_sage_fused_plan_f32(const int64_t* indptr, const int32_t* indices, int64_t n_dst,
                                      int64_t n_src, const float* x, int64_t ldx, int d_in,
                                      const float* x_self, int64_t ld_self, const float* w_packed,
                                      int d_out, const float* ep_scale, const float* ep_shift, int relu,
                                      float* out, int64_t ldo, const float* w2_packed, int d_out2,
                                      float* out2, int64_t ldo2, const int32_t* tile_order,
                                      const glnn_hub_plan* plan, void* stream);
GLNN_API int glnn_sage_fused_agg_f32(const int64_t* indptr, const int32_t* indices, int64_t n_dst,
                                     int64_t n_src, const float* x, int64_t ldx, int d_in,
                                     const float* x_self, int64_t ld_self, const float* w_packed,
                                     int d_out, const float* ep_scale, const float* ep_shift, int relu,
                                     float* out, int64_t ldo, const float* w2_packed, int d_out2,
                                     float* out2, int64_t ldo2, const int32_t* tile_order,
                                     const glnn_hub_plan* plan, float* agg_out, const float* agg_in,
                                     int64_t ld_agg, void* stream);

#define GLNN_MAX_CHUNKS 8
typedef struct glnn_chunk_signals {
  int32_t n_chunks;
  int64_t row_start[GLNN_MAX_CHUNKS + 1];
  int64_t self_row[GLNN_MAX_CHUNKS];
  int64_t out_row[GLNN_MAX_CHUNKS];
  int32_t* arrivals;
  uint32_t* signal[GLNN_MAX_CHUNKS];
  uint32_t epoch;
} glnn_chunk_signals;
GLNN_API int glnn_sage_fused_chunks_f32(const int64_t* indptr, const int32_t* indices, int64_t n_dst,
                                        int64_t n_src, const float* x, int64_t ldx, int d_in,
                                        const float* x_self, int64_t ld_self, const float* w_packed,
                                        int d_out, const float* ep_scale, const float* ep_shift, int relu,
                                        float* out, int64_t ldo, const float* w2_packed, int d_out2,
                                        float* out2, int64_t ldo2, const int32_t* tile_order,
                                        const glnn_hub_plan* plan, const glnn_chunk_signals* chunks, void* stream);
GLNN_API int glnn_spmm_csr_chunks_f32(const int64_t* indptr, const int32_t* indices, int64_t n_dst,
                                      int64_t n_src, const float* x, int64_t ldx, int d, int mode,
                                      const float* row_scale, const float* col_scale,
                                      const float* x_self, int64_t ld_self, const int64_t* self_rows,
                                      const float* ep_scale, const float* ep_shift, int relu, float* out,
                                      int64_t ldo, const glnn_hub_plan* plan, const glnn_chunk_signals* chunks,
                                      void* stream);
GLNN_API int glnn_signal_alloc(uint32_t** signal);
GLNN_API int glnn_signal_free(uint32_t* signal);
GLNN_API int glnn_signal_read(const uint32_t* signal, uint32_t* value);
GLNN_API int glnn_stream_wait_value32(void* stream, uint32_t* signal, uint32_t value);

#define GLNN_DEG_RAW 0
#define GLNN_DEG_RSQRT_CLAMP1 1
#define GLNN_DEG_INV_PLUS1 2
GLNN_API int glnn_degrees_f32(const int64_t* indptr, const int32_t* indices, int64_t n_dst,
                              int64_t n_src, int64_t nnz, int transform, float* in_deg,
                              float* out_deg, void* stream);

GLNN_API int glnn_gemm_f32(const float* a, int64_t lda, const int64_t* a_rows,
                           const float* a_scale, const float* a_shift, float drop_p,
                           uint32_t drop_seed, int64_t m, int k,
                           const float* b, int64_t ldb, int b_layout, int n,
                           const float* row_scale, const float* ep_scale, const float* ep_shift,
                           int relu, float* c, int64_t ldc, float* workspace,
                           int64_t workspace_floats, void* stream);

GLNN_API int glnn_gemm_tn_f32(const float* a, int64_t lda, int64_t m, int ka, const float* b,
                              int64_t ldb, const int64_t* b_rows, const float* b_scale,
                              const float* b_shift, float drop_p, uint32_t drop_seed, int nb,
                              float* c, int64_t ldc,
                              float* col_sum_a, float* workspace, int64_t workspace_floats,
                              void* stream);

#define GLNN_LOSS_NLL 0
#define GLNN_LOSS_KL 1
GLNN_API int glnn_softmax_loss_f32(const float* logits, int64_t ldz, int64_t rows, int c, int kind,
                                   const int64_t* labels, const int64_t* label_rows,
                                   const float* target_logp, int64_t ldt, const int64_t* target_rows,
                                   float lamb, float* dlogits, int64_t ldg, float* logprob_out,
                                   int64_t ldl, float* loss_out, float* loss_accum,
                                   float* workspace, int64_t workspace_floats, void* stream);

GLNN_API int glnn_classifier_loss_f32(const float* a, int64_t lda, const float* a_scale, const float* a_shift,
                                      float drop_p, uint32_t drop_seed, int64_t rows, int k, const float* w, int64_t ldw,
                                      int c, const float* bias, float* logits, int64_t ldz, int kind,
                                      const int64_t* labels, const int64_t* label_rows, const float* target_logp,
                                      int64_t ldt, const int64_t* target_rows, float lamb, float* dlogits, int64_t ldg,
                                      float* loss_out, float* loss_accum, float* workspace, int64_t workspace_floats,
                                      void* stream);

GLNN_API int glnn_log_softmax_f32(const float* logits, int64_t ldz, int64_t rows, int c, float* out,
                                  int64_t ldo, void* stream);

GLNN_API int glnn_bn_stats_f32(const float* z, int64_t ldz, int64_t rows, int h, const float* gamma,
                               const float* beta, float eps, float momentum, float* running_mean,
                               float* running_var, int64_t* num_batches_tracked, float* mean_out,
                               float* rstd_out, float* a_scale_out, float* a_shift_out,
                               float* workspace, int64_t workspace_floats, void* stream);

GLNN_API int glnn_linear_bn_stats_f32(const float* a, int64_t lda, int64_t m, int k, const float* w, int64_t ldw, int n,
                                      const float* bias, float* z, int64_t ldz, const float* gamma, const float* beta,
                                      float eps, float momentum, float* running_mean, float* running_var,
                                      int64_t* num_batches_tracked, float* mean_out, float* rstd_out, float* a_scale_out,
                                      float* a_shift_out, float* ws_gemm, int64_t ws_gemm_floats, float* ws_bn,
                                      int64_t ws_bn_floats, void* stream);

GLNN_API int glnn_bn_relu_bwd_f32(const float* da, int64_t ldda, const float* z, int64_t ldz,
                                  int64_t rows, int h, const float* gamma, const float* mean,
                                  const float* rstd, const float* a_scale, const float* a_shift,
                                  float drop_p, uint32_t drop_seed,
                                  float* dz, int64_t lddz, float* dgamma, float* dbeta,
                                  float* dz_col_sum,
                                  float* workspace, int64_t workspace_floats, void* stream);

GLNN_API int glnn_col_sum_f32(const float* x, int64_t ldx, int64_t rows, int h, float* out,
                              float* workspace, int64_t workspace_floats, void* stream);

GLNN_API int glnn_adam_step_f32(float* const* params, const float* const* grads,
                                float* const* exp_avg, float* const* exp_avg_sq,
                                const int64_t* sizes, int num_tensors, int64_t max_size,
                                float lr, float beta1, float beta2, float eps, float weight_decay,
                                int64_t step, void* stream);

#define GLNN_MLP_MAX_LAYERS 8
#define GLNN_MLP_COUNTERS 1024

typedef int (*glnn_exchange_fn)(void* ctx, const float* send, float* recv, int64_t floats, void* stream);

typedef struct glnn_mlp_step_desc {
  int32_t num_layers;
  int32_t batchnorm;
  int32_t dims[GLNN_MLP_MAX_LAYERS + 1];
  float dropout_p;
  float bn_eps;
  float bn_momentum;
  int64_t max_batch;
  float* w[GLNN_MLP_MAX_LAYERS];
  float* b[GLNN_MLP_MAX_LAYERS];
  float* gw[GLNN_MLP_MAX_LAYERS];
  float* gb[GLNN_MLP_MAX_LAYERS];
  float* gamma[GLNN_MLP_MAX_LAYERS];
  float* beta[GLNN_MLP_MAX_LAYERS];
  float* ggamma[GLNN_MLP_MAX_LAYERS];
  float* gbeta[GLNN_MLP_MAX_LAYERS];
  float* running_mean[GLNN_MLP_MAX_LAYERS];
  float* running_var[GLNN_MLP_MAX_LAYERS];
  int64_t* nbt[GLNN_MLP_MAX_LAYERS];
  float* mean[GLNN_MLP_MAX_LAYERS];
  float* rstd[GLNN_MLP_MAX_LAYERS];
  float* a_scale[GLNN_MLP_MAX_LAYERS];
  float* a_shift[GLNN_MLP_MAX_LAYERS];
  float* z[GLNN_MLP_MAX_LAYERS];
  int64_t ldz[GLNN_MLP_MAX_LAYERS];
// ... 357 lines not shown
```

Measured before the change: 15.53 billion edges/s.

## Precompute long-row sums via hub gather plan in row-range sweep launches

Per-row-range hub plans are built and cached so that long rows (above the long-row threshold, up to one hub segment) are gathered by the wide hub_gather kernel ahead of the main SpMM/fused kernel. The long-row role then only reads one precomputed slab entry instead of doing an 8-wave block gather. A cached device-side plan validation with a host sync is also added. The aim is to take long-row gathers off the serialized long-row blocks and spread them across the grid, at the cost of an extra launch, slab traffic, and a one-time sync per plan.

```diff
diff --git a/graphless-neural-networks_amd/_lib.py b/graphless-neural-networks_amd/_lib.py
--- a/graphless-neural-networks_amd/_lib.py
+++ b/graphless-neural-networks_amd/_lib.py
@@ -24,6 +24,7 @@
                              c_i64, c_int, c_vp, c_int, c_vp, c_i64, c_int, c_vp, c_vp],
     "glnn_hub_row_threshold": [],
     "glnn_hub_segment_edges": [],
+    "glnn_long_row_threshold": [],
     "glnn_spmm_csr_plan_f32": [c_vp, c_vp, c_i64, c_i64, c_vp, c_i64, c_int, c_int, c_vp, c_vp, c_vp, c_i64, c_vp, c_vp, c_vp,
                                c_int, c_vp, c_i64, c_vp, c_vp],
     "glnn_sage_fused_plan_f32": [c_vp, c_vp, c_i64, c_i64, c_vp, c_i64, c_int, c_vp, c_i64, c_vp, c_int, c_vp, c_vp, c_int, c_vp,
diff --git a/graphless-neural-networks_amd/csrc/spmm.hip b/graphless-neural-networks_amd/csrc/spmm.hip
--- a/graphless-neural-networks_amd/csrc/spmm.hip
+++ b/graphless-neural-networks_amd/csrc/spmm.hip
@@ -1,3 +1,7 @@
+#include <map>
+#include <mutex>
+#include <tuple>
+
 #include "glnn_common.h"
 #include "source_tail_dev.h"
 
@@ -288,6 +292,15 @@
   return t;
 }
 
+template <int LPR>
+__device__ __forceinline__ bool plan_long_share(const HubPlan& h, int64_t v, int col4, bool col_ok, int wave, int lane, float4& acc) {
+  const int hi = hub_find(h, v);
+  if (hi < 0) return false;
+  acc = make_float4(0.f, 0.f, 0.f, 0.f);
+  if (lane < LPR && col_ok) acc = ld4(h.slab + ((int64_t)h.seg_ptr[hi] * 8 + wave) * h.ld_slab + col4);
+  return true;
+}
+
 template <int LPR, int U, bool CS, int XF>
 __global__ __launch_bounds__(kBlock) void hub_gather_kernel(const SpmmArgs a) {
   const int lane = threadIdx.x & 63;
@@ -310,7 +323,7 @@
   if (lane < LPR && col_ok) st4(a.hub.slab + ((int64_t)sg * 8 + wave) * a.hub.ld_slab + col4, acc);
 }
 
-template <int LPR, int U, int MODE, bool CS, int XF = 0>
+template <int LPR, int U, int MODE, bool CS, int XF = 0, bool LP = false>
 __device__ __forceinline__ void long_rows_role(const SpmmArgs& a, int lane, int wave, int col4, bool col_ok, const EpCols& ep,
                                                const TailCols& xf) {
   __shared__ int64_t s_rows[kBlock];
@@ -333,6 +346,8 @@
       float4 acc;
       if (e1 - e0 > kHubRow)
         acc = hub_wave_share<LPR, U, CS, XF>(a.hub, a.indices, v, e0, e1, a.x, a.ldx, col4, col_ok, a.col_scale, wave, lane, xf);
+      else if (LP && e1 - e0 <= kHubSeg && plan_long_share<LPR>(a.hub, v, col4, col_ok, wave, lane, acc))
+        ;
       else
         acc = wave_gather_sum<LPR, U, CS, XF>(a.indices, e0, e1, wave, kWavesPerBlock, a.x, a.ldx, col4, col_ok, a.col_scale, lane, xf);
       if (lane < LPR) s_part[wave][lane] = acc;
@@ -348,7 +363,7 @@
   }
 }
 
-template <int LPR, int U, int MODE, bool CS, int XF>
+template <int LPR, int U, int MODE, bool CS, int XF, bool LP = false>
 __device__ __forceinline__ void long_rows_role_chunks(const SpmmArgs& a, const ChunkMap& cm, int lane, int wave, int col4, bool col_ok,
                                                       const EpCols& ep, const TailCols& xf) {
   __shared__ int64_t s_rows[kBlock];
@@ -382,6 +397,8 @@
         float4 acc;
         if (e1 - e0 > kHubRow)
           acc = hub_wave_share<LPR, U, CS, XF>(a.hub, a.indices, v, e0, e1, a.x, a.ldx, col4, col_ok, a.col_scale, wave, lane, xf);
+        else if (LP && e1 - e0 <= kHubSeg && plan_long_share<LPR>(a.hub, v, col4, col_ok, wave, lane, acc))
+          ;
         else
           acc = wave_gather_sum<LPR, U, CS, XF>(a.indices, e0, e1, wave, kWavesPerBlock, a.x, a.ldx, col4, col_ok, a.col_scale, lane, xf);
         if (lane < LPR) s_part[wave][lane] = acc;
@@ -405,7 +422,7 @@
   }
 }
 
-template <int LPR, int U, int MODE, bool CS, int XF = 0, bool CM = false>
+template <int LPR, int U, int MODE, bool CS, int XF = 0, bool CM = false, bool LP = false>
 __global__ __launch_bounds__(kBlock) void spmm_csr_kernel(const SpmmArgs a0) {
   SpmmArgs a = a0;
   if (gridDim.y > 1) {
@@ -425,8 +442,8 @@
   if (XF) xf = load_tail_cols(a.xf_scale, a.xf_shift, a.xf_mean, a.xf_rstd, a.xf_thr, a.xf_seed, a.xf_dscale, a.d, col_ok ? col4 : 0, a.xf_on);
 
   if ((int)blockIdx.x < a.n_long_blocks) {
-    if constexpr (CM) long_rows_role_chunks<LPR, U, MODE, CS, XF>(a, a0.cm, lane, wave, col4, col_ok, ep, xf);
-    else long_rows_role<LPR, U, MODE, CS, XF>(a, lane, wave, col4, col_ok, ep, xf);
+    if constexpr (CM) long_rows_role_chunks<LPR, U, MODE, CS, XF, LP>(a, a0.cm, lane, wave, col4, col_ok, ep, xf);
+    else long_rows_role<LPR, U, MODE, CS, XF, LP>(a, lane, wave, col4, col_ok, ep, xf);
     return;
   }
 
@@ -936,7 +953,7 @@
 
 constexpr int kAggNone = 0, kAggOut = 1, kAggIn = 2;
 
-template <int LPR, int U, int RT, bool CM = false, int AGG = kAggNone>
+template <int LPR, int U, int RT, bool CM = false, int AGG = kAggNone, bool LP = false>
 __global__ __launch_bounds__(kFusedBlock) void sage_fused_kernel(const FusedArgs a) {
   constexpr int kFusedRows = 32 * RT;
   extern __shared__ __attribute__((aligned(16))) float lds_a[];
@@ -1011,9 +1028,17 @@
     if (v >= a.n_dst) break;
     const int64_t e0 = a.indptr[v], e1 = a.indptr[v + 1];
     if (e1 - e0 <= kLongRow) continue;
-    const float4 acc = e1 - e0 > kHubRow
-        ? hub_wave_share<LPR, U, false, false>(a.hub, a.indices, v, e0, e1, a.x, a.ldx, col4, col_ok, nullptr, wave, lane, TailCols{})
-        : wave_gather_sum<LPR, U, false>(a.indices, e0, e1, wave, kFusedWaves, a.x, a.ldx, col4, col_ok, nullptr, lane, TailCols{});
+    float4 acc;
+    if constexpr (LP) {
+      if (e1 - e0 > kHubRow)
+        acc = hub_wave_share<LPR, U, false, false>(a.hub, a.indices, v, e0, e1, a.x, a.ldx, col4, col_ok, nullptr, wave, lane, TailCols{});
+      else if (!(e1 - e0 <= kHubSeg && plan_long_share<LPR>(a.hub, v, col4, col_ok, wave, lane, acc)))
+        acc = wave_gather_sum<LPR, U, false>(a.indices, e0, e1, wave, kFusedWaves, a.x, a.ldx, col4, col_ok, nullptr, lane, TailCols{});
+    } else {
+      acc = e1 - e0 > kHubRow
+          ? hub_wave_share<LPR, U, false, false>(a.hub, a.indices, v, e0, e1, a.x, a.ldx, col4, col_ok, nullptr, wave, lane, TailCols{})
+          : wave_gather_sum<LPR, U, false>(a.indices, e0, e1, wave, kFusedWaves, a.x, a.ldx, col4, col_ok, nullptr, lane, TailCols{});
+    }
     if (wave >= 4 && lane < LPR) s_part[wave - 4][lane] = acc;
     __syncthreads();
     if (wave < 4 && lane < LPR) s_part[wave][lane] = add4(acc, s_part[wave][lane]);
@@ -1156,9 +1181,27 @@
 }
 
 template <int LPR, int U>
-int launch_lpr(const SpmmArgs& a, int mode, hipStream_t st, int grid, int col_tiles = 1, int hub_segs = 0, bool short_rows = false) {
+int launch_lpr(const SpmmArgs& a, int mode, hipStream_t st, int grid, int col_tiles = 1, int hub_segs = 0, bool short_rows = false,
+               bool lp = false) {
   const bool cs = a.col_scale != nullptr;
   const dim3 g(grid, col_tiles);
+  if (lp) {
+    if (a.xf_on || col_tiles != 1)
+      return glnn::fail(GLNN_ERR_UNSUPPORTED, "glnn_spmm_csr_plan_f32: a plan with long rows takes rows of <= 256 floats without a source transform");
+    const int rc = launch_hub_gather<LPR, U>(a, mode, hub_segs, st);
+    if (rc != GLNN_OK) return rc;
+    if (a.cm.n > 0) {
+      if (mode != GLNN_AGG_SAGE_GCN) return glnn::fail(GLNN_ERR_UNSUPPORTED, "glnn_spmm_csr_chunks_f32: SAGE_GCN only");
+      hipLaunchKernelGGL((spmm_csr_kernel<LPR, U, GLNN_AGG_SAGE_GCN, false, false, true, true>), g, dim3(kBlock), 0, st, a);
+    } else if (mode == GLNN_AGG_SAGE_GCN) {
+      hipLaunchKernelGGL((spmm_csr_kernel<LPR, U, GLNN_AGG_SAGE_GCN, false, false, false, true>), g, dim3(kBlock), 0, st, a);
+    } else if (cs) {
+      hipLaunchKernelGGL((spmm_csr_kernel<LPR, U, GLNN_AGG_SUM, true, false, false, true>), g, dim3(kBlock), 0, st, a);
+    } else {
+      hipLaunchKernelGGL((spmm_csr_kernel<LPR, U, GLNN_AGG_SUM, false, false, false, true>), g, dim3(kBlock), 0, st, a);
+    }
+    return glnn::check_launch("glnn_spmm_csr_plan_f32(long rows)");
+  }
   if (hub_segs > 0) {
     const int rc = launch_hub_gather<LPR, U>(a, mode, hub_segs, st);
     if (rc != GLNN_OK) return rc;
@@ -1212,20 +1255,80 @@
   if (i < n) p[i] = degree_transform((float)reinterpret_cast<int*>(p)[i], transform);
 }
 
-}
-
-static int hub_plan_of(const glnn_hub_plan* plan, int d, HubPlan* h, int* n_seg, const char* who) {
+constexpr int kPlanBad = 1, kPlanLong = 2, kPlanRefused = 4;
+__global__ void hub_plan_check_kernel(const int64_t* __restrict__ indptr, int64_t n_dst, const int64_t* __restrict__ rows,
+                                      const int32_t* __restrict__ seg_ptr, int n_hub, int n_seg, int* flags) {
+  const int i = (int)(blockIdx.x * blockDim.x + threadIdx.x);
+  if (i >= n_hub) return;
+  int f = 0;
+  const int64_t r = rows[i];
+  if (r < 0 || r >= n_dst || (i > 0 && rows[i - 1] >= r)) {
+    f = kPlanBad;
+  } else {
+    const int64_t deg = indptr[r + 1] - indptr[r];
+    if ((int64_t)(seg_ptr[i + 1] - seg_ptr[i]) != (deg + kHubSeg - 1) / kHubSeg) f = kPlanBad;
+    else if (deg > kHubRow) f = 0;
+    else if (deg > kLongRow && deg <= kHubSeg) f = kPlanLong;
+    else f = kPlanRefused;
+  }
+  if ((i == 0 && seg_ptr[0] != 0) || (i == n_hub - 1 && seg_ptr[n_hub] != n_seg)) f |= kPlanBad;
+  if (f) atomicOr(flags, f);
+}
+
+}
+
+static int hub_plan_flags(const glnn_hub_plan* plan, const int64_t* indptr, int64_t n_dst, hipStream_t st, int* flags_out, const char* who) {
+  using Key = std::tuple<const void*, int64_t, const void*, const void*, int, int>;
+  static std::mutex mu;
+  static std::map<Key, int> seen;
+  static int* d_flags = nullptr;
+  const Key key(indptr, n_dst, plan->rows, plan->seg_ptr, plan->n_hub, plan->n_seg);
+  std::lock_guard<std::mutex> lock(mu);
+  const auto it = seen.find(key);
+  if (it != seen.end()) { *flags_out = it->second; return GLNN_OK; }
+  if (!d_flags && hipMalloc(reinterpret_cast<void**>(&d_flags), sizeof(int)) != hipSuccess) {
+    d_flags = nullptr;
+    return glnn::fail(GLNN_ERR_HIP, "%s: no memory for the plan check", who);
+  }
+  int flags = 0;
+  if (hipMemsetAsync(d_flags, 0, sizeof(int), st) != hipSuccess) return glnn::fail(GLNN_ERR_HIP, "%s: plan check (memset)", who);
+  hipLaunchKernelGGL(hub_plan_check_kernel, dim3((unsigned)((plan->n_hub + 255) / 256)), dim3(256), 0, st, indptr, n_dst, plan->rows,
+                     plan->seg_ptr, plan->n_hub, plan->n_seg, d_flags);
+  const int rc = glnn::check_launch(who);
+  if (rc != GLNN_OK) return rc;
+  if (hipMemcpyAsync(&flags, d_flags, sizeof(int), hipMemcpyDeviceToHost, st) != hipSuccess || hipStreamSynchronize(st) != hipSuccess)
+    return glnn::fail(GLNN_ERR_HIP, "%s: plan check (read-back)", who);
+  if (seen.size() >= (size_t)1 << 16) seen.clear();
+  if (!(flags & (kPlanBad | kPlanRefused))) seen[key] = flags;
+  *flags_out = flags;
+  return GLNN_OK;
+}
+
+static int hub_plan_of(const glnn_hub_plan* plan, const int64_t* indptr, int64_t n_dst, int d, hipStream_t st, HubPlan* h, int* n_seg,
+                       bool* long_rows, const char* who) {
   h->rows = nullptr; h->seg_ptr = nullptr; h->n_hub = 0; h->slab = nullptr; h->ld_slab = 0;
   *n_seg = 0;
+  *long_rows = false;
   if (!plan || plan->n_hub == 0) return GLNN_OK;
   const int dpad = (d + 3) & ~3;
   GLNN_REQUIRE(plan->n_hub > 0 && plan->n_seg >= plan->n_hub && plan->rows && plan->seg_ptr && plan->slab, "%s: incomplete hub plan", who);
   GLNN_REQUIRE(plan->ld_slab % 4 == 0 && plan->ld_slab >= dpad && plan->slab_rows >= 8 * (int64_t)plan->n_seg && glnn::aligned16(plan->slab),
                "%s: the hub plan's slab needs >= %d rows (8 per segment) of >= %d floats (ld multiple of 4), 16-byte aligned", who, 8 * plan->n_seg, dpad);
+  int flags = 0;
+  const int rcf = hub_plan_flags(plan, indptr, n_dst, st, &flags, who);
+  if (rcf != GLNN_OK) return rcf;
+  GLNN_REQUIRE(!(flags & kPlanBad), "%s: malformed hub plan (ascending row ids inside the launch's rows, ceil(degree / %d) segments each, "
+               "seg_ptr running from 0 to n_seg)", who, kHubSeg);
+  GLNN_REQUIRE(!(flags & kPlanRefused), "%s: the plan lists a row of %d..%d in-edges (two segments would not sum to the owner's bits) or of "
+               "<= %d: a plan holds rows of more than %d in-edges and, if wanted, one-segment long rows of %d..%d", who, kHubSeg + 1, kHubRow,
+               kLongRow, kHubRow, kLongRow + 1, kHubSeg);
   h->rows = plan->rows; h->seg_ptr = plan->seg_ptr; h->n_hub = plan->n_hub; h->slab = plan->slab; h->ld_slab = plan->ld_slab;
   *n_seg = plan->n_seg;
+  *long_rows = (flags & kPlanLong) != 0;
   return GLNN_OK;
 }
+
+extern "C" int glnn_long_row_threshold(void) { return kLongRow; }
 
 static int fill_chunk_map(const glnn_chunk_signals* chunks, int64_t n_dst, ChunkMap* cm, const char* who) {
   *cm = ChunkMap{};
@@ -1300,8 +1403,9 @@
       if (rcm != GLNN_OK) return rcm;
     }
     int hub_segs = 0;
+    bool lp = false;
     {
-      const int rch = hub_plan_of(d <= 256 ? plan : nullptr, d, &a.hub, &hub_segs, "glnn_spmm_csr_f32");
+      const int rch = hub_plan_of(d <= 256 ? plan : nullptr, indptr, n_dst, d, st, &a.hub, &hub_segs, &lp, "glnn_spmm_csr_f32");
       if (rch != GLNN_OK) return rch;
     }
     int64_t n_long = (n_dst + GLNN_LONG_BLOCK_ROWS - 1) / GLNN_LONG_BLOCK_ROWS;
@@ -1326,11 +1430,11 @@
     const int dv = (dt + 3) / 4;
     const bool short_rows = nnz_hint >= 0 && nnz_hint <= 6 * n_dst && glnn::opts().spmm_short != 0 && a.rows_per_block % kShortRows == 0;
     int rc;
-    if (dv <= 4) rc = launch_lpr<4, GLNN_SPMM_U>(a, mode, st, grid, 1, hub_segs);
-    else if (dv <= 8) rc = launch_lpr<8, GLNN_SPMM_U>(a, mode, st, grid, 1, hub_segs);
-    else if (dv <= 16) rc = launch_lpr<16, GLNN_SPMM_U>(a, mode, st, grid, 1, hub_segs);
-    else if (dv <= 32) rc = launch_lpr<32, GLNN_SPMM_U>(a, mode, st, grid, 1, hub_segs, short_rows);
-    else rc = launch_lpr<64, GLNN_SPMM_U>(a, mode, st, grid, wide ? (d + 255) / 256 : 1, hub_segs, short_rows);
+    if (dv <= 4) rc = launch_lpr<4, GLNN_SPMM_U>(a, mode, st, grid, 1, hub_segs, false, lp);
+    else if (dv <= 8) rc = launch_lpr<8, GLNN_SPMM_U>(a, mode, st, grid, 1, hub_segs, false, lp);
+    else if (dv <= 16) rc = launch_lpr<16, GLNN_SPMM_U>(a, mode, st, grid, 1, hub_segs, false, lp);
+    else if (dv <= 32) rc = launch_lpr<32, GLNN_SPMM_U>(a, mode, st, grid, 1, hub_segs, short_rows, lp);
+    else rc = launch_lpr<64, GLNN_SPMM_U>(a, mode, st, grid, wide ? (d + 255) / 256 : 1, hub_segs, short_rows, lp);
     if (rc != GLNN_OK) return rc;
   }
   return GLNN_OK;
@@ -1581,8 +1685,9 @@
   const int dv = dpad / 4;
   const int kv = a.kgroups * 2;
   int hub_segs = 0;
+  bool lp = false;
   {
-    const int rch = hub_plan_of(plan, d_in, &a.hub, &hub_segs, "glnn_sage_fused_f32");
+    const int rch = hub_plan_of(plan, indptr, n_dst, d_in, st, &a.hub, &hub_segs, &lp, "glnn_sage_fused_f32");
     if (rch != GLNN_OK) return rch;
   }
   if (hub_segs > 0) {
@@ -1601,7 +1706,21 @@
       hipLaunchKernelGGL((sage_fused_kernel<LPR_, GLNN_FUSED_U, RT_, false, kAggOut>), dim3((unsigned)blocks), dim3(kFusedBlock), smem, st, a); \
     else hipLaunchKernelGGL((sage_fused_kernel<LPR_, GLNN_FUSED_U, RT_>), dim3((unsigned)blocks), dim3(kFusedBlock), smem, st, a);             \
   } while (0)
-  if (kv <= 16 && dv <= 16) GLNN_FUSED_LAUNCH(16, 1); else if (kv <= 32) GLNN_FUSED_LAUNCH(32, 1); else GLNN_FUSED_LAUNCH(64, 1);
+#define GLNN_FUSED_LAUNCH_LP(LPR_, RT_)                                                                                                       \
+  do {                                                                                                                                        \
+    if (a.cm.n)                                                                                                                               \
+      hipLaunchKernelGGL((sage_fused_kernel<LPR_, GLNN_FUSED_U, RT_, true, kAggNone, true>), dim3((unsigned)blocks), dim3(kFusedBlock), smem, st, a); \
+    else if (a.agg_out)                                                                                                                       \
+      hipLaunchKernelGGL((sage_fused_kernel<LPR_, GLNN_FUSED_U, RT_, false, kAggOut, true>), dim3((unsigned)blocks), dim3(kFusedBlock), smem, st, a); \
+    else                                                                                                                                      \
+      hipLaunchKernelGGL((sage_fused_kernel<LPR_, GLNN_FUSED_U, RT_, false, kAggNone, true>), dim3((unsigned)blocks), dim3(kFusedBlock), smem, st, a); \
+  } while (0)
+  if (lp) {
+    if (kv <= 16 && dv <= 16) GLNN_FUSED_LAUNCH_LP(16, 1); else if (kv <= 32) GLNN_FUSED_LAUNCH_LP(32, 1); else GLNN_FUSED_LAUNCH_LP(64, 1);
+  } else {
+    if (kv <= 16 && dv <= 16) GLNN_FUSED_LAUNCH(16, 1); else if (kv <= 32) GLNN_FUSED_LAUNCH(32, 1); else GLNN_FUSED_LAUNCH(64, 1);
+  }
+#undef GLNN_FUSED_LAUNCH_LP
 #undef GLNN_FUSED_LAUNCH
   return glnn::check_launch("glnn_sage_fused_f32");
 }
diff --git a/graphless-neural-networks_amd/graph.py b/graphless-neural-networks_amd/graph.py
--- a/graphless-neural-networks_amd/graph.py
+++ b/graphless-neural-networks_amd/graph.py
@@ -98,6 +98,14 @@
             from . import ops
             self._cache["hub_plan"] = ops.hub_plan(self.indptr, self.n_dst)
         return self._cache["hub_plan"]
+
+    def range_plans(self):
+        if not self.indptr.is_cuda or self.n_dst == 0:
+            return None
+        if "range_plans" not in self._cache:
+            from . import ops
+            self._cache["range_plans"] = ops.RangePlans(self.indptr)
+        return self._cache["range_plans"]
 
     def has_zero_in_degree(self):
         if "zero_in" not in self._cache:
diff --git a/graphless-neural-networks_amd/models.py b/graphless-neural-networks_amd/models.py
--- a/graphless-neural-networks_amd/models.py
+++ b/graphless-neural-networks_amd/models.py
@@ -487,9 +487,11 @@
         xp = ops.gemm(x, layer.fc_neigh.weight) if layer._in_feats > layer._out_feats else None
         if g is not None and (xp is not None or layer.fused_eligible()):
             tailed = ep_scale is not None or ep_shift is not None or relu
-            launch = (ops.RowRangeLaunch(g.indptr, g.indices, xp, y, ep_scale=ep_scale, ep_shift=ep_shift, relu=relu) if xp is not None else
+            plans = g.range_plans() if SWEEP_PLANS else None
+            launch = (ops.RowRangeLaunch(g.indptr, g.indices, xp, y, ep_scale=ep_scale, ep_shift=ep_shift, relu=relu, plans=plans)
+                      if xp is not None else
                       ops.RowRangeLaunch(g.indptr, g.indices, x, y, w=layer.fc_neigh.weight, ep_scale=ep_scale,
-                                         ep_shift=ep_shift if tailed else layer.fc_neigh.bias, relu=relu, w_packed=wp))
+                                         ep_shift=ep_shift if tailed else layer.fc_neigh.bias, relu=relu, w_packed=wp, plans=plans))
             chunk = lambda s, e, block: launch(s, e)
         elif xp is not None:
             chunk = lambda s, e, block: ops.spmm(block.indptr, block.indices, xp, e - s, ops.AGG_SAGE_GCN, ep_scale=ep_scale, ep_shift=ep_shift,
@@ -538,6 +540,7 @@
 
 
 SWEEP_STREAMS = int(os.environ.get("GLNN_SWEEP_STREAMS", "8"))
+SWEEP_PLANS = os.environ.get("GLNN_SWEEP_PLANS", "1") != "0"
 _SWEEP_POOLS = {}
 
 
diff --git a/graphless-neural-networks_amd/ops.py b/graphless-neural-networks_amd/ops.py
--- a/graphless-neural-networks_amd/ops.py
+++ b/graphless-neural-networks_amd/ops.py
@@ -197,31 +197,61 @@
 
 class HubPlan:
 
-    def __init__(self, indptr, n_dst):
-        thr, seg = _lib.lib().glnn_hub_row_threshold(), _lib.lib().glnn_hub_segment_edges()
+    def __init__(self, indptr, n_dst, long_rows=False):
+        h = _lib.lib()
+        thr, seg, long_thr = h.glnn_hub_row_threshold(), h.glnn_hub_segment_edges(), h.glnn_long_row_threshold()
         deg = indptr[1:n_dst + 1] - indptr[:n_dst]
-        rows = torch.nonzero(deg > thr).flatten()
+        listed = deg > thr
+        if long_rows:
+            listed = listed | ((deg > long_thr) & (deg <= seg))
+        rows = torch.nonzero(listed).flatten()
         self.n_hub = int(rows.numel())
         self.rows = rows.contiguous()
         segs = (deg[rows] + (seg - 1)) // seg
         self.seg_ptr = torch.zeros(self.n_hub + 1, dtype=torch.int32, device=indptr.device)
+        self.n_seg = self.hub_edges = self.n_long = 0
         if self.n_hub:
             self.seg_ptr[1:] = segs.cumsum(0).to(torch.int32)
-        self.n_seg = int(self.seg_ptr[-1].item()) if self.n_hub else 0
-        self.hub_edges = int(deg[rows].sum().item()) if self.n_hub else 0
+            self.n_seg, self.hub_edges, self.n_long = torch.stack([segs.sum(), deg[rows].sum(), (deg[rows] <= thr).sum()]).tolist()
         self.slab = None
         self.desc = _lib.HubPlanDesc()
 
-    def desc_for(self, d, device):
+    def desc_for(self, d, device, slab=None):
         if self.n_hub == 0:
             return None
         ld = (d + 3) // 4 * 4
-        if self.slab is None or self.slab.shape[1] < ld:
-            self.slab = torch.empty(8 * self.n_seg, ld, dtype=torch.float32, device=device)
+        if slab is None:
+            if self.slab is None or self.slab.shape[1] < ld:
+                self.slab = torch.empty(8 * self.n_seg, ld, dtype=torch.float32, device=device)
+            slab = self.slab
         p = self.desc
         p.rows, p.seg_ptr, p.n_hub, p.n_seg = _p(self.rows), _p(self.seg_ptr), self.n_hub, self.n_seg
-        p.slab, p.ld_slab, p.slab_rows = _p(self.slab), self.slab.shape[1], self.slab.shape[0]
+        p.slab, p.ld_slab, p.slab_rows = _p(slab), _ld(slab), slab.shape[0]
         return ctypes.byref(p)
+
+
+class RangePlans:
+    SLAB_LD = 256
+
+    def __init__(self, indptr):
+        self.indptr, self.plans, self.slabs = indptr, {}, {}
+
+    def plan(self, s, e):
+        key = (s, e)
+        if key not in self.plans:
+            p = HubPlan(self.indptr[s:e + 1], e - s, long_rows=True)
+            self.plans[key] = p if p.n_hub else None
+        return self.plans[key]
+
+    def desc_for(self, s, e, d, stream_ptr):
+        p = self.plan(s, e)
+        if p is None:
+            return None
+        slab = self.slabs.get(stream_ptr)
+        if slab is None or slab.shape[0] < 8 * p.n_seg:
+            rows = 8 * max([p.n_seg] + [q.n_seg for q in self.plans.values() if q is not None])
+            slab = self.slabs[stream_ptr] = torch.empty(rows, self.SLAB_LD, dtype=torch.float32, device=self.indptr.device)
+        return p.desc_for(d, self.indptr.device, slab=slab)
 
 
 def hub_plan(indptr, n_dst):
@@ -626,7 +656,7 @@
 
 class RowRangeLaunch:
 
-    def __init__(self, indptr, indices, x, out, w=None, ep_scale=None, ep_shift=None, relu=False, w_packed=None):
+    def __init__(self, indptr, indices, x, out, w=None, ep_scale=None, ep_shift=None, relu=False, w_packed=None, plans=None):
         _need_cuda(indptr, indices, x, out, w, ep_scale, ep_shift)
         x = as_feat(x)
         _mat(out, "RowRangeLaunch out")
@@ -655,21 +685,29 @@
             self.mid = (n_src, self.x0, self.ldx, d_in)
             self.tail = (_p(wp), d_out, _p(_vec(ep_scale, d_out, "ep_scale")), _p(_vec(ep_shift, d_out, "ep_shift")), 1 if relu else 0)
         self.fn = _lib.lib().glnn_sage_fused_f32 if self.fused else _lib.lib().glnn_spmm_csr_f32
+        self.fn_plan = _lib.lib().glnn_sage_fused_plan_f32 if self.fused else _lib.lib().glnn_spmm_csr_plan_f32
+        if plans is not None and plans.indptr is not indptr:
+            raise ValueError("RowRangeLaunch: plans must be the RangePlans of this indptr")
+        self.plans = plans if self.info["d"] <= RangePlans.SLAB_LD else None
 
     def __call__(self, s, e):
         if not 0 <= s <= e <= self.n:
             raise ValueError("RowRangeLaunch: row range outside the CSR")
         n_dst = e - s
         ip, xs, o = self.ip0 + 8 * s, self.x0 + 4 * self.ldx * s, self.o0 + 4 * self.ldo * s
+        st = _stream()
+        plan = self.plans.desc_for(s, e, self.info["d"], st.value) if self.plans is not None else None
+        fn = self.fn if plan is None else self.fn_plan
         if self.fused:
-            args = (ip,) + self.head + (n_dst,) + self.mid + (xs, self.ldx) + self.tail + (o, self.ldo, None, 0, None, 0, None, _stream())
+            args = (ip,) + self.head + (n_dst,) + self.mid + (xs, self.ldx) + self.tail + (o, self.ldo, None, 0, None, 0, None)
         else:
-            args = (ip,) + self.head + (n_dst,) + self.mid + (xs, self.ldx, None) + self.tail + (o, self.ldo, _stream())
+            args = (ip,) + self.head + (n_dst,) + self.mid + (xs, self.ldx, None) + self.tail + (o, self.ldo)
+        args += (st,) if plan is None else (plan, st)
         if _TIMING is not None:
             with _Timed("sage_fused" if self.fused else "spmm", n_dst=n_dst, **self.info):
-                rc = self.fn(*args)
+                rc = fn(*args)
         else:
-            rc = self.fn(*args)
+            rc = fn(*args)
         if rc != 0:
             _lib.check(rc, "glnn_sage_fused_f32" if self.fused else "glnn_spmm_csr_f32")
 
diff --git a/include/glnn_hip.h b/include/glnn_hip.h
--- a/include/glnn_hip.h
+++ b/include/glnn_hip.h
@@ -52,6 +52,7 @@
 } glnn_hub_plan;
 GLNN_API int glnn_hub_row_threshold(void);
 GLNN_API int glnn_hub_segment_edges(void);
+GLNN_API int glnn_long_row_threshold(void);
 GLNN_API int glnn_spmm_csr_plan_f32(const int64_t* indptr, const int32_t* indices, int64_t n_dst,
                                     int64_t n_src, const float* x, int64_t ldx, int d, int mode,
                                     const float* row_scale, const float* col_scale,
```

Result: no change. 15.52 billion edges/s (median of 2 runs) (-0.0%).
